# kristi700/ViT-SSL

Hardware: AMD Instinct MI355X
Metric: images_per_sec (higher is better)
Workload: dtype bf16; 1 GPU; ViT-B/16 SimMIM 224x224 mask 0.6 dropout 0.1 AdamW, batch 256/GPU; global_batch=256, parallelism=dp1

## Files before the change

### vit-ssl_amd/csrc/elementwise.hip

```cpp
#include "common.h"

namespace {

constexpr int EW_THREADS = 256;

inline unsigned ew_grid(long long work_items) {
  long long g = (work_items + EW_THREADS - 1) / EW_THREADS;
  if (g < 1) g = 1;
  return (unsigned)g;
}

__global__ void dropout_mask_kernel(unsigned char* keep, long long ngroups, DropKey dk) {
  const long long grp = (long long)blockIdx.x * blockDim.x + threadIdx.x;
  if (grp >= ngroups) return;
  float m[4];
  drop_mult4(dk, (unsigned)grp, m);
  uchar4 o;
  o.x = m[0] != 0.f; o.y = m[1] != 0.f; o.z = m[2] != 0.f; o.w = m[3] != 0.f;
  if (dk.thr == 0) o = make_uchar4(1, 1, 1, 1);
  *(uchar4*)(keep + 4 * grp) = o;
}

template <bool GATHER, typename OutT>
__global__ void patchify_kernel(const float* __restrict__ img, const int* __restrict__ idx, OutT* __restrict__ out,
                                long long nrows, int C, int H, int W, int P) {
  const int gw = W / P, gh = H / P;
  const int pd4 = C * P * P / 4;
  const long long t = (long long)blockIdx.x * blockDim.x + threadIdx.x;
  if (t >= nrows * pd4) return;
  const long long r = t / pd4;
  const int f = (int)(t - r * pd4) * 4;
  const long long m = GATHER ? (long long)idx[r] : r;
  const long long b = m / (gh * gw);
  const int pi = (int)(m - b * gh * gw);
  const int py = pi / gw, px = pi - py * gw;
  const int c = f / (P * P);
  const int kh = (f - c * P * P) / P;
  const int kw = f - c * P * P - kh * P;
  const f32x4 v = *(const f32x4*)(img + ((b * C + c) * H + (py * P + kh)) * (long long)W + px * P + kw);
  if constexpr (sizeof(OutT) == 2) {
    u32x2 w = {pack_bf2(v[0], v[1]), pack_bf2(v[2], v[3])};
    *(u32x2*)((bf16_t*)out + r * (4LL * pd4) + f) = w;
  } else {
    *(f32x4*)((float*)out + r * (4LL * pd4) + f) = v;
  }
}

__global__ void gather_rows_bf16_kernel(const float* __restrict__ x, const int* __restrict__ idx, bf16_t* __restrict__ out,
                                        int n_idx, int cols) {
  const int c4n = cols >> 2;
  const long long t = (long long)blockIdx.x * blockDim.x + threadIdx.x;
  if (t >= (long long)n_idx * c4n) return;
  const int i = (int)(t / c4n);
  const int c = (int)(t - (long long)i * c4n) * 4;
  const f32x4 v = *(const f32x4*)(x + (long long)idx[i] * cols + c);
  u32x2 w = {pack_bf2(v[0], v[1]), pack_bf2(v[2], v[3])};
  *(u32x2*)(out + (long long)i * cols + c) = w;
}

__global__ void scatter_rows_f32_kernel(const bf16_t* __restrict__ src, const int* __restrict__ inv, float* __restrict__ g,
                                        long long rows, int cols) {
  const int c4n = cols >> 2;
  const long long t = (long long)blockIdx.x * blockDim.x + threadIdx.x;
  if (t >= rows * c4n) return;
  const long long r = t / c4n;
  const int c = (int)(t - r * c4n) * 4;
  const int i = inv[r];
  f32x4 v = {0.f, 0.f, 0.f, 0.f};
  if (i >= 0) {
    const u32x2 w = *(const u32x2*)(src + (long long)i * cols + c);
    v = f32x4{bf_lo(w[0]), bf_hi(w[0]), bf_lo(w[1]), bf_hi(w[1])};
  }
  *(f32x4*)(g + r * cols + c) = v;
}

__global__ void gather_cls_kernel(const float* __restrict__ x, float* __restrict__ out, int B, int T, int D) {
  const int d4n = D >> 2;
  const long long t = (long long)blockIdx.x * blockDim.x + threadIdx.x;
  if (t >= (long long)B * d4n) return;
  const int b = (int)(t / d4n);
  const int c = (int)(t - (long long)b * d4n) * 4;
  *(f32x4*)(out + (long long)b * D + c) = *(const f32x4*)(x + (long long)b * T * D + c);
}

__global__ void scatter_cls_kernel(const float* __restrict__ gcls, float* __restrict__ g, int B, int T, int D) {
  const int d4n = D >> 2;
  const long long t = (long long)blockIdx.x * blockDim.x + threadIdx.x;
  if (t >= (long long)B * T * d4n) return;
  const long long row = t / d4n;
  const int c = (int)(t - row * d4n) * 4;
  const long long b = row / T;
  f32x4 v = {0.f, 0.f, 0.f, 0.f};
  if (row - b * T == 0) v = *(const f32x4*)(gcls + b * D + c);
  *(f32x4*)(g + row * D + c) = v;
}

__global__ void embed_bwd_kernel(const float* __restrict__ dtok, const unsigned char* __restrict__ mask,
                                 bf16_t* __restrict__ dproj, float* __restrict__ dpos, float* __restrict__ dmask_token,
                                 float* __restrict__ dbias, float* __restrict__ dcls, int B, int tokens, int tok_offset, int D,
                                 float* __restrict__ ws, float* __restrict__ pos_parts) {
  const int t = blockIdx.x;
  const int T_out = tokens + tok_offset;
  const int per = (B + gridDim.y - 1) / gridDim.y;
  const int b0 = blockIdx.y * per;
  const int b1 = min(B, b0 + per);
  for (int c = threadIdx.x * 4; c < D; c += blockDim.x * 4) {
    f32x4 pos = {0.f, 0.f, 0.f, 0.f}, mt = pos, bias = pos;
    for (int bb = b0; bb < b1; bb += 4) {
      f32x4 v[4];
#pragma unroll
      for (int u = 0; u < 4; ++u)
        if (bb + u < b1) v[u] = *(const f32x4*)(dtok + ((long long)(bb + u) * T_out + t) * D + c);
#pragma unroll
      for (int u = 0; u < 4; ++u) {
        const int b = bb + u;
        if (b >= b1) break;
        pos += v[u];
        if (t >= tok_offset) {
          const long long m = (long long)b * tokens + (t - tok_offset);
          const bool masked = mask && mask[m];
          u32x2 w = {0u, 0u};
          if (masked) {
            mt += v[u];
          } else {
            bias += v[u];
            w = u32x2{pack_bf2(v[u][0], v[u][1]), pack_bf2(v[u][2], v[u][3])};
// ... 290 lines not shown
extern "C" int vitssl_dropout_mask(uint8_t* keep, int64_t rows, int64_t cols, vitssl_dropout_t d, void* stream) {
  VS_CHECK_ARG(keep && rows > 0 && cols > 0 && cols % 4 == 0, "dropout_mask: cols must be a multiple of 4");
  VS_CHECK_ARG((unsigned long long)rows * (unsigned long long)cols < (1ull << 34), "dropout_mask: the stream's group counter is 32 bits (rows * cols < 2^34)");
  const long long ng = rows * cols / 4;
  hipLaunchKernelGGL(dropout_mask_kernel, dim3(ew_grid(ng)), dim3(EW_THREADS), 0, (hipStream_t)stream, keep, ng, make_drop_key(d));
  VS_CHECK_LAUNCH("dropout_mask");
  return VITSSL_OK;
}

static int check_patch_args(const char* who, int B, int C, int H, int W, int P) {
  VS_CHECK_ARG(B > 0 && C > 0 && P > 0 && P % 4 == 0, "%s: patch size %d must be a positive multiple of 4", who, P);
  VS_CHECK_ARG(H % P == 0 && W % P == 0, "%s: image %dx%d not divisible by patch %d", who, H, W, P);
  return VITSSL_OK;
}

extern "C" int vitssl_patchify_bf16(const float* img, void* patches, int B, int C, int H, int W, int P, void* stream) {
  VS_CHECK_ARG(img && patches, "patchify: null pointer");
  if (int rc = check_patch_args("patchify", B, C, H, W, P)) return rc;
  const long long nrows = (long long)B * (H / P) * (W / P);
  const long long work = nrows * (C * P * P / 4);
  hipLaunchKernelGGL((patchify_kernel<false, bf16_t>), dim3(ew_grid(work)), dim3(EW_THREADS), 0, (hipStream_t)stream, img,
                     (const int*)nullptr, (bf16_t*)patches, nrows, C, H, W, P);
  VS_CHECK_LAUNCH("patchify");
  return VITSSL_OK;
}

extern "C" int vitssl_gather_patches_f32(const float* img, const int32_t* idx, float* out, int n_idx, int C, int H, int W,
                                         int P, void* stream) {
  VS_CHECK_ARG(img && idx && out && n_idx > 0, "gather_patches: null pointer / empty");
  if (int rc = check_patch_args("gather_patches", 1, C, H, W, P)) return rc;
  const long long work = (long long)n_idx * (C * P * P / 4);
  hipLaunchKernelGGL((patchify_kernel<true, float>), dim3(ew_grid(work)), dim3(EW_THREADS), 0, (hipStream_t)stream, img, idx,
                     out, (long long)n_idx, C, H, W, P);
  VS_CHECK_LAUNCH("gather_patches");
  return VITSSL_OK;
}

extern "C" int vitssl_gather_rows_bf16(const float* x, const int32_t* idx, void* out, int n_idx, int cols, void* stream) {
  VS_CHECK_ARG(x && idx && out && n_idx > 0 && cols > 0 && cols % 4 == 0, "gather_rows: bad args");
  hipLaunchKernelGGL(gather_rows_bf16_kernel, dim3(ew_grid((long long)n_idx * (cols / 4))), dim3(EW_THREADS), 0,
                     (hipStream_t)stream, x, idx, (bf16_t*)out, n_idx, cols);
  VS_CHECK_LAUNCH("gather_rows");
  return VITSSL_OK;
}

extern "C" int vitssl_scatter_rows_f32(const void* src_bf16, const int32_t* inv, float* g, int64_t rows, int cols, void* stream) {
  VS_CHECK_ARG(src_bf16 && inv && g && rows > 0 && cols > 0 && cols % 4 == 0, "scatter_rows: bad args");
  hipLaunchKernelGGL(scatter_rows_f32_kernel, dim3(ew_grid(rows * (cols / 4))), dim3(EW_THREADS), 0, (hipStream_t)stream,
                     (const bf16_t*)src_bf16, inv, g, (long long)rows, cols);
  VS_CHECK_LAUNCH("scatter_rows");
  return VITSSL_OK;
}

extern "C" int vitssl_gather_cls_f32(const float* x, float* out, int B, int T, int D, void* stream) {
  VS_CHECK_ARG(x && out && B > 0 && T > 0 && D > 0 && D % 4 == 0, "gather_cls: bad args");
  hipLaunchKernelGGL(gather_cls_kernel, dim3(ew_grid((long long)B * (D / 4))), dim3(EW_THREADS), 0, (hipStream_t)stream, x, out, B, T, D);
  VS_CHECK_LAUNCH("gather_cls");
  return VITSSL_OK;
}

extern "C" int vitssl_scatter_cls_f32(const float* gcls, float* g, int B, int T, int D, void* stream) {
  VS_CHECK_ARG(gcls && g && B > 0 && T > 0 && D > 0 && D % 4 == 0, "scatter_cls: bad args");
  hipLaunchKernelGGL(scatter_cls_kernel, dim3(ew_grid((long long)B * T * (D / 4))), dim3(EW_THREADS), 0, (hipStream_t)stream, gcls, g, B, T, D);
  VS_CHECK_LAUNCH("scatter_cls");
  return VITSSL_OK;
}

static int embed_bwd_splits(int B, int T_out) {
  int bs = 2048 / T_out;
  if (bs < 1) bs = 1;
  if (bs > B) bs = B;
  if (bs > 16) bs = 16;
  return bs;
}

constexpr int EMBED_YSPLITS = 128;
static long long embed_slots_floats(int bs, int T_out, int D) {
  const long long a = (long long)bs * T_out * D, b = (long long)EMBED_YSPLITS * 2 * D;
  return a > b ? a : b;
}
static int64_t embed_ws_floats(int bs, int T_out, int D) { return (int64_t)bs * T_out * 2 * D + embed_slots_floats(bs, T_out, D); }

extern "C" int64_t vitssl_embed_bwd_workspace_floats(int B, int tokens, int tok_offset, int D) {
  if (B <= 0 || tokens <= 0 || D <= 0) return 0;
  const int T_out = tokens + tok_offset;
  return embed_ws_floats(embed_bwd_splits(B, T_out), T_out, D);
}

extern "C" int vitssl_embed_bwd(const float* dtok, const uint8_t* mask, void* dproj_bf16, float* dpos, float* dmask_token,
                                float* dbias, float* dcls, int B, int tokens, int tok_offset, int D, float* workspace,
                                int64_t workspace_floats, void* stream) {
  VS_CHECK_ARG(dtok && dproj_bf16 && B > 0 && tokens > 0 && D > 0 && D % 4 == 0, "embed_bwd: bad args");
  VS_CHECK_ARG(tok_offset == 0 || tok_offset == 1, "embed_bwd: tok_offset must be 0 or 1");
  VS_CHECK_ARG(!mask || dmask_token, "embed_bwd: mask without dmask_token");
  const int T_out = tokens + tok_offset;
  const int bs = embed_bwd_splits(B, T_out);
  const int ysplits = EMBED_YSPLITS;
  if (!vs_parts(workspace, workspace_floats, embed_ws_floats(bs, T_out, D), "embed_bwd", "vitssl_embed_bwd_workspace_floats")) return VITSSL_ERR_ARG;
  float* ws = (dmask_token || dbias) ? workspace : nullptr;
  float* parts = workspace + (long long)bs * T_out * 2 * D;
  const bool pos_sums = dpos || (dcls && tok_offset == 1);
  hipLaunchKernelGGL(embed_bwd_kernel, dim3(T_out, bs), dim3(EW_THREADS), 0, (hipStream_t)stream, dtok, mask, (bf16_t*)dproj_bf16,
                     dpos, dmask_token, dbias, dcls, B, tokens, tok_offset, D, ws, pos_sums ? parts : nullptr);
  VS_CHECK_LAUNCH("embed_bwd");
  const long long rows = (long long)T_out * D;
  if (dpos && vs_reduce_parts(dpos, parts, bs, rows, rows, (hipStream_t)stream) != VITSSL_OK) return VITSSL_ERR_LAUNCH;
// ... 89 lines not shown
```

### vit-ssl_amd/csrc/gemm_nt.hip

```cpp
#include "nt_epilogue.h"

namespace {

template <int BK_, int WM_, int WN_, int MI_ = 8>
struct NtCfg {
  static constexpr int BK = BK_, WM = WM_, WN = WN_;
  static constexpr int MI = MI_;
  static constexpr int WROWS = 16 * MI_;
  static constexpr int BM = WROWS * WM_, BN = 64 * WN_;
  static constexpr int WAVES = WM_ * WN_, THREADS = 64 * WM_ * WN_;
  static constexpr int ROWB = BK_ * 2;
  static constexpr int A_BYTES = BM * ROWB, B_BYTES = BN * ROWB;
  static constexpr int BUF_BYTES = A_BYTES + B_BYTES;
  static constexpr int LDS_BYTES = 2 * BUF_BYTES;
  static constexpr int MIN_WAVES_PER_SIMD = 2;
  static constexpr int WG_PER_CU = (WAVES == 8) ? 1 : 2;
};
using NtBig = NtCfg<64, 2, 4>;
using NtSmall = NtCfg<32, 2, 2>;
using NtBig224 = NtCfg<64, 2, 4, 7>;
using NtBig192 = NtCfg<64, 2, 4, 6>;

template <int BK_>
__device__ __forceinline__ int nt_swz(int r) {
// ... 108 lines not shown

    for (int t = 0; t < nk; ++t) {
      char* bufA = smem + par * CFG::BUF_BYTES;
      char* nA = smem + (par ^ 1) * CFG::BUF_BYTES;
      const bool more = t + 1 < nk;
      const bool fetch = more || has_next;
      const long long sm = more ? m0 : m0n;
      const int sn = more ? n0 : n0n;
      const int sk = kb + (more ? (t + 1) * BK : 0);
      if constexpr (BK == 64) {
        if (fetch) stage_tile<BK, BM, CFG::WAVES>(rsA, nA, sm, sk, p.K, wave, lane);
        compute_half(bufA, bufA + CFG::A_BYTES, IC<0>{});
        if (fetch) stage_tile<BK, BN, CFG::WAVES>(rsB, nA + CFG::A_BYTES, sn, sk, p.K, wave, lane);
        compute_half(bufA, bufA + CFG::A_BYTES, IC<1>{});
      } else {
        if (fetch) {
          stage_tile<BK, BM, CFG::WAVES>(rsA, nA, sm, sk, p.K, wave, lane);
          stage_tile<BK, BN, CFG::WAVES>(rsB, nA + CFG::A_BYTES, sn, sk, p.K, wave, lane);
        }
        compute_half(bufA, bufA + CFG::A_BYTES, IC<0>{});
      }
      par ^= 1;
      if (more) {
        asm volatile("s_waitcnt vmcnt(0)" ::: "memory");
        __syncthreads();
      }
    }

    nt_epilogue<EPI, CFG>(p, acc, m0, n0, wm, wn, lane);

    if (!has_next) break;
    constexpr int TAIL = nt_epi_tail_stores<EPI>();
    static_assert(TAIL <= nt_epi_row_ops<EPI, false>(true) * MI, "more than this epilogue is certain to store");
    wait_vmcnt_round_down<TAIL>();
    m0 = m0n;
    n0 = n0n;
  }
}

__device__ __forceinline__ i32x8 join_frags(const bf16x8& lo, const bf16x8& hi) {
  const u32x4 a = __builtin_bit_cast(u32x4, lo), b = __builtin_bit_cast(u32x4, hi);
  return i32x8{(int)a[0], (int)a[1], (int)a[2], (int)a[3], (int)b[0], (int)b[1], (int)b[2], (int)b[3]};
}

template <int EPI, typename CFG, bool F8 = false>
__global__ __launch_bounds__(CFG::THREADS, 2) void gemm_nt_pp_kernel(NtParams p) {
  extern __shared__ __attribute__((aligned(16))) char smem[];
  static_assert(CFG::BK == 64 && CFG::WM == 2 && CFG::WN == 4, "ping-pong loop is written for 8 waves, BK = 64");
  constexpr int BM = CFG::BM, BN = CFG::BN, MI = CFG::MI;
  constexpr int MH1 = MI - 4;
  constexpr int BUF = CFG::BUF_BYTES;
  constexpr int DUMMY = 2 * BUF;
  constexpr unsigned OOBV = 0x80000000u;
  constexpr bool USE_GLUT = EPI == VITSSL_EPI_GELU;
  constexpr int GLUT_BASE = 2 * BUF + 1024;
  constexpr int GLUT_IMM = USE_GLUT ? GLUT_BASE - (int)GLUT_LO8 : -1;
  static_assert(!USE_GLUT || (GLUT_IMM >= 0 && GLUT_IMM < 65536), "the table's offset must fit the ds_read immediate");

  const int lane = threadIdx.x & 63;
  const int wave = __builtin_amdgcn_readfirstlane(threadIdx.x >> 6);
  const int wm = wave >> 2, wn = wave & 3;
  const int ntiles = p.tiles_m * p.tiles_n;
  const int G = gridDim.x;
  const int bid = blockIdx.x;

  auto tile_of = [&](int r, long long& m0, int& n0) { return nt_tile_of<BM, BN>(p, ntiles, G, bid, r, m0, n0); };

  long long m0 = 0;
  int n0 = 0;
  if (!tile_of(0, m0, n0)) return;

  if (p.stagger > 0) {
    const int rem = ntiles % G;
    if (rem != 0 && bid >= rem && wave == 0) {
      const unsigned long long delay = (unsigned long long)p.stagger * (unsigned)(bid - rem) / (unsigned)(G - rem);
      const unsigned long long t0 = __builtin_amdgcn_s_memrealtime();
      while (__builtin_amdgcn_s_memrealtime() - t0 < delay) __builtin_amdgcn_s_sleep(8);
    }
  }

  constexpr unsigned ESZ = F8 ? 1u : 2u;
  const unsigned long long a_bytes = (unsigned long long)p.M * p.K * ESZ;
  const unsigned long long b_bytes = (unsigned long long)p.N * p.K * ESZ;
  const int nk = F8 ? p.K / 128 : p.K / 64;
  const unsigned rowb = (unsigned)p.K * ESZ;

  unsigned voffA[2][2], voffB[2][2];
  int ldsA[2][2], ldsB[2][2];
#pragma unroll
  for (int h = 0; h < 2; ++h)
#pragma unroll
    for (int e = 0; e < 2; ++e) {
      const int s = 2 * wave + e;
      {
        const int per_g = h == 0 ? 8 : 2 * MH1;
        const bool ok = s < 2 * per_g;
        const int g = s / per_g, q = s - g * per_g;
        const int r = g * CFG::WROWS + 64 * h + 8 * q;
        const int rl = r + (lane >> 3);
        const int sc = (lane & 7) ^ ((rl >> 1) & 7);
        voffA[h][e] = ok ? (unsigned)rl * rowb + (unsigned)sc * 16u : OOBV;
        ldsA[h][e] = ok ? r * 128 : DUMMY;
      }
      {
        const int c = s >> 2, q = s & 3;
        const int r = 64 * c + 32 * h + 8 * q;
        const int rl = r + (lane >> 3);
// ... 166 lines not shown
  constexpr int NW_POST = (NW + S) > 63 ? 63 : (NW + S);
  int buf = 0;
#ifdef VITSSL_NT_STAMPS
  auto stamp = [&](int round, int which) {
    if (!(p.stamps && (wave & 3) == 0 && lane == 0 && round < 16)) return;
    p.stamps[(((size_t)bid * 2 + wm) * 16 + round) * 4 + which] = __builtin_amdgcn_s_memrealtime();
    p.stamps[(size_t)256 * 2 * 16 * 4 + (((size_t)bid * 2 + wm) * 16 + round) * 4 + which] = __builtin_amdgcn_s_memtime();
  };
#else
  auto stamp = [&](int, int) {};
#endif
  for (int round = 0;; ++round) {
    stamp(round, 0);
    if (wm == 1) raw_barrier();
#pragma unroll
    for (int j = 0; j < 4; ++j)
#pragma unroll
      for (int i = 0; i < MI; ++i) acc[j][i] = f32x4{0.f, 0.f, 0.f, 0.f};
    for (int t = 0; t < nk; ++t) {
      const bool last = t + 1 == nk;
      if (t == 0 && round > 0) ktile(buf, c1, c2, last, IC<NW_POST>{});
      else ktile(buf, c1, c2, last, IC<NW>{});
      c1 = c2;
      c2 = cur_next(c2);
      buf ^= 1;
    }
    stamp(round, 1);
    if constexpr (F8) {
      if (p.alpha || p.alpha2) {
        const float al = (p.alpha ? *p.alpha : 1.0f) * (p.alpha2 ? *p.alpha2 : 1.0f);
#pragma unroll
        for (int j = 0; j < 4; ++j)
#pragma unroll
          for (int i = 0; i < MI; ++i) acc[j][i] *= al;
      }
    }
    nt_epilogue<EPI, CFG, F8, GLUT_IMM, true>(p, acc, m0, n0, wm, wn, lane, smem, smem + (buf ^ 1) * BUF + ldsB[1][0]);
    stamp(round, 2);
#ifdef VITSSL_NT_STAMPS
    if (p.stamps) {
      asm volatile("s_waitcnt vmcnt(0)" ::: "memory");
      stamp(round, 3);
    }
#endif
    if (!tile_of(round + 1, m0, n0)) break;
  }
  asm volatile("s_waitcnt vmcnt(0)" ::: "memory");
}

int cu_count() { return vitssl_persistent_cus(); }

template <int EPI, typename CFG, bool F8 = false>
int launch_pp(NtParams p, hipStream_t s) {
  constexpr int LDS = 2 * CFG::BUF_BYTES + 1024 + (EPI == VITSSL_EPI_GELU ? GLUT_BYTES : 0);
  static VsOnce attr_done{false};
  if (int rc = ensure_lds(gemm_nt_pp_kernel<EPI, CFG, F8>, LDS, attr_done, "gemm_nt")) return rc;
  const long long ntiles = (long long)p.tiles_m * p.tiles_n;
  const long long slots = cu_count();
  const long long grid = ntiles < slots ? ntiles : slots;
  constexpr float STAGGER_SCALE = 1.0f;
  static VsEnvMilli stagger_knob;
  const float stagger_scale = stagger_knob.get("VITSSL_NT_STAGGER", STAGGER_SCALE);
  constexpr int STAGGER_EPIS = (1 << VITSSL_EPI_RESID) | (1 << VITSSL_EPI_DGELU);
  static VsEnvInt stagger_mask_knob;
  const int stagger_mask = stagger_mask_knob.get("VITSSL_NT_STAGGER_EPIS", STAGGER_EPIS);
  const float tile_us = (float)(p.K * p.esz / 128) * 1.45f * (float)CFG::MI / 8.f + nt_epi(EPI).epi_us;
  p.stagger = ((stagger_mask >> nt_epi(EPI).stagger_bit) & 1) ? (int)(stagger_scale * tile_us * 100.f) : 0;
  vitssl_note_nt_grid((int)grid);
  hipLaunchKernelGGL((gemm_nt_pp_kernel<EPI, CFG, F8>), dim3((unsigned)grid), dim3(CFG::THREADS), LDS, s, p);
  VS_CHECK_LAUNCH("gemm_nt_pp");
  return VITSSL_OK;
}

template <int EPI, typename CFG>
int launch_cfg_parts(NtParams p, hipStream_t s) {
  if constexpr (CFG::LDS_BYTES > 48 * 1024) {
    static VsOnce attr_done{false};
    if (int rc = ensure_lds(gemm_nt_kernel<EPI, CFG>, CFG::LDS_BYTES, attr_done, "gemm_nt")) return rc;
  }
  p.tiles_m = (int)ceil_div64(p.M, CFG::BM);
  p.tiles_n = (int)ceil_div64(p.N, CFG::BN);
  const int want = (int)((2 * 1024 * 1024) / ((long long)CFG::BN * p.K * p.esz));
  static VsEnvInt group_env;
  const int group_knob = group_env.get("VITSSL_NT_GROUPN", 0);
  if (group_knob > 0) p.group_n = group_knob < p.tiles_n ? group_knob : p.tiles_n;
  else if (p.tiles_n <= 4) p.group_n = p.tiles_n;
  else if (want <= 2) p.group_n = 2;
  else if (p.tiles_n % 6 == 0 && want >= 6) p.group_n = 6;
  else if (p.tiles_n % 4 == 0) p.group_n = 4;
  else if (p.tiles_n % 3 == 0) p.group_n = 3;
  else p.group_n = want < 4 ? want : 4;
  if (p.esz == 1) {
    if ((p.N & 7) != 0) {
      vitssl_set_error("gemm_fp8_nt: N=%d must be a multiple of 8", p.N);
      return VITSSL_ERR_ARG;
    }
    if constexpr (CFG::WAVES == 8 && CFG::BK == 64 && nt_epi(EPI).fp8) {
      return launch_pp<EPI, CFG, true>(p, s);
    } else {
      vitssl_set_error("gemm_fp8_nt: epilogue %d / tile configuration not built for fp8 operands", EPI);
      return VITSSL_ERR_ARG;
    }
  }
  if constexpr (CFG::WAVES == 8 && CFG::BK == 64 && EPI != EPI_F32_SPLITK) {
    if (p.k_chunk == 0 && (p.N & 7) == 0) return launch_pp<EPI, CFG>(p, s);
  }
  static VsEnvInt persist_env;
// ... 44 lines not shown
  p.colsum = vs_sum_parts(p.workspace, p.workspace_floats, (long long)groups * p.N, p.M, p.N, "gemm_nt column sums");
  if (!p.colsum) return VITSSL_ERR_ARG;
  const int rc = launch_cfg_parts<EPI, CFG>(p, s);
  if (rc != VITSSL_OK) return rc;
  return vs_reduce_parts(colsum, p.colsum, groups, p.N, p.N, s);
}

template <int EPI>
int launch_nt(const NtParams& p, hipStream_t s) {
  if constexpr (EPI == VITSSL_EPI_F32) {
    if (!p.colsum && p.esz == 2) {
      bool done = false;
      const int rc = launch_splitk_f32(p, s, &done);
      if (rc != VITSSL_OK || done) return rc;
    }
  }
  const int mode = p.esz == 1 ? 0 : nt_tile_override();
  if (mode == 1) return launch_cfg<EPI, NtBig>(p, s);
  if (mode == 2) return launch_cfg<EPI, NtSmall>(p, s);
  if (mode == 3) return launch_cfg<EPI, NtBig192>(p, s);
  if (mode == 4) return launch_cfg<EPI, NtBig224>(p, s);
  const long long big_tiles = ceil_div64(p.M, 256) * ceil_div64(p.N, 256);
  if (big_tiles < 64 && p.esz == 2) return launch_cfg<EPI, NtSmall>(p, s);
  const long long slots = cu_count();
  const long long tn = ceil_div64(p.N, 256);
  const double c256 = (double)ceil_div64(ceil_div64(p.M, 256) * tn, slots);
  const double c224 = 0.90 * (double)ceil_div64(ceil_div64(p.M, 224) * tn, slots);
  const double c192 = 0.78 * (double)ceil_div64(ceil_div64(p.M, 192) * tn, slots);
  double best = c256;
  if (c192 < 0.9 * c256 && c192 <= c224) best = c192;
  else if (c224 < 0.95 * c256) best = c224;
  if (best == c192 && best != c256) return launch_cfg<EPI, NtBig192>(p, s);
  if (best == c224 && best != c256) return launch_cfg<EPI, NtBig224>(p, s);
  return launch_cfg<EPI, NtBig>(p, s);
}

}

#ifdef VITSSL_NT_STAMPS
static unsigned long long* g_nt_stamps = nullptr;
extern "C" void vitssl_debug_nt_stamps(void* buf) { g_nt_stamps = (unsigned long long*)buf; }
#endif

static NtEpiFacts caller_epi(int epi) { return nt_epi(epi >= EPI_F32_SPLITK ? -1 : epi); }

static int check_rowscale(const char* who, const vitssl_rowscale_t* rows, int64_t M) {
  VS_CHECK_ARG(rows->scale && rows->groups > 0 && rows->rows_per_group > 0, "%s: row scales need scale, groups > 0 and rows_per_group > 0", who);
  VS_CHECK_ARG(rows->groups * (int64_t)rows->rows_per_group == M, "%s: groups (%lld) * rows_per_group (%d) must equal M (%lld)", who,
               (long long)rows->groups, rows->rows_per_group, (long long)M);
  return VITSSL_OK;
}

static int gemm_nt_entry(const vitssl_gemm_t* g, int esz, const vitssl_fp8_gemm_t* q, void* stream, const vitssl_rowscale_t* rows = nullptr,
                         const vitssl_colscale_t* cols = nullptr, void* branch = nullptr) {
  const char* who = cols ? "gemm_nt_ls" : rows ? "gemm_nt_rows" : esz == 1 ? "gemm_fp8_nt" : "gemm_nt";
  VS_CHECK_ARG(g && g->A && g->B && (g->out0 || (esz == 1 && caller_epi(g->epilogue).q8_of == 0 && q && q->out_fp8)), "%s: null operand", who);
  VS_CHECK_ARG(g->M > 0 && g->N > 0 && g->K > 0, "%s: empty problem M=%lld N=%d K=%d", who, (long long)g->M, g->N, g->K);
  VS_CHECK_ARG(g->K % (128 / esz) == 0, "%s: K=%d must be a multiple of %d", who, g->K, 128 / esz);
  VS_CHECK_ARG(g->N % 4 == 0, "%s: N=%d must be a multiple of 4", who, g->N);
  VS_CHECK_ARG(g->N <= (1 << 20), "%s: N=%d exceeds 2^20 (epilogue windows use 32-bit byte offsets)", who, g->N);
  VS_CHECK_ARG((unsigned long long)g->M * g->K * (unsigned)esz < (1ull << 31) && (unsigned long long)g->N * g->K * (unsigned)esz < (1ull << 31),
               "%s: operand larger than 2 GiB (M=%lld N=%d K=%d)", who, (long long)g->M, g->N, g->K);
  NtParams p{(const bf16_t*)g->A, (const bf16_t*)g->B, g->M, g->N, g->K, g->bias, g->aux, g->out0, g->out1, g->colsum, g->workspace,
             g->workspace_floats, make_drop_key(g->drop)};
  p.drop_on = p.dk.thr != 0;
  p.embed = g->embed;
  p.esz = esz;
  if (q) {
    p.alpha = q->alpha;
    p.alpha2 = q->alpha2;
    p.out2 = q->out_fp8;
    p.qscale = q->out_scale;
    p.qamax = q->out_amax;
  }
  p.rows_per_group = 1;
#ifdef VITSSL_NT_STAMPS
  p.stamps = g_nt_stamps;
#endif
  hipStream_t s = (hipStream_t)stream;
  VS_CHECK_ARG(!g->colsum || caller_epi(g->epilogue).colsum, "%s: column sums are built for the BF16 / F32 / DGELU epilogues only", who);
  VS_CHECK_ARG(!p.drop_on || (unsigned long long)g->M * (unsigned long long)g->N < (1ull << 34),
               "%s: dropout over %lld x %d elements: the stream's group counter is 32 bits (M * N < 2^34)", who, (long long)g->M, g->N);
  if (rows || cols) {
    VS_CHECK_ARG(g->epilogue == VITSSL_EPI_RESID, "%s: %s scales are built for VITSSL_EPI_RESID only, got epilogue %d", who,
                 cols ? "column" : "row", g->epilogue);
    VS_CHECK_ARG(g->aux, "%s: EPI_RESID needs aux (residual)", who);
    if (cols) {
      VS_CHECK_ARG(cols->gamma, "%s: null gamma", who);
      VS_CHECK_ARG(cols->cols == g->N, "%s: cols (%d) must equal N (%d)", who, cols->cols, g->N);
    }
    if (rows) {
      if (int rc = check_rowscale(who, rows, g->M)) return rc;
      p.rowscale = rows->scale;
      p.rows_per_group = (unsigned)rows->rows_per_group;
    }
    if (!cols) return launch_nt<EPI_RESID_ROWS>(p, s);
    p.colscale = cols->gamma;
    p.out1 = branch;
    return launch_nt<EPI_RESID_LS>(p, s);
  }
  switch (g->epilogue) {
    case VITSSL_EPI_BF16: return launch_nt<VITSSL_EPI_BF16>(p, s);
    case VITSSL_EPI_F32: return launch_nt<VITSSL_EPI_F32>(p, s);
    case VITSSL_EPI_GELU:
      VS_CHECK_ARG(g->out1 || p.out2, "%s: EPI_GELU needs out1 (or, with fp8 operands, out_fp8)", who);
      return launch_nt<VITSSL_EPI_GELU>(p, s);
    case VITSSL_EPI_RESID:
      VS_CHECK_ARG(g->aux, "%s: EPI_RESID needs aux (residual)", who);
      return launch_nt<VITSSL_EPI_RESID>(p, s);
    case VITSSL_EPI_DGELU:
      VS_CHECK_ARG(g->aux, "%s: EPI_DGELU needs aux (pre-activation)", who);
      return launch_nt<VITSSL_EPI_DGELU>(p, s);
    case VITSSL_EPI_EMBED:
      VS_CHECK_ARG(g->embed.pos && g->embed.tokens > 0 && g->embed.out_tokens >= g->embed.tokens + g->embed.tok_offset,
                   "%s: EPI_EMBED needs pos/tokens", who);
      VS_CHECK_ARG(!g->embed.mask || g->embed.mask_token, "%s: EPI_EMBED mask without mask_token", who);
      return launch_nt<VITSSL_EPI_EMBED>(p, s);
    default:
      vitssl_set_error("%s: unknown epilogue %d", who, g->epilogue);
      return VITSSL_ERR_ARG;
  }
}

extern "C" int vitssl_gemm_bf16_nt(const vitssl_gemm_t* g, void* stream) { return gemm_nt_entry(g, 2, nullptr, stream); }

extern "C" int vitssl_gemm_bf16_nt_rows(const vitssl_gemm_t* g, const vitssl_rowscale_t* rows, void* stream) {
  VS_CHECK_ARG(rows, "gemm_nt_rows: null row scales (vitssl_gemm_bf16_nt is the launch without them)");
  return gemm_nt_entry(g, 2, nullptr, stream, rows);
}

extern "C" int vitssl_gemm_bf16_nt_ls(const vitssl_gemm_t* g, const vitssl_colscale_t* cols, const vitssl_rowscale_t* rows,
                                      void* branch_bf16, void* stream) {
  VS_CHECK_ARG(cols, "gemm_nt_ls: null column scales (vitssl_gemm_bf16_nt / vitssl_gemm_bf16_nt_rows are the launches without them)");
  return gemm_nt_entry(g, 2, nullptr, stream, rows, cols, branch_bf16);
}

extern "C" int vitssl_gemm_fp8_nt(const vitssl_gemm_t* g, const vitssl_fp8_gemm_t* q, void* stream) {
  VS_CHECK_ARG(g && caller_epi(g->epilogue).fp8, "gemm_fp8_nt: fp8 operands are built for the BF16 / F32 / GELU / RESID / DGELU epilogues");
  VS_CHECK_ARG(!(q && q->out_fp8) || caller_epi(g->epilogue).q8_of >= 0, "gemm_fp8_nt: out_fp8 belongs to EPI_GELU / EPI_DGELU");
  return gemm_nt_entry(g, 1, q, stream);
}
```

### vit-ssl_amd/csrc/layernorm.hip

```cpp
#include "../../include/vitssl_droppath.h"
#include "../../include/vitssl_layerscale.h"
#include "common.h"

namespace {

constexpr int LN_THREADS = 256;

template <int V, bool Q8 = false>
__global__ __launch_bounds__(LN_THREADS) void ln_fwd_kernel(const float* __restrict__ x, const float* __restrict__ gamma,
                                                            const float* __restrict__ beta, bf16_t* __restrict__ y,
                                                            float* __restrict__ mean, float* __restrict__ rstd,
                                                            long long rows, int cols, float eps, unsigned char* __restrict__ y8 = nullptr) {
  const int lane = threadIdx.x & 63;
  const int wave = threadIdx.x >> 6;
  const int c4n = cols >> 2;
  f32x4 g[V], b[V];
#pragma unroll
  for (int v = 0; v < V; ++v) {
    const int c4 = lane + 64 * v;
    if (c4 < c4n) {
      g[v] = *(const f32x4*)(gamma + 4 * c4);
      b[v] = *(const f32x4*)(beta + 4 * c4);
    }
  }
  const float inv = 1.0f / (float)cols;
  const long long row_step = (long long)gridDim.x * 4;
  f32x4 nxt[V];
  auto fetch = [&](long long row) {
    if (row >= rows) return;
#pragma unroll
    for (int v = 0; v < V; ++v) {
      const int c4 = lane + 64 * v;
      if (c4 < c4n) nxt[v] = *(const f32x4*)(x + row * cols + 4 * c4);
    }
  };
  fetch((long long)blockIdx.x * 4 + wave);
  for (long long row = (long long)blockIdx.x * 4 + wave; row < rows; row += row_step) {
    f32x4 xv[V];
    float s = 0.f;
#pragma unroll
    for (int v = 0; v < V; ++v) {
      const int c4 = lane + 64 * v;
      if (c4 < c4n) {
        xv[v] = nxt[v];
        s += xv[v][0] + xv[v][1] + xv[v][2] + xv[v][3];
      }
    }
    fetch(row + row_step);
    const float mu = wave_sum(s) * inv;
    float ss = 0.f;
#pragma unroll
    for (int v = 0; v < V; ++v) {
      const int c4 = lane + 64 * v;
      if (c4 < c4n) {
        xv[v] -= mu;
        ss += xv[v][0] * xv[v][0] + xv[v][1] * xv[v][1] + xv[v][2] * xv[v][2] + xv[v][3] * xv[v][3];
      }
    }
    const float rs = rsqrtf(wave_sum(ss) * inv + eps);
    if (lane == 0) {
      mean[row] = mu;
      rstd[row] = rs;
    }
    bf16_t* yr = y + row * cols;
#pragma unroll
    for (int v = 0; v < V; ++v) {
      const int c4 = lane + 64 * v;
      if (c4 < c4n) {
        const f32x4 o = xv[v] * rs * g[v] + b[v];
        if (!Q8 || y) {
          u32x2 w = {pack_bf2(o[0], o[1]), pack_bf2(o[2], o[3])};
          *(u32x2*)(yr + 4 * c4) = w;
        }
        if constexpr (Q8) *(unsigned*)(y8 + row * cols + 4 * c4) = pack_fp8x4(o[0], o[1], o[2], o[3]);
      }
    }
  }
}

constexpr int ln_bwd_blocks(int V, bool has_ln, bool has_cs) {
  if (!has_ln) return (V <= 2 || (V == 3 && !has_cs)) ? 4 : (V <= 4 ? 3 : 1);
  return V <= 1 ? 4 : (V == 2 ? (has_cs ? 3 : 4) : (V == 3 ? (has_cs ? 2 : 3) : (V == 4 ? 2 : 1)));
}

struct LnLsArgs {
  const float* gamma;
  const bf16_t* branch;
  float* dls;
};
__device__ __forceinline__ const LnLsArgs& ln_first(const LnLsArgs& a) { return a; }
constexpr int ln_bwd_ls_blocks(int V, bool has_ln) { return has_ln && V == 4 ? 1 : ln_bwd_blocks(V, has_ln, true); }

template <int V, bool HAS_LN, bool HAS_CS, bool Q8 = false, bool PAIR = false, bool ROWS = false, typename... LSARGS>
__global__ __launch_bounds__(LN_THREADS, sizeof...(LSARGS) ? ln_bwd_ls_blocks(V, HAS_LN) : ln_bwd_blocks(V, HAS_LN, HAS_CS || (ROWS && PAIR))) void ln_bwd_kernel(const bf16_t* __restrict__ dy, const float* __restrict__ x,
                                                            const float* __restrict__ mean, const float* __restrict__ rstd,
                                                            const float* __restrict__ gamma, const float* g_res,
                                                            float* g_out, bf16_t* __restrict__ gm, float* __restrict__ dgamma,
                                                            float* __restrict__ dbeta, float* __restrict__ gm_colsum,
                                                            DropKey dk, int drop_on, long long rows, int cols,
                                                            unsigned char* __restrict__ gm8 = nullptr,
                                                            const float* __restrict__ qscale = nullptr, float* qamax = nullptr,
                                                            const float* __restrict__ rowscale = nullptr, unsigned rows_per_group = 1,
                                                            LSARGS... lsargs) {
  constexpr bool LS = sizeof...(LSARGS) > 0;
  const float* __restrict__ lsgamma = nullptr;
  const bf16_t* __restrict__ branch = nullptr;
  float* __restrict__ dls = nullptr;
  if constexpr (LS) {
    const LnLsArgs& a = ln_first(lsargs...);
    lsgamma = a.gamma;
    branch = a.branch;
    dls = a.dls;
  }
  __shared__ __attribute__((aligned(16))) float red[4][V * 256];
  const int lane = threadIdx.x & 63;
  const int wave = threadIdx.x >> 6;
  const int c4n = cols >> 2;
  const int c4h = PAIR ? c4n >> 1 : c4n;
  static_assert(!PAIR || (HAS_LN && !Q8), "row pairs are built for the LayerNorm form with a bf16 image");
  static_assert(!ROWS || !Q8, "row scales are built for the bf16 image");
  static_assert(!LS || (ROWS && HAS_CS), "LayerScale is built on the form with row scales and column sums");
  f32x4 g[V], acc_dg[V], acc_db[V], acc_cs[V];
  f32x4 lsg[V], acc_ls[V];
  bool hi[V];
#pragma unroll
  for (int v = 0; v < V; ++v) {
    const int c4 = lane + 64 * v;
    hi[v] = PAIR && c4 >= c4h;
    acc_dg[v] = f32x4{0.f, 0.f, 0.f, 0.f};
    acc_db[v] = acc_dg[v];
    acc_cs[v] = acc_dg[v];
    if (HAS_LN && c4 < c4n) g[v] = *(const f32x4*)(gamma + 4 * (c4 - (hi[v] ? c4h : 0)));
    if constexpr (LS) {
      acc_ls[v] = acc_dg[v];
      if (c4 < c4n) lsg[v] = *(const f32x4*)(lsgamma + 4 * (c4 - (hi[v] ? c4h : 0)));
    }
  }
  const float inv = 1.0f / (float)(PAIR ? cols >> 1 : cols);
  const float qs = (Q8 && qscale) ? *qscale : 1.0f;
  float qmax = 0.f;
  f32x4 nx[V], ngr[V];
  u32x2 ndy[V];
  u32x2 nbr[V];
  float nmu = 0.f, nrs = 0.f, nmuB = 0.f, nrsB = 0.f;
  float nsc = 1.f, nscB = 1.f;
  auto fetch = [&](long long row) {
    if (!HAS_LN || row >= rows) return;
    if constexpr (ROWS && !LS) {
      nsc = rowscale[(PAIR ? 2u * (unsigned)row : (unsigned)row) / rows_per_group];
      if constexpr (PAIR) nscB = rowscale[(2u * (unsigned)row + 1u) / rows_per_group];
    }
    if constexpr (LS) {
      if (rowscale) {
        nsc = rowscale[(PAIR ? 2u * (unsigned)row : (unsigned)row) / rows_per_group];
        if constexpr (PAIR) nscB = rowscale[(2u * (unsigned)row + 1u) / rows_per_group];
      }
    }
    if constexpr (PAIR) {
      nmu = mean[2 * row];
      nrs = rstd[2 * row];
      nmuB = mean[2 * row + 1];
      nrsB = rstd[2 * row + 1];
    } else {
      nmu = mean[row];
      nrs = rstd[row];
    }
#pragma unroll
    for (int v = 0; v < V; ++v) {
      const int c4 = lane + 64 * v;
      if (c4 < c4n) {
        if (g_res) ngr[v] = *(const f32x4*)(g_res + row * cols + 4 * c4);
        ndy[v] = *(const u32x2*)(dy + row * cols + 4 * c4);
        if constexpr (LS) {
          if (dls) nbr[v] = *(const u32x2*)(branch + row * cols + 4 * c4);
        }
        nx[v] = *(const f32x4*)(x + row * cols + 4 * c4);
      }
    }
  };
  const long long row_step = (long long)gridDim.x * 4;
  fetch((long long)blockIdx.x * 4 + wave);
  for (long long row = (long long)blockIdx.x * 4 + wave; row < rows; row += row_step) {
    f32x4 dx[V];
    u32x2 brp[V];
    float sc = 1.f, scB = 1.f;
    if constexpr (ROWS && !HAS_LN && !LS) sc = rowscale[__builtin_amdgcn_readfirstlane((unsigned)row / rows_per_group)];
    if constexpr (LS && !HAS_LN) {
      if (rowscale) sc = rowscale[__builtin_amdgcn_readfirstlane((unsigned)row / rows_per_group)];
    }
    if constexpr (ROWS && HAS_LN) {
      sc = nsc;
      scB = nscB;
    }
    if constexpr (HAS_LN) {
      const float mu = nmu, rs = nrs, muB = nmuB, rsB = nrsB;
      f32x4 xh[V], gr[V];
      u32x2 dyp[V];
#pragma unroll
      for (int v = 0; v < V; ++v) {
        xh[v] = nx[v];
        gr[v] = ngr[v];
        dyp[v] = ndy[v];
      }
      if constexpr (LS) {
#pragma unroll
        for (int v = 0; v < V; ++v) brp[v] = nbr[v];
      }
      fetch(row + row_step);
      float s1 = 0.f, s2 = 0.f, s1B = 0.f, s2B = 0.f;
#pragma unroll
      for (int v = 0; v < V; ++v) {
        const int c4 = lane + 64 * v;
        if (c4 < c4n) {
          const f32x4 d = {bf_lo(dyp[v][0]), bf_hi(dyp[v][0]), bf_lo(dyp[v][1]), bf_hi(dyp[v][1])};
          xh[v] = (xh[v] - (hi[v] ? muB : mu)) * (hi[v] ? rsB : rs);
          const f32x4 dyg = d * g[v];
          acc_dg[v] += d * xh[v];
          acc_db[v] += d;
          const float t1 = dyg[0] + dyg[1] + dyg[2] + dyg[3];
          const f32x4 t = dyg * xh[v];
          const float t2 = t[0] + t[1] + t[2] + t[3];
          if (hi[v]) {
            s1B += t1;
            s2B += t2;
          } else {
            s1 += t1;
            s2 += t2;
          }
        }
      }
      const float m1 = wave_sum(s1) * inv;
      const float m2 = wave_sum(s2) * inv;
      const float m1B = PAIR ? wave_sum(s1B) * inv : 0.f;
      const float m2B = PAIR ? wave_sum(s2B) * inv : 0.f;
#pragma unroll
      for (int v = 0; v < V; ++v) {
        const int c4 = lane + 64 * v;
        if (c4 < c4n) {
          const f32x4 d = {bf_lo(dyp[v][0]), bf_hi(dyp[v][0]), bf_lo(dyp[v][1]), bf_hi(dyp[v][1])};
          dx[v] = (d * g[v] - (hi[v] ? m1B : m1) - xh[v] * (hi[v] ? m2B : m2)) * (hi[v] ? rsB : rs);
          if (g_res) dx[v] += gr[v];
          *(f32x4*)(g_out + row * cols + 4 * c4) = dx[v];
        }
      }
    } else {
#pragma unroll
      for (int v = 0; v < V; ++v) {
        const int c4 = lane + 64 * v;
        if (c4 < c4n) dx[v] = *(const f32x4*)(g_res + row * cols + 4 * c4);
        if constexpr (LS) {
          if (dls && c4 < c4n) brp[v] = *(const u32x2*)(branch + row * cols + 4 * c4);
        }
      }
    }
    if (gm || (Q8 && gm8)) {
#pragma unroll
      for (int v = 0; v < V; ++v) {
        const int c4 = lane + 64 * v;
        if (c4 < c4n) {
          f32x4 o = dx[v];
          if (drop_on) {
            bool keep[4];
            drop_keep4(dk, drop_words(dk, (unsigned)row * (unsigned)c4n + (unsigned)c4), keep);
#pragma unroll
            for (int r = 0; r < 4; ++r) o[r] = keep[r] ? o[r] * dk.scale : 0.f;
          }
          if constexpr (ROWS) o *= hi[v] ? scB : sc;
          if constexpr (LS) {
            o *= lsg[v];
            if (dls) {
              const float rsv = hi[v] ? scB : sc;
              const f32x4 u = {bf_lo(brp[v][0]), bf_hi(brp[v][0]), bf_lo(brp[v][1]), bf_hi(brp[v][1])};
#pragma unroll
              for (int r = 0; r < 4; ++r) acc_ls[v][r] += rsv == 0.f ? 0.f : rsv * dx[v][r] * u[r];
            }
          }
          if (gm) {
            u32x2 w = {pack_bf2(o[0], o[1]), pack_bf2(o[2], o[3])};
            *(u32x2*)(gm + row * cols + 4 * c4) = w;
          }
          if constexpr (Q8) {
            *(unsigned*)(gm8 + row * cols + 4 * c4) = pack_fp8x4(o[0] * qs, o[1] * qs, o[2] * qs, o[3] * qs);
            qmax = fmaxf(qmax, fmaxf(fmaxf(fabsf(o[0]), fabsf(o[1])), fmaxf(fabsf(o[2]), fabsf(o[3]))));
          }
          if (HAS_CS) acc_cs[v] += o;
        }
      }
    }
  }
  if constexpr (Q8) {
    if (qamax) {
      qmax = wave_max(qmax);
      unsigned* slot = (unsigned*)qamax;
      if (lane == 0 && __float_as_uint(qmax) > __builtin_nontemporal_load(slot)) atomicMax(slot, __float_as_uint(qmax));
    }
  }
#pragma unroll
  for (int qty = 0; qty < (LS ? 4 : 3); ++qty) {
    if (qty < 2 && !HAS_LN) continue;
    if (qty == 2 && !HAS_CS) continue;
    float* target = qty == 0 ? dgamma : (qty == 1 ? dbeta : gm_colsum);
    if constexpr (LS) {
      if (qty == 3) target = dls;
    }
    if (!target) continue;
#pragma unroll
    for (int v = 0; v < V; ++v) {
      const int c4 = lane + 64 * v;
      if (c4 < c4n) {
        f32x4 a = qty == 0 ? acc_dg[v] : (qty == 1 ? acc_db[v] : acc_cs[v]);
        if constexpr (LS) {
          if (qty == 3) a = acc_ls[v];
        }
        *(f32x4*)&red[wave][4 * c4] = a;
      }
    }
    __syncthreads();
    if constexpr (PAIR) {
      const int ch = cols >> 1;
      for (int c = threadIdx.x; c < ch; c += LN_THREADS)
        target[(long long)blockIdx.x * ch + c] = (red[0][c] + red[1][c] + red[2][c] + red[3][c]) +
                                                 (red[0][c + ch] + red[1][c + ch] + red[2][c + ch] + red[3][c + ch]);
    } else {
      for (int c = threadIdx.x; c < cols; c += LN_THREADS)
        target[(long long)blockIdx.x * cols + c] = red[0][c] + red[1][c] + red[2][c] + red[3][c];
    }
    __syncthreads();
  }
}

constexpr long long LN_FWD_GRID_CAP = 4096;
inline int ln_grid(long long rows, bool fwd = false, int cols = 1024) {
  long long g = (rows + 3) / 4;
  long long cap = fwd ? LN_FWD_GRID_CAP : (long long)vitssl_persistent_cus() * (cols <= 512 ? 2 : 1);
  if (g > cap) g = cap;
  if (g < 1) g = 1;
  return (int)g;
}

struct LnBwdCall {
  const char* who;
  const void* dy;
  const float *x, *mean, *rstd, *gamma, *g_res;
  float* g_out;
  void* gm;
  float *dgamma, *dbeta, *gm_colsum;
  vitssl_dropout_t drop;
  int64_t rows;
  int cols;
  float* workspace;
  int64_t workspace_floats;
  hipStream_t s;
  void* gm8;
  const float* qscale;
  float* qamax;
  const vitssl_rowscale_t* rowscale;
  const float* lsgamma;
  const void* branch;
  float* dls;
};

template <bool HAS_LN, bool Q8 = false, bool ROWS = false, bool LS = false>
int launch_ln_bwd(const LnBwdCall& c) {
  static_assert(!Q8 || !ROWS, "row scales are built for the bf16 image");
  static_assert(!LS || ROWS, "LayerScale is built on the form with row scales");
  const int64_t rows = c.rows;
  const int cols = c.cols;
  DropKey dk = make_drop_key(c.drop);
  const int on = dk.thr != 0;
  VS_CHECK_ARG(!on || (unsigned long long)rows * (unsigned long long)cols < (1ull << 34),
               "%s: the dropout stream's group counter is 32 bits (rows * cols < 2^34)", c.who);
  constexpr bool CAN_PAIR = HAS_LN && !Q8;
  const bool pair = CAN_PAIR && cols == 384 && (rows & 1) == 0;
  const long long krows = pair ? rows / 2 : rows;
  const int kcols = pair ? 768 : cols;
  const int grid = ln_grid(krows, false, kcols);
  const long long slab = (long long)grid * cols;

  constexpr int NSUMS = LS ? 4 : 3;
  float* const target[4] = {HAS_LN ? c.dgamma : nullptr, HAS_LN ? c.dbeta : nullptr, c.gm_colsum, LS ? c.dls : nullptr};
  float* slot[4] = {nullptr, nullptr, nullptr, nullptr};
  const bool sums = target[0] || target[1] || target[2] || target[3];
  if (sums) {
    const char* sizing = LS ? "vitssl_layerscale_workspace_floats" : "vitssl_sum_workspace_floats";
    const long long promised = LS ? vitssl_layerscale_workspace_floats(rows, cols) : vitssl_sum_workspace_floats(rows, cols);
    VS_CHECK_ARG(NSUMS * slab <= promised, "%s: this launch needs %lld floats of workspace, %s(%lld, %d) promises %lld", c.who,
                 NSUMS * slab, sizing, (long long)rows, cols, promised);
    float* parts = vs_parts(c.workspace, c.workspace_floats, promised, c.who, sizing);
    if (!parts) return VITSSL_ERR_ARG;
    for (int q = 0; q < NSUMS; ++q)
      if (target[q]) slot[q] = parts + q * slab;
  }

  const float* rscale = c.rowscale ? c.rowscale->scale : nullptr;
  const unsigned rpg = c.rowscale ? (unsigned)c.rowscale->rows_per_group : 1u;
#define VS_LN_BWD_ARGS                                                                                                              \
  dim3(grid), dim3(LN_THREADS), 0, c.s, (const bf16_t*)c.dy, c.x, c.mean, c.rstd, c.gamma, c.g_res, c.g_out, (bf16_t*)c.gm, slot[0], \
      slot[1], slot[2], dk, on, krows, kcols, (unsigned char*)c.gm8, c.qscale, c.qamax, rscale, rpg
  auto launch = [&](auto v, auto cs, auto pr) {
    constexpr int V = decltype(v)::value;
    constexpr bool CS = decltype(cs)::value, PAIR = decltype(pr)::value;
    static_assert(!PAIR || (CAN_PAIR && V == 3), "row pairs: the LayerNorm form with a bf16 image, 2 x 384 columns");
    static_assert(!LS || CS, "LayerScale is built with the column sums");
    if constexpr (LS)
      hipLaunchKernelGGL((ln_bwd_kernel<V, HAS_LN, CS, Q8, PAIR, ROWS, LnLsArgs>), VS_LN_BWD_ARGS,
                         LnLsArgs{c.lsgamma, (const bf16_t*)c.branch, slot[3]});
    else
      hipLaunchKernelGGL((ln_bwd_kernel<V, HAS_LN, CS, Q8, PAIR, ROWS>), VS_LN_BWD_ARGS);
  };
#undef VS_LN_BWD_ARGS
  auto with_cs = [&](auto v, auto pr) {
    if (LS || c.gm_colsum) launch(v, std::true_type{}, pr);
    else if constexpr (!LS) launch(v, std::false_type{}, pr);
  };
  using std::integral_constant;
  if (pair) {
    if constexpr (CAN_PAIR) with_cs(integral_constant<int, 3>{}, std::true_type{});
  } else if (cols <= 256) with_cs(integral_constant<int, 1>{}, std::false_type{});
  else if (cols <= 512) with_cs(integral_constant<int, 2>{}, std::false_type{});
  else if (cols <= 768) with_cs(integral_constant<int, 3>{}, std::false_type{});
  else if (cols <= 1024) with_cs(integral_constant<int, 4>{}, std::false_type{});
  else with_cs(integral_constant<int, 8>{}, std::false_type{});
  VS_CHECK_LAUNCH(LS ? c.who : (ROWS ? "layernorm_bwd_rows" : "layernorm_bwd"));
  if (!sums) return VITSSL_OK;
  return vs_reduce_parts(VsSums{{target[0], target[1], target[2], target[3]}, {slot[0], slot[1], slot[2], slot[3]}}, grid, cols, cols, c.s);
}

template <bool Q8>
int launch_ln_fwd(const char* who, const float* x, const float* gamma, const float* beta, void* y_bf16, void* y_fp8, float* mean,
                  float* rstd, int64_t rows, int cols, float eps, hipStream_t s) {
  const int grid = ln_grid(rows, true);
#define VS_LNF(V)                                                                                                                 \
  hipLaunchKernelGGL((ln_fwd_kernel<V, Q8>), dim3(grid), dim3(LN_THREADS), 0, s, x, gamma, beta, (bf16_t*)y_bf16, mean, rstd, \
                     (long long)rows, cols, eps, (unsigned char*)y_fp8)
  if (cols <= 256) VS_LNF(1);
  else if (cols <= 512) VS_LNF(2);
  else if (cols <= 768) VS_LNF(3);
  else if (cols <= 1024) VS_LNF(4);
  else VS_LNF(8);
#undef VS_LNF
  VS_CHECK_LAUNCH(who);
  return VITSSL_OK;
}

}

extern "C" int vitssl_layernorm_fwd(const float* x, const float* gamma, const float* beta, void* y_bf16, float* mean,
                                    float* rstd, int64_t rows, int cols, float eps, void* stream) {
  VS_CHECK_ARG(x && gamma && beta && y_bf16 && mean && rstd, "layernorm_fwd: null pointer");
  VS_CHECK_ARG(rows > 0 && cols > 0 && cols % 4 == 0 && cols <= 2048, "layernorm_fwd: cols=%d must be a multiple of 4 and <= 2048", cols);
  return launch_ln_fwd<false>("layernorm_fwd", x, gamma, beta, y_bf16, nullptr, mean, rstd, rows, cols, eps, (hipStream_t)stream);
}

extern "C" int vitssl_layernorm_fwd_fp8(const float* x, const float* gamma, const float* beta, void* y_bf16, void* y_fp8,
                                        float* mean, float* rstd, int64_t rows, int cols, float eps, void* stream) {
  VS_CHECK_ARG(x && gamma && beta && y_fp8 && mean && rstd, "layernorm_fwd_fp8: null pointer");
  VS_CHECK_ARG(rows > 0 && cols > 0 && cols % 4 == 0 && cols <= 2048, "layernorm_fwd_fp8: cols=%d must be a multiple of 4 and <= 2048", cols);
  return launch_ln_fwd<true>("layernorm_fwd_fp8", x, gamma, beta, y_bf16, y_fp8, mean, rstd, rows, cols, eps, (hipStream_t)stream);
}
// ... 49 lines not shown
}

extern "C" int vitssl_grad_mask_cast_rows(const float* g, void* gm_bf16, float* gm_colsum, vitssl_dropout_t drop,
                                          const vitssl_rowscale_t* rowscale, int64_t rows, int cols, float* workspace,
                                          int64_t workspace_floats, void* stream) {
  VS_CHECK_ARG(g && gm_bf16, "grad_mask_cast_rows: null pointer");
  VS_CHECK_ARG(rows > 0 && cols > 0 && cols % 4 == 0 && cols <= 2048, "grad_mask_cast_rows: cols=%d must be a multiple of 4 and <= 2048", cols);
  if (int rc = check_rowscale("grad_mask_cast_rows", rowscale, rows)) return rc;
  return launch_ln_bwd<false, false, true>({LN_BWD_WHO, nullptr, nullptr, nullptr, nullptr, nullptr, g, nullptr, gm_bf16, nullptr, nullptr,
                                            gm_colsum, drop, rows, cols, workspace, workspace_floats, (hipStream_t)stream, nullptr, nullptr,
                                            nullptr, rowscale});
}

extern "C" int vitssl_grad_mask_cast(const float* g, void* gm_bf16, float* gm_colsum, vitssl_dropout_t drop,
                                     int64_t rows, int cols, float* workspace, int64_t workspace_floats, void* stream) {
  VS_CHECK_ARG(g && gm_bf16, "grad_mask_cast: null pointer");
  VS_CHECK_ARG(rows > 0 && cols > 0 && cols % 4 == 0 && cols <= 2048, "grad_mask_cast: cols=%d must be a multiple of 4 and <= 2048", cols);
  return launch_ln_bwd<false>({LN_BWD_WHO, nullptr, nullptr, nullptr, nullptr, nullptr, g, nullptr, gm_bf16, nullptr, nullptr, gm_colsum, drop,
                               rows, cols, workspace, workspace_floats, (hipStream_t)stream});
}

static int check_ls(const char* who, const vitssl_rowscale_t* rowscale, const vitssl_colscale_t* colscale, const void* branch,
                    const float* dls, int64_t rows, int cols) {
  VS_CHECK_ARG(rows > 0 && cols > 0 && cols % 4 == 0 && cols <= 2048, "%s: cols=%d must be a multiple of 4 and <= 2048", who, cols);
  VS_CHECK_ARG(rows < (1ll << 31), "%s: rows = %lld outside rows < 2^31", who, (long long)rows);
  VS_CHECK_ARG(colscale && colscale->gamma, "%s: null column scales", who);
  VS_CHECK_ARG(colscale->cols == cols, "%s: column scales hold %d entries for %d columns", who, colscale->cols, cols);
  VS_CHECK_ARG((branch != nullptr) == (dls != nullptr), "%s: branch_bf16 and dls are given together or not at all", who);
  if (rowscale) return check_rowscale(who, rowscale, rows);
  return VITSSL_OK;
}

extern "C" int vitssl_layernorm_bwd_ls(const void* dy_bf16, const float* x, const float* mean, const float* rstd, const float* gamma,
                                       const float* g_res, float* g_out, void* gm_bf16, float* dgamma, float* dbeta, float* gm_colsum,
                                       vitssl_dropout_t drop, const vitssl_rowscale_t* rowscale, const vitssl_colscale_t* colscale,
                                       const void* branch_bf16, float* dls, int64_t rows, int cols, float* workspace,
                                       int64_t workspace_floats, void* stream) {
  VS_CHECK_ARG(dy_bf16 && x && mean && rstd && gamma && g_out && dgamma && dbeta && gm_bf16, "layernorm_bwd_ls: null pointer");
  if (int rc = check_ls("layernorm_bwd_ls", rowscale, colscale, branch_bf16, dls, rows, cols)) return rc;
  return launch_ln_bwd<true, false, true, true>({"layernorm_bwd_ls", dy_bf16, x, mean, rstd, gamma, g_res, g_out, gm_bf16, dgamma, dbeta,
                                                 gm_colsum, drop, rows, cols, workspace, workspace_floats, (hipStream_t)stream, nullptr, nullptr,
                                                 nullptr, rowscale, colscale->gamma, branch_bf16, dls});
}

extern "C" int vitssl_grad_mask_cast_ls(const float* g, void* gm_bf16, float* gm_colsum, vitssl_dropout_t drop,
                                        const vitssl_rowscale_t* rowscale, const vitssl_colscale_t* colscale, const void* branch_bf16,
                                        float* dls, int64_t rows, int cols, float* workspace, int64_t workspace_floats, void* stream) {
  VS_CHECK_ARG(g && gm_bf16, "grad_mask_cast_ls: null pointer");
  if (int rc = check_ls("grad_mask_cast_ls", rowscale, colscale, branch_bf16, dls, rows, cols)) return rc;
  return launch_ln_bwd<false, false, true, true>({"grad_mask_cast_ls", nullptr, nullptr, nullptr, nullptr, nullptr, g, nullptr, gm_bf16, nullptr,
                                                  nullptr, gm_colsum, drop, rows, cols, workspace, workspace_floats, (hipStream_t)stream,
                                                  nullptr, nullptr, nullptr, rowscale, colscale->gamma, branch_bf16, dls});
}
```

### vit-ssl_amd/csrc/nt_epilogue.h

```cpp
#pragma once
#include "../../include/vitssl_droppath.h"
#include "../../include/vitssl_layerscale.h"
#include "common.h"

namespace {

struct NtParams {
  const bf16_t* A;
  const bf16_t* B;
  long long M;
  int N, K;
  const float* bias;
  const void* aux;
  void* out0;
  void* out1;
  float* colsum;
  float* workspace;
  int64_t workspace_floats;
  DropKey dk;
  int drop_on;
  vitssl_embed_t embed;
  int tiles_m, tiles_n;
  int group_n;
  int k_chunk;
  int stagger;
  int esz;
  const float* alpha;
  void* out2;
  const float* alpha2;
  const float* qscale;
  float* qamax;
  const float* rowscale;
  unsigned rows_per_group;
  const float* colscale;
#ifdef VITSSL_NT_STAMPS
  unsigned long long* stamps;
#endif
};

constexpr int EPI_F32_SPLITK = 100;
constexpr int EPI_RESID_ROWS = 101;
constexpr int EPI_RESID_LS = 102;

enum NtOut1 { OUT1_NONE, OUT1_REQUIRED, OUT1_OPTIONAL };
struct NtEpiFacts {
  int out0_esz;
  bool windowed;
  NtOut1 out1;
  int aux_esz;
  bool colsum, fp8;
  int q8_of;
  bool drops, resid;
  int stagger_bit;
  float epi_us;
};
constexpr NtEpiFacts nt_epi(int epi) {
  switch (epi) {
    case VITSSL_EPI_BF16:  return NtEpiFacts{2, true,  OUT1_NONE,     0, true,  true,  -1, false, false, VITSSL_EPI_BF16,  2.f};
    case VITSSL_EPI_F32:   return NtEpiFacts{4, true,  OUT1_NONE,     0, true,  true,  -1, false, false, VITSSL_EPI_F32,   4.f};
    case VITSSL_EPI_GELU:  return NtEpiFacts{2, true,  OUT1_REQUIRED, 0, false, true,   1, true,  false, VITSSL_EPI_GELU,  7.f};
    case VITSSL_EPI_RESID: return NtEpiFacts{4, true,  OUT1_NONE,     4, false, true,  -1, true,  true,  VITSSL_EPI_RESID, 8.f};
    case VITSSL_EPI_DGELU: return NtEpiFacts{2, true,  OUT1_NONE,     2, true,  true,   0, false, false, VITSSL_EPI_DGELU, 5.f};
    case VITSSL_EPI_EMBED: return NtEpiFacts{4, false, OUT1_NONE,     0, false, false, -1, false, false, VITSSL_EPI_EMBED, 4.f};
    case EPI_F32_SPLITK:   return NtEpiFacts{4, false, OUT1_NONE,     0, false, false, -1, false, false, -1,               4.f};
    case EPI_RESID_ROWS:   return NtEpiFacts{4, true,  OUT1_NONE,     4, false, false, -1, true,  true,  VITSSL_EPI_RESID, 8.f};
    case EPI_RESID_LS:     return NtEpiFacts{4, true,  OUT1_OPTIONAL, 4, false, false, -1, true,  true,  VITSSL_EPI_RESID, 8.f};
    default:               return NtEpiFacts{0, false, OUT1_NONE,     0, false, false, -1, false, false, -1,               0.f};
  }
}

template <int EPI, int MI, bool PREF>
constexpr int nt_row_group() {
  return nt_epi(EPI).resid ? (PREF ? 1 : (MI % 2 == 0 ? 2 : 1)) : EPI == VITSSL_EPI_DGELU ? (PREF ? 2 : (MI % 4 == 0 ? 4 : 2)) : 4;
}

template <int EPI, bool F8>
constexpr int nt_epi_row_ops(bool stores_only) {
  constexpr NtEpiFacts E = nt_epi(EPI);
  if (!E.windowed) return 0;
  const int out0 = (F8 && E.q8_of == 0) ? 1 : E.out0_esz;
  const int out1 = E.out1 != OUT1_REQUIRED ? 0 : (F8 && E.q8_of == 1) ? 1 : 2;
  return (stores_only ? 0 : E.aux_esz) + out0 + out1;
}
template <int EPI, int MI, bool F8>
constexpr int nt_epi_vmem_ops() { return nt_epi_row_ops<EPI, F8>(false) * MI; }
template <int EPI>
constexpr int nt_epi_tail_stores() { return nt_epi_row_ops<EPI, false>(true) * nt_row_group<EPI, 8, false>(); }
template <int EPI, int MI>
constexpr bool nt_counts_are(int bf, int f8, int tail) {
  return nt_epi_vmem_ops<EPI, MI, false>() == bf * MI && (!nt_epi(EPI).fp8 || nt_epi_vmem_ops<EPI, MI, true>() == f8 * MI) &&
         nt_epi_tail_stores<EPI>() == tail;
}
template <int MI>
constexpr bool nt_counts_are_as_written() {
  return nt_counts_are<VITSSL_EPI_BF16, MI>(2, 2, 8) && nt_counts_are<VITSSL_EPI_GELU, MI>(4, 3, 16) && nt_counts_are<VITSSL_EPI_DGELU, MI>(4, 3, 8) &&
         nt_counts_are<VITSSL_EPI_F32, MI>(4, 4, 16) && nt_counts_are<VITSSL_EPI_RESID, MI>(8, 8, 8) && nt_counts_are<EPI_RESID_ROWS, MI>(8, 8, 8) &&
         nt_counts_are<EPI_RESID_LS, MI>(8, 8, 8) && nt_counts_are<VITSSL_EPI_EMBED, MI>(0, 0, 0) && nt_counts_are<EPI_F32_SPLITK, MI>(0, 0, 0);
}
static_assert(nt_counts_are_as_written<6>() && nt_counts_are_as_written<7>() && nt_counts_are_as_written<8>(), "epilogue vmem counts");


constexpr int GLUT_E_LO = 127 - 14;
constexpr int GLUT_BINADES = 18;
constexpr int GLUT_ENTRIES = GLUT_BINADES * 128 * 2;
constexpr int GLUT_BYTES = GLUT_ENTRIES * 4;
constexpr unsigned GLUT_LO8 = (unsigned)GLUT_E_LO << 10;
constexpr unsigned GLUT_HI8 = (unsigned)(GLUT_E_LO + GLUT_BINADES) << 10;

__device__ __forceinline__ unsigned glut_rot2(unsigned w) {
  unsigned t, r;
  asm("v_pk_lshrrev_b16 %0, 15, %1 op_sel_hi:[0,1]" : "=v"(t) : "v"(w));
  asm("v_pk_mad_u16 %0, %1, 2, %2 op_sel_hi:[1,0,1]" : "=v"(r) : "v"(w), "v"(t));
  return r;
}
__device__ __forceinline__ void glut_addr2(unsigned r, unsigned& a0, unsigned& a1) {
  asm("v_lshlrev_b32_sdwa %0, 2, %1 dst_sel:DWORD dst_unused:UNUSED_PAD src0_sel:DWORD src1_sel:WORD_0" : "=v"(a0) : "v"(r));
  asm("v_lshlrev_b32_sdwa %0, 2, %1 dst_sel:DWORD dst_unused:UNUSED_PAD src0_sel:DWORD src1_sel:WORD_1" : "=v"(a1) : "v"(r));
}
__device__ __forceinline__ bool glut_out_of_range(unsigned r01, unsigned r23) {
  const unsigned lo2 = ((unsigned)GLUT_E_LO << 8) * 0x10001u, span = ((unsigned)(GLUT_BINADES << 8) - 1u) * 0x10001u;
  unsigned d01, d23, dm, e;
  asm("v_pk_sub_u16 %0, %1, %2" : "=v"(d01) : "v"(r01), "s"(lo2));
  asm("v_pk_sub_u16 %0, %1, %2" : "=v"(d23) : "v"(r23), "s"(lo2));
  asm("v_pk_max_u16 %0, %1, %2" : "=v"(dm) : "v"(d01), "v"(d23));
  asm("v_pk_sub_u16 %0, %1, %2 clamp" : "=v"(e) : "v"(dm), "s"(span));
  return e != 0;
}
template <int OFF>
__device__ __forceinline__ unsigned glut_read(const char* smem, unsigned a) {
  (void)smem;
  return *(const __attribute__((address_space(3))) unsigned*)(unsigned long long)(a + (unsigned)OFF);
}

struct NtWindow {
  char* xs;
  unsigned tw16, tr16a, tw32, tr32a;
  __device__ __forceinline__ void lines_of_bf16(const u32x2 (&w)[2][2], u32x4& s1, u32x4& s2) const {
#pragma unroll
    for (int j = 0; j < 4; ++j) *(u32x2*)(xs + (tw16 ^ (unsigned)(32 * j))) = w[j >> 1][j & 1];
    s1 = *(const u32x4*)(xs + tr16a);
    s2 = *(const u32x4*)(xs + ((tr16a + 1024u) ^ 64u));
  }
  __device__ __forceinline__ void put_lines_bf16(const u32x4& s1, const u32x4& s2) const {
    *(u32x4*)(xs + tr16a) = s1;
    *(u32x4*)(xs + ((tr16a + 1024u) ^ 64u)) = s2;
  }
  __device__ __forceinline__ u32x2 bf16_of_lines(int j) const { return *(const u32x2*)(xs + (tw16 ^ (unsigned)(32 * j))); }
  __device__ __forceinline__ void lines_of_f32(const f32x4& v0, const f32x4& v1, u32x4& s1, u32x4& s2) const {
    *(f32x4*)(xs + tw32) = v0;
    *(f32x4*)(xs + (tw32 ^ 64u)) = v1;
    s1 = *(const u32x4*)(xs + tr32a);
    s2 = *(const u32x4*)(xs + tr32a + 1024);
  }
  __device__ __forceinline__ void f32_of_lines(f32x4& v0, f32x4& v1) const {
    *(f32x4*)(xs + tr32a) = v0;
    *(f32x4*)(xs + tr32a + 1024) = v1;
    v0 = *(const f32x4*)(xs + tw32);
    v1 = *(const f32x4*)(xs + (tw32 ^ 64u));
  }
};

__device__ __forceinline__ float amax4(float a, float b, float c, float d) { return fmaxf(fmaxf(fabsf(a), fabsf(b)), fmaxf(fabsf(c), fabsf(d))); }

template <int EPI, typename CFG, bool Q8 = false, int GLUT_OFF = -1, bool TLS = false>
__device__ __forceinline__ void nt_epilogue(const NtParams& p, f32x4 (&acc)[4][CFG::MI], const long long m0, const int n0,
                                            const int wm, const int wn, const int lane_in, const char* lds = nullptr, char* xs = nullptr) {
  constexpr int MI = CFG::MI;
  constexpr NtEpiFacts E = nt_epi(EPI);
  constexpr bool LS = EPI == EPI_RESID_LS;
  int lane = lane_in;
  if (TLS) asm volatile("" : "+v"(lane));
  constexpr bool GLUT = EPI == VITSSL_EPI_GELU && GLUT_OFF >= 0;
  const bool glut_on = GLUT && (!Q8 || (p.out1 == nullptr && p.qamax == nullptr));
  constexpr bool CS = E.colsum, DROPS = E.drops;
  float csum[4][4];
  if (CS && p.colsum) {
#pragma unroll
    for (int j = 0; j < 4; ++j)
#pragma unroll
      for (int r = 0; r < 4; ++r) csum[j][r] = 0.f;
  }
  const int g4 = lane >> 4;
  const bool wide = TLS || (p.N & 7) == 0;
  constexpr unsigned OOB = 0x80000000u;
  const long long rows_left = p.M - m0;
  auto window = [&](const void* base, int elt) {
    const unsigned long long bytes = (unsigned long long)rows_left * (unsigned long long)p.N * (unsigned)elt;
    const unsigned rec = bytes > 0x80000000ull ? 0x80000000u : (unsigned)bytes;
    return __builtin_amdgcn_make_buffer_rsrc((void*)((const char*)base + m0 * p.N * elt), 0, (int)rec, 0x00020000);
  };
  const unsigned row_l = (unsigned)(wm * CFG::WROWS + (lane & 15));
  const unsigned un = (unsigned)p.N;
  const int odd = g4 & 1;

  auto off_bf16_wide = [&](int i, int jp) -> unsigned {
    const int n = n0 + wn * 64 + (2 * jp + odd) * 16 + 4 * (g4 - odd);
    return n < p.N ? ((row_l + 16u * i) * un + (unsigned)n) * 2u : OOB;
  };
  auto off_elem = [&](int i, int n, unsigned elt) -> unsigned { return n < p.N ? ((row_l + 16u * i) * un + (unsigned)n) * elt : OOB; };
  constexpr bool tls = TLS;
  const int tm = lane & 15, trho = lane >> 3, tkap = lane & 7;
  const unsigned tw16 = (unsigned)(tm * 128 + ((g4 ^ (2 * (tm >> 1))) << 3));
  const unsigned tr16a = (unsigned)(trho * 128 + ((tkap ^ (trho >> 1)) << 4));
  const unsigned tw32 = (unsigned)(tm * 128 + ((g4 ^ (tm & 7)) << 4));
  const unsigned tr32a = (unsigned)(trho * 128 + ((tkap ^ trho) << 4));
  const NtWindow win{xs, tw16, tr16a, tw32, tr32a};
  const unsigned trow = (unsigned)(wm * CFG::WROWS + trho);
  const int tn16 = n0 + wn * 64 + 8 * tkap;
  const unsigned tb16 = tn16 < p.N ? (trow * un + (unsigned)tn16) * 2u : OOB;
  auto off_line16 = [&](int i, int half) -> unsigned { return tb16 + (unsigned)(16 * i + 8 * half) * (un * 2u); };
  auto off_line32 = [&](int i, int jp, int half) -> unsigned {
    const int n = n0 + wn * 64 + 32 * jp + 4 * tkap;
    const unsigned b = n < p.N ? (trow * un + (unsigned)n) * 4u : OOB;
    return b + (unsigned)(16 * i + 8 * half) * (un * 4u);
  };
  int nn[2][2];
  bool okn[2][2];
  auto pack_pair = [&](const u32x2& w0, const u32x2& w1) -> u32x4 {
    auto lo = __builtin_amdgcn_permlane16_swap(w0[0], w1[0], false, false);
    auto hi = __builtin_amdgcn_permlane16_swap(w0[1], w1[1], false, false);
    return u32x4{lo[0], hi[0], lo[1], hi[1]};
  };
  auto store_bf16_row = [&](__amdgpu_buffer_rsrc_t rs, int i, const u32x2 (&w)[2][2], auto aux_c) {
    constexpr int AUXV = decltype(aux_c)::value;
    if (tls) {
// ... 20 lines not shown
      u32x4 s1, s2;
      win.lines_of_f32(v0, v1, s1, s2);
      __builtin_amdgcn_raw_buffer_store_b128(s1, rs, off_line32(i, jp, 0), 0, F32_AUX);
      __builtin_amdgcn_raw_buffer_store_b128(s2, rs, off_line32(i, jp, 1), 0, F32_AUX);
    } else {
      __builtin_amdgcn_raw_buffer_store_b128(__builtin_bit_cast(u32x4, v0), rs, off_elem(i, nnp[0], 4u), 0, F32_AUX);
      __builtin_amdgcn_raw_buffer_store_b128(__builtin_bit_cast(u32x4, v1), rs, off_elem(i, nnp[1], 4u), 0, F32_AUX);
    }
  };
  auto store_fp8_row = [&](__amdgpu_buffer_rsrc_t rs, int i, const unsigned (&out_q)[2][2]) {
    if ((p.N & 15) == 0) {
      auto s02 = __builtin_amdgcn_permlane32_swap(out_q[0][0], out_q[1][0], false, false);
      auto s13 = __builtin_amdgcn_permlane32_swap(out_q[0][1], out_q[1][1], false, false);
      auto e = __builtin_amdgcn_permlane16_swap(s02[0], s13[0], false, false);
      auto f = __builtin_amdgcn_permlane16_swap(s02[1], s13[1], false, false);
      if (tls) {
        *(u32x4*)(xs + tm * 64 + ((g4 ^ ((tm >> 1) & 3)) << 4)) = u32x4{e[0], e[1], f[0], f[1]};
        const int rho4 = lane >> 2, kap4 = lane & 3;
        const u32x4 s8 = *(const u32x4*)(xs + rho4 * 64 + ((kap4 ^ ((rho4 >> 1) & 3)) << 4));
        const int n8 = n0 + wn * 64 + 16 * kap4;
        const unsigned o8 = n8 < p.N ? ((unsigned)(wm * CFG::WROWS + 16 * i + rho4) * un + (unsigned)n8) : OOB;
        __builtin_amdgcn_raw_buffer_store_b128(s8, rs, o8, 0, 0);
      } else {
        const int n = n0 + wn * 64 + 16 * g4;
        __builtin_amdgcn_raw_buffer_store_b128(u32x4{e[0], e[1], f[0], f[1]}, rs, off_elem(i, n, 1u), 0, 0);
      }
    } else {
#pragma unroll
      for (int jp = 0; jp < 2; ++jp)
#pragma unroll
        for (int h = 0; h < 2; ++h) __builtin_amdgcn_raw_buffer_store_b32(out_q[jp][h], rs, off_elem(i, nn[jp][h], 1u), 0, 0);
    }
  };

  __amdgpu_buffer_rsrc_t rsOut0, rsOut1, rsOut2, rsAux;
  constexpr bool Q8EPI = Q8 && E.q8_of >= 0;
  const bool q8 = Q8EPI && p.out2 != nullptr;
  if (q8) rsOut2 = window(p.out2, 1);
  const float qs = (Q8EPI && p.qscale) ? *p.qscale : 1.0f;
  float qmax = 0.f;
  if constexpr (E.windowed) rsOut0 = window(p.out0, E.out0_esz);
  if constexpr (E.out1 != OUT1_NONE) {
    if (E.out1 == OUT1_REQUIRED || p.out1) rsOut1 = window(p.out1, 2);
  }
  if constexpr (E.aux_esz != 0) rsAux = window(p.aux, E.aux_esz);

  f32x4 bias4[2][2];
  f32x4 gam4[2][2];
  unsigned a0col[2][2];
  const unsigned a0rowstep = 16u * (unsigned)(p.N >> 2) * DROP_C0;
  unsigned a0row = 0;
  if (DROPS && p.drop_on)
    a0row = drop_a0(p.dk, (unsigned)(m0 + wm * CFG::WROWS + (lane & 15)) * (unsigned)(p.N >> 2));
  const float gelu_hs = (DROPS && p.drop_on) ? 0.5f * p.dk.scale : 0.5f;
  const float gelu_cs = (DROPS && p.drop_on) ? 0.3989422804014327f * p.dk.scale : 0.3989422804014327f;
#pragma unroll
  for (int jp = 0; jp < 2; ++jp)
#pragma unroll
    for (int h = 0; h < 2; ++h) {
      nn[jp][h] = n0 + wn * 64 + (2 * jp + h) * 16 + 4 * g4;
      a0col[jp][h] = (unsigned)(nn[jp][h] >> 2) * DROP_C0;
      okn[jp][h] = nn[jp][h] < p.N;
      bias4[jp][h] = f32x4{0.f, 0.f, 0.f, 0.f};
      if (p.bias && (EPI != EPI_F32_SPLITK || blockIdx.y == 0) && okn[jp][h]) bias4[jp][h] = *(const f32x4*)(p.bias + nn[jp][h]);
      if constexpr (LS) {
        gam4[jp][h] = f32x4{0.f, 0.f, 0.f, 0.f};
        if (okn[jp][h]) gam4[jp][h] = *(const f32x4*)(p.colscale + nn[jp][h]);
      }
    }

  constexpr bool PREF = TLS && E.aux_esz != 0;
  constexpr int RG = nt_row_group<EPI, MI, PREF>();
  constexpr int NB = PREF ? 2 : 1;
  f32x4 res[NB][RG][2][2];
  u32x4 raw[NB][RG][2];
  float rsc[NB][RG];
  auto load_group = [&](const int ig, const int b) {
    const int cnt = MI - ig < RG ? MI - ig : RG;
    if constexpr (EPI == EPI_RESID_ROWS || LS) {
#pragma unroll
      for (int ii = 0; ii < RG; ++ii) {
        if (ii >= cnt) continue;
        if constexpr (LS) rsc[b][ii] = 1.0f;
        if (EPI == EPI_RESID_ROWS || p.rowscale) {
          const long long mr = m0 + wm * CFG::WROWS + (ig + ii) * 16 + (lane & 15);
          rsc[b][ii] = p.rowscale[mr < p.M ? (unsigned)mr / p.rows_per_group : 0u];
        }
      }
    }
    if constexpr (E.resid) {
#pragma unroll
      for (int ii = 0; ii < RG; ++ii)
#pragma unroll
        for (int jp = 0; jp < 2; ++jp) {
          if (ii >= cnt) continue;
          if (tls) {
            res[b][ii][jp][0] = __builtin_bit_cast(f32x4, __builtin_amdgcn_raw_buffer_load_b128(rsAux, off_line32(ig + ii, jp, 0), 0, 0));
            res[b][ii][jp][1] = __builtin_bit_cast(f32x4, __builtin_amdgcn_raw_buffer_load_b128(rsAux, off_line32(ig + ii, jp, 1), 0, 0));
          } else {
#pragma unroll
            for (int h = 0; h < 2; ++h)
              res[b][ii][jp][h] = __builtin_bit_cast(f32x4, __builtin_amdgcn_raw_buffer_load_b128(rsAux, off_elem(ig + ii, nn[jp][h], 4u), 0, 0));
          }
        }
    }
    if constexpr (EPI == VITSSL_EPI_DGELU) {
// ... 35 lines not shown
              }
              continue;
            }
            auto sa = __builtin_amdgcn_permlane16_swap(raw[gb][ii][jp][0], raw[gb][ii][jp][2], false, false);
            auto sb = __builtin_amdgcn_permlane16_swap(raw[gb][ii][jp][1], raw[gb][ii][jp][3], false, false);
            gpre[ii][jp][0] = u32x2{sa[0], sb[0]};
            gpre[ii][jp][1] = u32x2{sa[1], sb[1]};
          }
      } else {
#pragma unroll
        for (int ii = 0; ii < RG; ++ii)
#pragma unroll
          for (int jp = 0; jp < 2; ++jp)
#pragma unroll
            for (int h = 0; h < 2; ++h)
              if (ii < cnt) gpre[ii][jp][h] = __builtin_amdgcn_raw_buffer_load_b64(rsAux, off_elem(ig + ii, nn[jp][h], 2u), 0, 0);
      }
    }

#pragma unroll
    for (int ii = 0; ii < RG; ++ii) {
      if (ii >= cnt) continue;
      const int i = ig + ii;
      const long long m = m0 + wm * CFG::WROWS + i * 16 + (lane & 15);
      const bool okm = m < p.M;
      u32x2 out_a[2][2], out_b[2][2];
      unsigned out_q[2][2];
      unsigned gl[16];
      bool gslow[2][2];
      if (GLUT && glut_on) {
#pragma unroll
        for (int jp = 0; jp < 2; ++jp)
#pragma unroll
          for (int h = 0; h < 2; ++h) {
            const f32x4 vv = acc[2 * jp + h][i] + bias4[jp][h];
            const unsigned w0 = pack_bf2(vv[0], vv[1]), w1 = pack_bf2(vv[2], vv[3]);
            const unsigned r01 = glut_rot2(w0), r23 = glut_rot2(w1);
            gslow[jp][h] = __builtin_amdgcn_ballot_w64(glut_out_of_range(r01, r23)) != 0;
            unsigned ad[4];
            glut_addr2(r01, ad[0], ad[1]);
            glut_addr2(r23, ad[2], ad[3]);
            const int q = 8 * jp + 4 * h;
#pragma unroll
            for (int r = 0; r < 4; ++r) gl[q + r] = glut_read<GLUT_OFF>(lds, ad[r]);
          }
      }
#pragma unroll
      for (int jp = 0; jp < 2; ++jp) {
        f32x4 v[2] = {acc[2 * jp][i] + bias4[jp][0], acc[2 * jp + 1][i] + bias4[jp][1]};

        if constexpr (EPI == VITSSL_EPI_BF16) {
          out_a[jp][0] = u32x2{pack_bf2(v[0][0], v[0][1]), pack_bf2(v[0][2], v[0][3])};
          out_a[jp][1] = u32x2{pack_bf2(v[1][0], v[1][1]), pack_bf2(v[1][2], v[1][3])};
        } else if constexpr (EPI == VITSSL_EPI_GELU) {
          unsigned km[2][2] = {{0xffffffffu, 0xffffffffu}, {0xffffffffu, 0xffffffffu}};
          u32x2 dw[2] = {u32x2{0u, 0u}, u32x2{0u, 0u}};
          const bool dropping = p.drop_on;
          if (dropping) {
#pragma unroll
            for (int h = 0; h < 2; ++h) {
              dw[h] = drop_words_a0(p.dk, a0row + (unsigned)i * a0rowstep + a0col[jp][h]);
              km[h][0] = drop_keep_pair(p.dk, dw[h][0]);
              km[h][1] = drop_keep_pair(p.dk, dw[h][1]);
            }
          }
#pragma unroll
          for (int h = 0; h < 2; ++h) {
            if (GLUT && glut_on && !gslow[jp][h]) {
              const int q = 8 * jp + 4 * h;
              const u32x2 lo = u32x2{__builtin_amdgcn_perm(gl[q + 1], gl[q], 0x05040100u) & km[h][0],
                                     __builtin_amdgcn_perm(gl[q + 3], gl[q + 2], 0x05040100u) & km[h][1]};
              if constexpr (!Q8) {
                out_b[jp][h] = lo;
                out_a[jp][h] = u32x2{__builtin_amdgcn_perm(gl[q + 1], gl[q], 0x07060302u) & km[h][0],
                                     __builtin_amdgcn_perm(gl[q + 3], gl[q + 2], 0x07060302u) & km[h][1]};
              } else {
                out_a[jp][h] = lo;
                const unsigned b01 = __builtin_amdgcn_perm(gl[q + 1], gl[q], 0x0c0c0602u), b23 = __builtin_amdgcn_perm(gl[q + 3], gl[q + 2], 0x06020c0cu);
                out_q[jp][h] = (b01 | b23) & __builtin_amdgcn_perm(km[h][1], km[h][0], 0x06040200u);
              }
              continue;
            }
            float y[4], d[4];
#pragma unroll
            for (int r = 0; r < 4; ++r) gelu_both_scaled(round_bf(v[h][r]), gelu_hs, gelu_cs, y[r], d[r]);
            out_b[jp][h] = u32x2{pack_bf2(y[0], y[1]) & km[h][0], pack_bf2(y[2], y[3]) & km[h][1]};
            out_a[jp][h] = u32x2{pack_bf2(d[0], d[1]) & km[h][0], pack_bf2(d[2], d[3]) & km[h][1]};
            if constexpr (Q8) {
              if (dropping) {
                bool keep[4];
                drop_keep4(p.dk, dw[h], keep);
#pragma unroll
                for (int r = 0; r < 4; ++r) y[r] = keep[r] ? y[r] : 0.f;
              }
              out_q[jp][h] = pack_fp8x4(y[0] * qs, y[1] * qs, y[2] * qs, y[3] * qs);
              if (okm && okn[jp][h]) qmax = fmaxf(qmax, amax4(y[0], y[1], y[2], y[3]));
            }
          }
        } else if constexpr (EPI == VITSSL_EPI_DGELU) {
#pragma unroll
          for (int h = 0; h < 2; ++h) {
            const u32x2 gpv = gpre[ii][jp][h];
            v[h][0] *= bf_lo(gpv[0]);
            v[h][1] *= bf_hi(gpv[0]);
            v[h][2] *= bf_lo(gpv[1]);
            v[h][3] *= bf_hi(gpv[1]);
            out_a[jp][h] = u32x2{pack_bf2(v[h][0], v[h][1]), pack_bf2(v[h][2], v[h][3])};
            if constexpr (Q8) {
              out_q[jp][h] = pack_fp8x4(v[h][0] * qs, v[h][1] * qs, v[h][2] * qs, v[h][3] * qs);
              if (okm && okn[jp][h]) qmax = fmaxf(qmax, amax4(v[h][0], v[h][1], v[h][2], v[h][3]));
            }
          }
        } else if constexpr (EPI == EPI_F32_SPLITK) {
#pragma unroll
          for (int h = 0; h < 2; ++h) {
            if (!(okm && okn[jp][h])) continue;
            float* o = (float*)p.out0 + m * p.N + nn[jp][h];
#pragma unroll
            for (int r = 0; r < 4; ++r) unsafeAtomicAdd(o + r, v[h][r]);
          }
        } else if constexpr (EPI == VITSSL_EPI_F32) {
          store_f32_pair(rsOut0, i, jp, v[0], v[1], nn[jp]);
        } else if constexpr (E.resid) {
          if (tls) win.f32_of_lines(res[gb][ii][jp][0], res[gb][ii][jp][1]);
          if constexpr (EPI == EPI_RESID_ROWS || LS) {
            const float rs = rsc[gb][ii];
            const float cs = p.drop_on ? rs * p.dk.scale : rs;
#pragma unroll
            for (int h = 0; h < 2; ++h) {
              bool keep[4] = {true, true, true, true};
              if (p.drop_on) drop_keep4(p.dk, drop_words_a0(p.dk, a0row + (unsigned)i * a0rowstep + a0col[jp][h]), keep);
              float u[4];
#pragma unroll
              for (int r = 0; r < 4; ++r) {
                const float kv = keep[r] ? v[h][r] : 0.f;
                float sc = cs;
                if constexpr (LS) {
                  u[r] = p.drop_on ? kv * p.dk.scale : kv;
                  sc = cs * gam4[jp][h][r];
                }
                const float t = fmaf(kv, sc, res[gb][ii][jp][h][r]);
                v[h][r] = rs == 0.f ? res[gb][ii][jp][h][r] : t;
              }
              if constexpr (LS) out_a[jp][h] = u32x2{pack_bf2(u[0], u[1]), pack_bf2(u[2], u[3])};
            }
          } else {
#pragma unroll
            for (int h = 0; h < 2; ++h) {
              if (p.drop_on) {
                bool keep[4];
                drop_keep4(p.dk, drop_words_a0(p.dk, a0row + (unsigned)i * a0rowstep + a0col[jp][h]), keep);
#pragma unroll
                for (int r = 0; r < 4; ++r) v[h][r] = fmaf(keep[r] ? v[h][r] : 0.f, p.dk.scale, res[gb][ii][jp][h][r]);
              } else {
                v[h] += res[gb][ii][jp][h];
              }
            }
          }
          store_f32_pair(rsOut0, i, jp, v[0], v[1], nn[jp]);
        } else {
#pragma unroll
          for (int h = 0; h < 2; ++h) {
            if (!(okm && okn[jp][h])) continue;
            const long long img = m / p.embed.tokens;
            const int rin = (int)(m - img * p.embed.tokens);
            if (p.embed.mask && p.embed.mask[m]) v[h] = *(const f32x4*)(p.embed.mask_token + nn[jp][h]);
            v[h] += *(const f32x4*)(p.embed.pos + (long long)(p.embed.tok_offset + rin) * p.N + nn[jp][h]);
            const long long orow = img * p.embed.out_tokens + p.embed.tok_offset + rin;
            *(f32x4*)((float*)p.out0 + orow * p.N + nn[jp][h]) = v[h];
          }
        }
        if (CS && p.colsum) {
#pragma unroll
          for (int h = 0; h < 2; ++h)
            if (okm && okn[jp][h]) {
#pragma unroll
              for (int r = 0; r < 4; ++r) csum[2 * jp + h][r] += v[h][r];
            }
        }
      }
      if constexpr (E.windowed && E.out0_esz == 2) {
        if (!(Q8 && E.q8_of == 0) || p.out0) store_bf16_row(rsOut0, i, out_a, IC<EPI == VITSSL_EPI_GELU ? 2 : 0>{});
      }
      if constexpr (E.out1 == OUT1_REQUIRED) {
        if (!(Q8 && E.q8_of == 1) || p.out1) store_bf16_row(rsOut1, i, out_b, IC<0>{});
      }
      if constexpr (E.out1 == OUT1_OPTIONAL) {
        if (p.out1) store_bf16_row(rsOut1, i, out_a, IC<2>{});
      }
      if constexpr (Q8EPI) {
        if (q8) store_fp8_row(rsOut2, i, out_q);
      }
    }
  }

  if (CS && p.colsum) {
    f32x4 red[4];
#pragma unroll
    for (int j = 0; j < 4; ++j) {
#pragma unroll
      for (int r = 0; r < 4; ++r) {
        float s = csum[j][r];
        s += __shfl_xor(s, 1, 64);
        s += __shfl_xor(s, 2, 64);
        s += __shfl_xor(s, 4, 64);
        s += __shfl_xor(s, 8, 64);
        red[j][r] = s;
      }
    }
    if (tls) {
      if ((lane & 15) == 0) {
#pragma unroll
        for (int j = 0; j < 4; ++j) *(f32x4*)(xs + (16 * j + 4 * g4) * 4) = red[j];
      }
      asm volatile("" ::: "memory");
      const float v = *(const volatile float*)(xs + lane * 4);
      const int n = n0 + wn * 64 + lane;
      if (n < p.N) p.colsum[(m0 / CFG::WROWS + wm) * p.N + n] = v;
    } else {
#pragma unroll
      for (int j = 0; j < 4; ++j)
#pragma unroll
        for (int r = 0; r < 4; ++r) {
          const int n = n0 + wn * 64 + j * 16 + 4 * (lane >> 4) + r;
          if ((lane & 15) == 0 && n < p.N) p.colsum[(m0 / CFG::WROWS + wm) * p.N + n] = red[j][r];
        }
    }
  }
  if constexpr (Q8EPI) {
    if (p.qamax) {
      qmax = wave_max(qmax);
      unsigned* slot = (unsigned*)p.qamax;
      if (lane == 0 && __float_as_uint(qmax) > __builtin_nontemporal_load(slot)) atomicMax(slot, __float_as_uint(qmax));
    }
  }
// ... 4 lines not shown
```

### vit-ssl_amd/vit_core/ssl/simmim/model.py

```python
from typing import Optional

import torch
from torch import nn
from torch.autograd import Function

from ... import _runtime as R
from ..._runtime import BF16, F32, L, ops
from ...encoder_block import EncoderBlock, check_layer_scale_init
from .masking import draw_mask, mask_indices_np


class _SimMIMRuntime:

    def __init__(self, model: "SimMIMViT", device):
        self.model = model
        self.device = device
        C, H, W = model.input_shape
        self.P = model.patch_size
        self.C, self.H, self.W = C, H, W
        self.N = (H // self.P) * (W // self.P)
        self.geo = R.PatchGeometry(C, self.P)
        self.Pd, self.Pdp, self.Np = self.geo.Pd, self.geo.Pdp, self.geo.Np
        self.D = model.embed_dim
        self.store = R.FlatStore(model, device)
        st = self.store
        prefixes = [f"encoder_blocks.{i}." for i in range(len(model.encoder_blocks))]
        self.stack = R.EncoderStack(st, prefixes, self.D, model.num_heads, model.mlp_dim, model.dropout_p,
                                    drop_path=R.drop_path_rates(model.drop_path_rate, len(prefixes)),
                                    layer_scale=model.layer_scale_init is not None)
        self.ws = R.Workspace()
        self.geo.register_proj(st, "proj", lambda: st.view("projection.weight", (self.D, self.Pd)), self.D)
        self.head = R.PatchHead(st, self.geo, "head", "simmim_head.weight", "simmim_head.bias", self.D, self.ws)
        self.stage = R.HostStage()
        self.rec = None
        self.save_gen = 0

    def valid_for(self, device) -> bool:
        return device == self.device and self.store.is_attached()

    def embed(self, x, mask_d, tag=""):
        st, ws = self.store, self.ws
        B = x.shape[0]
        M = B * self.N
        patches = ws.get(tag + "patches", (M, self.Pdp), BF16, x.device)
        self.geo.patchify(x, patches)
        x0 = ws.get(tag + "x0", (M, self.D), F32, x.device)
        ops.gemm_nt(patches, st.w("proj"), x0, L.EPI_EMBED, bias=st.view("projection.bias"),
                    embed=(mask_d, st.view("mask_token") if mask_d is not None else None,
                           st.view("positional_embedding", (self.N, self.D)), self.N, self.N, 0))
        return x0, patches

    def prepare_mask(self, mask_cpu, dev):
        return tuple(self.stage.upload(mask_indices_np(mask_cpu.contiguous()), dev))

    def forward(self, x, training: bool, save: bool, mask_cpu=None, prepared=None):
        st, ws = self.store, self.ws
        if x.dim() != 4 or tuple(x.shape[1:]) != (self.C, self.H, self.W):
            raise L.VitsslError(f"SimMIMViT: expected input [B,{self.C},{self.H},{self.W}], got {tuple(x.shape)}")
        self.stack.check_tokens(self.N)
        x = R.as_f32(x)
        B = x.shape[0]
        M = B * self.N
        st.refresh_weights()
        dev = x.device
        if prepared is None:
            if mask_cpu is None:
                mask_cpu = draw_mask(B, self.N, self.model.mask_ratio)
            prepared = self.prepare_mask(mask_cpu, dev)
        seed = R.next_seed() if self.stack.needs_seed(training) else 0
        idx_d, inv_d, mask_d = prepared
        Mm = idx_d.numel()

        targets = torch.empty(Mm, self.Pd, dtype=F32, device=dev)
        if Mm == 0:
            if save:
                self.save_gen += 1
                self.rec = dict(B=B, M=M, Mm=0)
            return torch.empty(0, self.Pd, dtype=F32, device=dev), targets, mask_d.view(B, self.N, 1).bool()
        self.geo.gather_targets(x, idx_d, targets)
        tag = "" if save else "tmp."
        x0, patches = self.embed(x, mask_d, tag)
        xL, _ = self.stack.forward(x0, B, self.N, training, seed, save=save, slot="a")
        sel = ws.get(tag + "sel", (Mm, self.D), BF16, dev)
        ops.gather_rows_bf16(xL, idx_d, sel)
        pred = self.head.forward(sel)
        if save:
            self.save_gen += 1
            self.rec = dict(B=B, M=M, Mm=Mm, idx=idx_d, inv=inv_d, mask=mask_d, patches=patches, sel=sel)
        return pred, targets, mask_d.view(B, self.N, 1).bool()

    def backward(self, dpred_bf16, reducer=None):
        st, ws, rec = self.store, self.ws, self.rec
        B, M, Mm = rec["B"], rec["M"], rec["Mm"]
        if Mm == 0:
            if reducer is not None:
                reducer.ready(0, st.gflat.numel())
            return
        dev = dpred_bf16.device
        gv = st.gview
        self.head.wgrad(dpred_bf16, rec["sel"])
        dsel = ws.get("dsel", (Mm, self.D), BF16, dev)
        self.head.dgrad(dpred_bf16, dsel)
        g = ws.get("g", (M, self.D), F32, dev)
        ops.scatter_rows_f32(dsel, rec["inv"], g)
        if reducer is not None:
            reducer.ready(*st.span("simmim_head.weight", "simmim_head.bias"))
        g = self.stack.backward(g, slot="a", reducer=reducer)
        dproj = ws.get("dproj", (M, self.D), BF16, dev)
        ops.embed_bwd(g, rec["mask"], dproj, gv("positional_embedding", (self.N, self.D)), gv("mask_token"),
                      gv("projection.bias"), None, B, self.N, 0, self.D)
        self.geo.proj_wgrad(dproj, rec["patches"], gv("projection.weight", (self.D, self.Pd)), ws)
        if reducer is not None:
            reducer.ready(*st.span("mask_token", "positional_embedding"))
            reducer.ready(*st.span("projection.weight", "projection.bias"))


class _SimMIMFn(Function):
    @staticmethod
    def forward(ctx, rt, x, training, need, *params):
        pred, targets, mask = rt.forward(x, training, save=need)
        ctx.rt, ctx.gen = rt, rt.save_gen
        ctx.mark_non_differentiable(targets, mask)
        return pred, targets, mask

    @staticmethod
    def backward(ctx, dpred, _dt, _dm):
        rt = ctx.rt
        return (None, None, None, None, *R.backward_grads("SimMIMViT", ctx.gen, rt.save_gen, rt.store,
                                                          lambda: rt.backward(rt.geo.widen_grad(dpred))))


class SimMIMViT(nn.Module):
    def __init__(
        self,
        num_blocks: int,
        input_shape,
        embed_dim: int,
        patch_size: int,
        num_heads: int = 8,
        mlp_dim: int = 3072,
        dropout: float = 0.1,
        mask_ratio: float = 0.6,
        *,
        layer_scale_init: Optional[float] = None,
        drop_path_rate: float = 0.0,
    ):
        super().__init__()
        self.layer_scale_init = check_layer_scale_init(layer_scale_init)
        self.encoder_blocks = nn.ModuleList(
            [EncoderBlock(embed_dim, num_heads, mlp_dim, dropout, layer_scale_init=self.layer_scale_init) for _ in range(num_blocks)]
        )
        self.unfold = nn.Unfold(kernel_size=(patch_size, patch_size), stride=patch_size)
        self.projection = nn.Linear((input_shape[0] * patch_size * patch_size), embed_dim)
        self.mask_token = nn.Parameter(torch.randn(1, 1, embed_dim))
        self.positional_embedding = nn.Parameter(torch.rand(1, (input_shape[1] // patch_size) ** 2, embed_dim))
        self.simmim_head = nn.Linear(embed_dim, input_shape[0] * patch_size * patch_size)

        self.mask_ratio = mask_ratio
        self.input_shape = tuple(input_shape)
        self.embed_dim, self.patch_size = embed_dim, patch_size
        self.num_heads, self.mlp_dim, self.dropout_p = num_heads, mlp_dim, float(dropout)
        self.drop_path_rate = float(drop_path_rate)
        R.drop_path_rates(self.drop_path_rate, num_blocks)
        if input_shape[1] % patch_size != 0 or input_shape[2] % patch_size != 0:
            raise ValueError(
                f"Image dimensions H={input_shape[1]}, W={input_shape[2]} must be divisible by patch_size={patch_size}")
        self._rt = None

    def runtime(self, device=None) -> _SimMIMRuntime:
        return R.model_runtime(self, "SimMIMViT", _SimMIMRuntime, self.mask_token, device)

    def flat_store(self):
        return self.runtime().store

    def forward(self, x: torch.Tensor, return_bool_mask=False):
        R.require_gpu(x, "SimMIMViT")
        rt = self.runtime(x.device)
        need = torch.is_grad_enabled() and any(p.requires_grad for p in rt.store.params)
        pred, targets, mask = _SimMIMFn.apply(rt, x, self.training, need, *rt.store.params)
        if return_bool_mask:
            return pred, targets, mask
        return pred, targets

    @torch.no_grad()
    def inference_forward(self, x: torch.Tensor, return_patch_features=False):
        self.eval()
        R.require_gpu(x, "SimMIMViT")
        rt = self.runtime(x.device)
        rt.stack.check_tokens(rt.N)
        rt.store.refresh_weights()
        x = R.as_f32(x)
        B = x.shape[0]
        x0, _ = rt.embed(x, None, "inf.")
        xL, _ = rt.stack.forward(x0, B, rt.N, False, 0, save=False, slot="inf")
        feats = xL.view(B, rt.N, rt.D)
        return feats.clone() if return_patch_features else feats.mean(dim=1)

    def train_step(self, x: torch.Tensor, optimizer, reducer=None, mask_cpu=None, prepared=None) -> torch.Tensor:
        R.require_gpu(x, "SimMIMViT.train_step")
        rt = self.runtime(x.device)
        with R.fused_step(self, rt.store, optimizer, reducer) as apply:
            pred, targets, _ = rt.forward(x, True, save=True, mask_cpu=mask_cpu, prepared=prepared)
            n = pred.numel()
            loss_sum = rt.ws.get("loss_sum", (1,), F32, x.device)
            loss_sum.zero_()
            if n == 0:
                loss_sum.fill_(float("nan"))
                n = 1
                rt.backward(pred, reducer)
            else:
                dpb = rt.ws.get("dpred", (pred.shape[0], rt.Pdp), BF16, x.device)
                rt.geo.l1_loss(pred, targets, loss_sum, dpb, gscale=1.0 / n)
                rt.backward(dpb, reducer)
            apply()
            self.last_pred, self.last_targets = pred, targets
            return loss_sum[0] / n
```

### vit-ssl_amd/vitssl_hip/_lib.py

```python
import ctypes as C
import os
import re

_HERE = os.path.dirname(os.path.abspath(__file__))
LIB_PATH = os.environ.get("VITSSL_LIB") or os.path.join(_HERE, "libvitssl_hip.so")
_INCLUDE = os.path.normpath(os.path.join(_HERE, "..", "..", "include"))
HEADERS = {key: os.path.join(_INCLUDE, f"vitssl_{key}.h")
           for key in ("hip", "transforms", "metrics", "classify", "attention_hd", "patch", "optim", "mixup", "droppath", "layerscale",
                       "lamb", "bce")}
_INCLUDE_EXT = os.path.normpath(os.path.join(_HERE, "..", "..", "include_ext"))
EXT_HEADERS = {"mae": os.path.join(_INCLUDE_EXT, "vitssl_mae.h")}
_INCLUDE_ADDONS = os.path.normpath(os.path.join(_HERE, "..", "..", "include_addons"))
ADDON_HEADERS = {m.group(1): os.path.join(_INCLUDE_ADDONS, m.group(0))
                 for m in (re.fullmatch(r"vitssl_(\w+)\.h", f) for f in sorted(os.listdir(_INCLUDE_ADDONS))) if m}


class VitsslError(RuntimeError):
    pass


class Dropout(C.Structure):
    _fields_ = [("p", C.c_float), ("site", C.c_uint32), ("seed", C.c_uint64)]


# ... 157 lines not shown
        "vitssl_optim_table_build": [C.POINTER(OptimSegment), _i, _i64, _vp, _i64],
        "vitssl_grad_sumsq_workspace_bytes": _returns(_i64, _i),
        "vitssl_grad_sumsq": [_vp, _vp, _i, _vp, _vp, _i64, _vp],
        "vitssl_adamw_segments": [_vp, _vp, _vp, _vp, _vp, _i, _f, _f, _f, _f, _i, _f, _vp, _f, _vp],
    },
    "mixup": {
        "vitssl_mix_batch": [_vp, _vp, _vp, _vp, _i, _i, _i, _i, _vp],
        "vitssl_classify_loss_mix_workspace_floats": _returns(_i64, _i, _i),
        "vitssl_classify_loss_mix": [_vp, _vp, _vp, _vp, _i, _i, _i, _d, _i64, _f, _vp, _vp, _i, _vp, _vp, _vp, _vp, _vp, _i64, _vp],
    },
    "droppath": {
        "vitssl_droppath_table": [_vp, C.POINTER(C.c_float), C.POINTER(C.c_uint32), _i, _i, C.c_uint64, _vp],
        "vitssl_gemm_bf16_nt_rows": [_pGemm, _pRows, _vp],
        "vitssl_layernorm_bwd_rows": [_vp, _vp, _vp, _vp, _vp, _vp, _vp, _vp, _vp, _vp, _vp, Dropout, _pRows, _i64, _i, _vp, _i64, _vp],
        "vitssl_grad_mask_cast_rows": [_vp, _vp, _vp, Dropout, _pRows, _i64, _i, _vp, _i64, _vp],
    },
    "layerscale": {
        "vitssl_gemm_bf16_nt_ls": [_pGemm, _pCols, _pRows, _vp, _vp],
        "vitssl_layerscale_workspace_floats": _returns(_i64, _i64, _i),
        "vitssl_layernorm_bwd_ls": [_vp, _vp, _vp, _vp, _vp, _vp, _vp, _vp, _vp, _vp, _vp, Dropout, _pRows, _pCols, _vp, _vp, _i64, _i,
                                    _vp, _i64, _vp],
        "vitssl_grad_mask_cast_ls": [_vp, _vp, _vp, Dropout, _pRows, _pCols, _vp, _vp, _i64, _i, _vp, _i64, _vp],
    },
    "lamb": {
        "vitssl_lamb_workspace_bytes": _returns(_i64, C.POINTER(OptimSegment), _i),
        "vitssl_lamb_segments": [_vp, _vp, _vp, _vp, _vp, _i, _f, _f, _f, _f, _i, _f, _vp, _f, _i, _vp, _vp, _i64, _vp],
    },
    "bce": {
        "vitssl_classify_bce_workspace_floats": _returns(_i64, _i, _i),
        "vitssl_classify_bce": [_vp, _vp, _vp, _vp, _i, _i, _i, _d, _d, _i, _i64, _f, _vp, _vp, _i, _vp, _vp, _vp, _vp, _vp, _i64, _vp],
    },
}
REGISTRY = {key: {name: p if isinstance(p, tuple) else (C.c_int, p) for name, p in table.items()} for key, table in _ABI.items()}

_EXT_ABI = {
    "mae": {
        "vitssl_mae_tokens_fwd": [_vp, _vp, _vp, _vp, _vp, _i, _i, _i, _i, _vp],
        "vitssl_mae_tokens_bwd": [_vp, _vp, _vp, _vp, _i, _i, _i, _i, _vp, _i64, _vp],
        "vitssl_mae_unshuffle_fwd": [_vp, _vp, _vp, _vp, _vp, _i, _i, _i, _i, _vp],
        "vitssl_mae_unshuffle_bwd": [_vp, _vp, _vp, _vp, _vp, _i, _i, _i, _i, _vp, _i64, _vp],
        "vitssl_mae_loss": [_vp, _i64, _vp, _vp, _vp, _i64, _i, _i, _i, _f, _vp, _i64, _vp],
        "vitssl_mae_gather_rows_bf16": [_vp, _vp, _vp, _i64, _i, _vp],
        "vitssl_mae_gather_rows_f32": [_vp, _vp, _vp, _i64, _i, _vp],
        "vitssl_mae_scatter_rows_f32": [_vp, _vp, _vp, _i64, _i, _vp],
    },
}
EXT_REGISTRY = {key: {name: p if isinstance(p, tuple) else (C.c_int, p) for name, p in table.items()} for key, table in _EXT_ABI.items()}

_ADDON_ABI = {
    "pool": {
        "vitssl_pool_tokens_fwd": [_vp, _vp, _i, _i, _i, _vp],
        "vitssl_pool_tokens_bwd": [_vp, _vp, _i, _i, _i, _vp],
    },
}
ADDON_REGISTRY = {key: {name: p if isinstance(p, tuple) else (C.c_int, p) for name, p in _ADDON_ABI[key].items()} for key in ADDON_HEADERS}

DROPPATH_SITE_BIT = 0x80000000
DROPPATH_MAX_SITES = 128
LAMB_ALWAYS_ADAPT, LAMB_TRUST_CLIP = 1, 2

_lib = None


def header_path(key):
    for table in (HEADERS, EXT_HEADERS):
        if key in table:
            return table[key]
    return ADDON_HEADERS[key]


def header_text(key):
    with open(header_path(key)) as f:
        txt = re.sub(r"/\*.*?\*/", "", f.read(), flags=re.S)
    return re.sub(r"//.*$|^\s*#.*$", "", txt, flags=re.M)


def declarations(key="hip"):
    def ctype(s):
        return re.sub(r"\s*\*", "*", " ".join(s.split()))
    decls = {}
    for ret, name, params in re.findall(r"(?<=[;{}])\s*([A-Za-z_][\w\s*]*?)\b(vitssl_[a-z0-9_]+)\s*\(([^()]*)\)\s*;", header_text(key)):
        params = [] if params.strip() == "void" else [ctype(re.sub(r"\w+\s*$", "", p)) for p in params.split(",")]
        decls[name] = (ctype(ret), params)
    return decls


def header_symbols(key="hip"):
    return sorted(declarations(key))


def lib():
    global _lib
    if _lib is not None:
        return _lib
    if not os.path.exists(LIB_PATH):
        raise VitsslError(
            f"{LIB_PATH} not found: the HIP library is not built. Run `python __graft_entry__.py` "
            "(or __graft_entry__.build()). There is no CPU fallback for the vit_core hot path.")
    import torch
    l = C.CDLL(LIB_PATH)
    if l.vitssl_version() != ABI_VERSION:
        raise VitsslError(f"{LIB_PATH} implements C-ABI version {l.vitssl_version()}, these bindings expect {ABI_VERSION}: "
                          "rebuild it (python __graft_entry__.py)")
    for table in list(REGISTRY.values()) + list(EXT_REGISTRY.values()) + list(ADDON_REGISTRY.values()):
        for name, (restype, argtypes) in table.items():
            fn = getattr(l, name)
# ... 11 lines not shown
```

### vit-ssl_amd/vitssl_hip/engine.py

```python
from __future__ import annotations

import re
from typing import Callable, Dict, List, NamedTuple, Optional, Tuple

import numpy as np
import torch
from torch import nn

from . import _lib as L
from . import ops

BF16 = torch.bfloat16
F32 = torch.float32
FP8 = ops.FP8
ALIGN = 64
MAX_TOKENS = 2048
FP8_MAX_TOKENS = 256

import os as _os

_LINEAR_OPERANDS = _os.environ.get("VITSSL_LINEAR_OPERANDS", "bf16")


def set_linear_operands(kind: str):
# ... 542 lines not shown
                        raise L.VitsslError(f"LayerScale: {b + leaf!r} holds {store.offsets[b + leaf][1]} values, expected embed_dim = {D}")
        if self.fp8 and (D % 128 != 0 or F % 128 != 0):
            raise L.VitsslError(f"fp8 linear operands need embed_dim ({D}) and mlp_dim ({F}) to be multiples of 128")
        for b in self.bp:
            a = b + "self_attention."
            srcs = {
                "wqkv": lambda a=a, D=D: store.span_view(a + "w_query.weight", a + "w_value.weight", (3 * D, D)),
                "wo": lambda a=a: store.view(a + "final_linear.weight", (D, D)),
                "w1": lambda b=b: store.view(b + "feed_forward.linear_in.weight", (F, D)),
                "w2": lambda b=b: store.view(b + "feed_forward.linear_out.weight", (D, F)),
            }
            for leaf, src in srcs.items():
                if self.fp8:
                    store.register_fp8_weight(b + leaf, src)
                else:
                    store.register_weight(b + leaf, src)
        self._gs_by_slot: Dict[str, dict] = {}
        self._gs = None

    def _n(self, i, leaf):
        return self.bp[i] + leaf

    def block_span(self, i) -> Tuple[int, int]:
        return self._spans[i]

    def _drop(self, i, which, seed, training):
        if not training or self.p <= 0.0:
            return ops.NO_DROP
        return ops.make_dropout(self.p, seed, self.site_base + 3 * i + which)

    def needs_seed(self, training: bool) -> bool:
        return bool(training) and (self.p > 0.0 or self.drop_path is not None)

    def drop_path_sites(self) -> List[Tuple[float, int]]:
        return [(r, L.DROPPATH_SITE_BIT | ((self.site_base + 2 * i + br) & 0x7FFFFFFF)) for i, r in enumerate(self.drop_path or [])
                for br in (0, 1)]

    def drop_path_table(self, slot: str = "a") -> Optional[torch.Tensor]:
        return self._saved[slot].get("dp")

    def check_tokens(self, T: int):
        if self.fp8 and self.dh != 64:
            raise L.VitsslError(f"fp8 linear operands support head dim 64 only, got embed_dim / num_heads = {self.D} / {self.H} = "
                                f"{self.dh}: use bf16 operands (set_linear_operands('bf16') or VITSSL_LINEAR_OPERANDS=bf16), which "
                                f"cover {ops.HD_SUPPORTED}")
        ops.attn_family(self.dh)
        if self.fp8 and T > FP8_MAX_TOKENS:
            raise L.VitsslError(f"fp8 linear operands support sequences of up to {FP8_MAX_TOKENS} tokens, got {T}: use bf16 "
                                f"operands (set_linear_operands('bf16') or VITSSL_LINEAR_OPERANDS=bf16), which cover up to "
                                f"{MAX_TOKENS} tokens")
        if T > MAX_TOKENS:
            raise L.VitsslError(f"sequence length {T} > {MAX_TOKENS} unsupported by the attention kernels")

    def _scaled(self, dp, T, i, k, branch=None, dls=False):
        kw = {}
        if dp is not None and self.drop_path[i] > 0.0:
            kw["rows"] = (dp[2 * i + k - 1], T)
        if self.layer_scale:
            name = self._n(i, f"layer_scale{k}.gamma")
            kw["cols"] = self.store.view(name)
            if branch is not None:
                kw["branch"] = branch
            if dls:
                kw["dls"] = self.store.gview(name)
        return kw

    def _ln_fwd(self, x, i, leaf, y, mean, rstd):
        gamma, beta = self.store.view(self._n(i, leaf + ".weight")), self.store.view(self._n(i, leaf + ".bias"))
        if self.fp8:
            ops.layernorm_fwd_fp8(x, gamma, beta, None, y, mean, rstd)
        else:
            ops.layernorm_fwd(x, gamma, beta, y, mean, rstd)

    def _gemm(self, A, i, leaf, out, epilogue, dgrad=False, image=None, **kw):
        name = self._n(i, leaf)
        if self.fp8:
            w, alpha = (self.store.w8t if dgrad else self.store.w8)(name)
            ops.gemm_fp8_nt(A, w, out, epilogue, alpha=alpha, out_fp8=image, **kw)
        else:
            ops.gemm_nt(A, self.store.w(name + ".T" if dgrad else name), out, epilogue, out1=image, **kw)

    def _attn_fwd(self, qkv, att, att_op, lse, B, T, probs):
        if self.fp8:
            ops.attn_fwd(qkv, att, lse, B, T, self.H, self.dh, probs=probs, out_fp8=att_op)
        else:
            ops.attn_fwd_any(qkv, att, lse, B, T, self.H, self.dh, probs=probs)

    def _attn_bwd(self, s, dout, q, delta, B, T):
        if self.fp8:
            ops.attn_bwd(s["qkv"], s["att"], dout, s["lse"], q.x, delta, B, T, self.H, self.dh, dqkv_fp8=q.x8, scale=q.scale, amax=q.amax)
            self._settle(q)
        else:
            ops.attn_bwd_any(s["qkv"], s["att"], dout, s["lse"], q.x, delta, B, T, self.H, self.dh)

    def _dgrad(self, q, i, leaf, out, epilogue=L.EPI_BF16, emits=None, **kw):
        if self.fp8:
            kw["alpha2"] = q.inv
            if emits is not None:
                kw.update(image=emits.x8, out_scale=emits.scale, out_amax=emits.amax)
        self._gemm(q.x8 if self.fp8 else q.x, i, leaf, out, epilogue, dgrad=True, **kw)
        if self.fp8 and emits is not None:
            self._settle(emits)

    def _ln_bwd(self, ln, g, q, gm_colsum, drop, **scaled):
        f8 = (q.x8, q.scale, q.amax) if self.fp8 else ()
        if ln is None:
            (ops.grad_mask_cast_fp8 if self.fp8 else ops.grad_mask_cast)(g, q.x, *f8, gm_colsum, drop, **scaled)
        else:
            *head, i, leaf = ln
            w, b = self._n(i, leaf + ".weight"), self._n(i, leaf + ".bias")
            (ops.layernorm_bwd_fp8 if self.fp8 else ops.layernorm_bwd)(*head, self.store.view(w), g, g, q.x, *f8, self.store.gview(w),
                                                                       self.store.gview(b), gm_colsum, drop, **scaled)
        if self.fp8:
            self._settle(q)

    def forward(self, x: torch.Tensor, B: int, T: int, training: bool, seed: int, save: bool, slot: str = "a",
                return_attn: bool = False):
        st, D, H, F = self.store, self.D, self.H, self.F
        self.check_tokens(T)
        M = B * T
        dev = x.device
        g = self.ws.get
        probs = None
        rec = {"B": B, "T": T, "seed": seed, "training": training, "blocks": []}
        dp = None
        if training and self.drop_path is not None:
            dp = ops.droppath_table(self.drop_path_sites(), B, seed, g(f"{slot}.dp" if save else f"{slot}.tmp.dp", (2 * self.L, B), F32, dev))
        rec["dp"] = dp
        cur = x
        for i in range(self.L):
            tag = f"{slot}.{i}." if save else f"{slot}.tmp."
            img = lambda n, n8, cols: g(tag + (n8 if self.fp8 else n), (M, cols), FP8 if self.fp8 else BF16, dev)
            h1, h2, a = img("h1", "h1_8", D), img("h2", "h2_8", D), img("a", "a8", F)
            att = g(tag + "att", (M, D), BF16, dev)
            att_op = img("att", "att8", D) if self.fp8 else att
            ls1 = g(tag + "ls1", (M, D), BF16, dev) if self.layer_scale and save else None
            ls2 = g(tag + "ls2", (M, D), BF16, dev) if self.layer_scale and save else None
            mean1, rstd1 = g(tag + "mean1", (M,), F32, dev), g(tag + "rstd1", (M,), F32, dev)
            mean2, rstd2 = g(tag + "mean2", (M,), F32, dev), g(tag + "rstd2", (M,), F32, dev)
            qkv = g(tag + "qkv", (M, 3 * D), BF16, dev)
            lse = g(tag + "lse", (B, H, T), F32, dev)
            xmid = g(tag + "xmid", (M, D), F32, dev)
            u = g(tag + "u", (M, F), BF16, dev)
            xout = g(f"{slot}.{i}.xout" if save else f"{slot}.tmp.xout{i & 1}", (M, D), F32, dev)

            if return_attn and i == self.L - 1:
                probs = torch.empty(B, H, T, T, dtype=F32, device=dev)
            b1, b2 = st.view(self._n(i, "feed_forward.linear_in.bias")), st.view(self._n(i, "feed_forward.linear_out.bias"))
            self._ln_fwd(cur, i, "layer_norm1", h1, mean1, rstd1)
            self._gemm(h1, i, "wqkv", qkv, L.EPI_BF16)
            self._attn_fwd(qkv, att, att_op, lse, B, T, probs if i == self.L - 1 else None)
            self._gemm(att_op, i, "wo", xmid, L.EPI_RESID, aux=cur, drop=self._drop(i, 0, seed, training), **self._scaled(dp, T, i, 1, branch=ls1))
            self._ln_fwd(xmid, i, "layer_norm2", h2, mean2, rstd2)
            self._gemm(h2, i, "w1", u, L.EPI_GELU, bias=b1, image=a, drop=self._drop(i, 1, seed, training))
            self._gemm(a, i, "w2", xout, L.EPI_RESID, bias=b2, aux=xmid, drop=self._drop(i, 2, seed, training), **self._scaled(dp, T, i, 2, branch=ls2))
            if save:
                rec["blocks"].append(dict(xin=cur, h1=h1, mean1=mean1, rstd1=rstd1, qkv=qkv, att=att, att_op=att_op, lse=lse, xmid=xmid,
                                          h2=h2, mean2=mean2, rstd2=rstd2, u=u, a=a, ls1=ls1, ls2=ls2))
            cur = xout
        if save:
            self._saved[slot] = rec
        return cur, probs

    def backward(self, g: torch.Tensor, slot: str = "a", reducer: Optional[GradReducer] = None,
                 scale_key: Optional[str] = None, input_grad_only: bool = False) -> torch.Tensor:
        st, D, H, F = self.store, self.D, self.H, self.F
        rec = self._saved[slot]
        B, T, seed, training, dp = rec["B"], rec["T"], rec["seed"], rec["training"], rec.get("dp")
        M = B * T
        dev = g.device
        w = self.ws.get
        bw = f"bwd{M}."
        gv = st.gview
        last = self.L - 1
        wgrad = self.fp8 or not input_grad_only
        gs = self._grad_scale_state(dev, scale_key or slot) if self.fp8 else None
        jit = self.fp8 and not gs["valid"]
        kinds = (("gm", "gm8", D), ("du", "du8", F), ("gm2" if wgrad and not self.fp8 else "gm", "gm8b", D), ("dqkv", "dq8", 3 * D))
        x = [w(bw + n, (M, cols), BF16, dev) if not self.fp8 or jit else None for n, _, cols in kinds]
        x8 = [w(bw + n8, (M, cols), FP8, dev) if self.fp8 else None for _, n8, cols in kinds]
        dh_ = w(bw + "dh", (M, D), BF16, dev)
        delta = w(bw + "delta", (B, H, T), F32, dev)

        plain = [_GradOperand(t) for t in x]

        def grad(i, t):
            if not self.fp8:
                return plain[t]
            return _GradOperand(x[t], x8[t], gs["scale"][i, t:t + 1], gs["amax"][i, t:t + 1], gs["inv"][i, t:t + 1])

        def scaled(i, k):
            return self._scaled(dp, T, i, k, branch=rec["blocks"][i][f"ls{k}"] if wgrad else None, dls=wgrad)

        gm = grad(last, 0)
        self._ln_bwd(None, g, gm, gv(self._n(last, "feed_forward.linear_out.bias")), self._drop(last, 2, seed, training), **scaled(last, 2))
        for i in range(last, -1, -1):
            s = rec["blocks"][i]
            a_ = self.bp[i] + "self_attention."
            du, gm2, dqkv = grad(i, 1), grad(i, 2), grad(i, 3)
            self._dgrad(gm, i, "w2", du.x, L.EPI_DGELU, emits=du, aux=s["u"],
                        colsum=gv(self._n(i, "feed_forward.linear_in.bias")))
            self._dgrad(du, i, "w1", dh_)
            self._ln_bwd((dh_, s["xmid"], s["mean2"], s["rstd2"], i, "layer_norm2"), g, gm2, None, self._drop(i, 0, seed, training),
                         **scaled(i, 1))
            self._dgrad(gm2, i, "wo", dh_)
            self._attn_bwd(s, dh_, dqkv, delta, B, T)
            self._dgrad(dqkv, i, "wqkv", dh_)
            if wgrad:
                jobs = [(gm, s["a"], gv(self._n(i, "feed_forward.linear_out.weight"), (D, F))),
                        (du, s["h2"], gv(self._n(i, "feed_forward.linear_in.weight"), (F, D))),
                        (gm2, s["att_op"], gv(a_ + "final_linear.weight", (D, D))),
                        (dqkv, s["h1"], st.span_view(a_ + "w_query.weight", a_ + "w_value.weight", (3 * D, D), grad=True))]
                if self.fp8:
                    ops.gemm_fp8_tn_batch([(q.x8, act, dw, None, q.inv) for q, act, dw in jobs])
                else:
                    ops.gemm_tn_batch([(q.x, act, dw) for q, act, dw in jobs])
            ln1 = (dh_, s["xin"], s["mean1"], s["rstd1"])
            if i > 0:
                gm = grad(i - 1, 0)
                self._ln_bwd(ln1 + (i, "layer_norm1"), g, gm, gv(self._n(i - 1, "feed_forward.linear_out.bias")),
                             self._drop(i - 1, 2, seed, training), **scaled(i - 1, 2))
            else:
                ops.layernorm_bwd(*ln1, st.view(self._n(i, "layer_norm1.weight")), g, g, None,
                                  gv(self._n(i, "layer_norm1.weight")), gv(self._n(i, "layer_norm1.bias")), None, ops.NO_DROP)
            if reducer is not None and wgrad:
                lo, hi = self.block_span(i)
                reducer.ready(lo, hi)
        if self.fp8:
            gs["used"].copy_(gs["scale"])
            self._rescale(gs["scale"], gs["inv"], gs["amax"], margin=1)
            gs["amax"].zero_()
            gs["valid"] = True
        return g

    @staticmethod
    def _scale_from_amax(amax: torch.Tensor, margin: int) -> torch.Tensor:
        mant, e = torch.frexp(amax)
        k = (9 - e - (mant > 0.875).to(e.dtype) - margin).clamp(-120, 120)
        return torch.bitwise_left_shift(k.to(torch.int32) + 127, 23).view(torch.float32)

    def _grad_scale_state(self, dev, slot: str = "a"):
        gs = self._gs_by_slot.get(slot)
        if gs is None or gs["scale"].device != dev:
            mk = lambda v: torch.full((self.L, 4), v, dtype=F32, device=dev)
            gs = {"scale": mk(1.0), "inv": mk(1.0), "amax": mk(0.0), "used": mk(1.0), "valid": False}
            self._gs_by_slot[slot] = gs
        self._gs = gs
        return gs

    def _rescale(self, scale, inv, amax, margin: int):
        ok = (amax > 0) & torch.isfinite(amax)
        new = torch.where(ok, self._scale_from_amax(torch.where(ok, amax, torch.ones_like(amax)), margin), scale)
        scale.copy_(new)
        inv.copy_(1.0 / new)

    def _settle(self, q):
        if q.x is not None and q.x8 is not None:
            self._rescale(q.scale, q.inv, q.amax, margin=0)
            ops.quantize_fp8(q.x, q.x8, scale=q.scale)

    def fp8_grad_scales(self, slot: Optional[str] = None) -> torch.Tensor:
        gs = self._gs if slot is None else self._gs_by_slot[slot]
        return gs["used"].clone()

    def recalibrate_fp8(self):
        for gs in self._gs_by_slot.values():
            gs["valid"] = False
# ... 1 lines not shown
```

### vit-ssl_amd/vitssl_hip/ops.py

```python
import collections
import ctypes as C
import operator

import torch

from . import _lib as L
from ._lib import Dropout, Embed, Fp8Gemm, Gemm, call

BF16 = torch.bfloat16
F32 = torch.float32
FP8 = torch.float8_e4m3fn


def _stream():
    return C.c_void_p(torch.cuda.current_stream().cuda_stream)


def _chk(t, dtype, name, shape=None):
    if t is None:
        raise L.VitsslError(f"{name}: tensor is None")
    if not t.is_cuda:
        raise L.VitsslError(f"{name}: expected a CUDA (HIP) tensor, got {t.device}; there is no CPU fallback")
    if t.device.index != torch.cuda.current_device():
        raise L.VitsslError(f"{name}: tensor lives on {t.device} but the current device is cuda:{torch.cuda.current_device()}; "
# ... 45 lines not shown
def layernorm_fwd(x, gamma, beta, y, mean, rstd, eps=1e-5):
    rows, cols = x.shape
    ev = _prof_begin()
    call("vitssl_layernorm_fwd", _chk(x, F32, "x"), _chk(gamma, F32, "gamma", (cols,)), _chk(beta, F32, "beta", (cols,)),
         _chk(y, BF16, "y", (rows, cols)), _chk(mean, F32, "mean", (rows,)), _chk(rstd, F32, "rstd", (rows,)),
         rows, cols, float(eps), _stream())
    _prof_end(ev, "ln_fwd", 0.0, rows * (6 * cols + 8))


def layernorm_fwd_fp8(x, gamma, beta, y, y8, mean, rstd, eps=1e-5):
    rows, cols = x.shape
    ev = _prof_begin()
    call("vitssl_layernorm_fwd_fp8", _chk(x, F32, "x"), _chk(gamma, F32, "gamma", (cols,)), _chk(beta, F32, "beta", (cols,)),
         _opt(y, BF16, "y", (rows, cols)), _chk(y8, FP8, "y8", (rows, cols)), _chk(mean, F32, "mean", (rows,)),
         _chk(rstd, F32, "rstd", (rows,)), rows, cols, float(eps), _stream())
    _prof_end(ev, "ln_fwd", 0.0, rows * ((7 if y is not None else 5) * cols + 8))


def _scalar(t, name):
    if t is None:
        return C.c_void_p(0)
    if t.numel() != 1:
        raise L.VitsslError(f"{name}: expected a 1-element fp32 device tensor")
    return _chk(t, F32, name)


def quantize_fp8(x, y8, scale=None, amax=None):
    call("vitssl_quantize_fp8_scaled", _chk(x, BF16, "x"), _chk(y8, FP8, "y8", x.shape), x.numel(), _scalar(scale, "scale"),
         _scalar(amax, "amax"), _stream())


def droppath_table(pairs, B, seed, out):
    n = len(pairs)
    if not 1 <= n <= L.DROPPATH_MAX_SITES:
        raise L.VitsslError(f"droppath_table: {n} (rate, site) pairs outside [1, {L.DROPPATH_MAX_SITES}]")
    rates = (C.c_float * n)(*[float(r) for r, _ in pairs])
    sites = (C.c_uint32 * n)(*[int(s) & 0xFFFFFFFF for _, s in pairs])
    call("vitssl_droppath_table", _chk(out, F32, "scale", (n, B)), rates, sites, n, int(B), C.c_uint64(int(seed) & 0xFFFFFFFFFFFFFFFF),
         _stream())
    return out


def _rowscale(rows, M, name):
    scale, rpg = rows
    rpg = int(rpg)
    if rpg <= 0 or M % rpg != 0:
        raise L.VitsslError(f"{name}: rows_per_group {rpg} does not divide the {M} rows")
    r = L.RowScale()
    r.scale = _chk(scale, F32, name + " rows.scale", (M // rpg,))
    r.groups, r.rows_per_group = M // rpg, rpg
    return r


def _colscale(cols, N, name):
    c = L.ColScale()
    c.gamma = _chk(cols, F32, name + " cols(gamma)", (N,))
    c.cols = N
    return c


_LnForm = collections.namedtuple("_LnForm", "sfx query")
_LN_PLAIN = _LnForm("", "vitssl_sum_workspace_floats")
_LN_FP8 = _LnForm("_fp8", "vitssl_sum_workspace_floats")
_LN_ROWS = _LnForm("_rows", "vitssl_sum_workspace_floats")
_LN_LS = _LnForm("_ls", "vitssl_layerscale_workspace_floats")


def _ln_bwd(who, ln, g_res, gm, gm_colsum, drop, fp8=None, rows=None, cols=None, branch=None, dls=None):
    M, N = (ln[1] if ln else g_res).shape
    if cols is not None:
        if (branch is None) != (dls is None):
            raise L.VitsslError(f"{who}: branch= and dls= are given together (gamma's gradient) or both left out")
        form = _LN_LS
        extra = (C.byref(_rowscale(rows, M, who)) if rows is not None else None, C.byref(_colscale(cols, N, who)),
                 _opt(branch, BF16, who + " branch", (M, N)), _opt(dls, F32, who + " dls", (N,)))
    else:
        if branch is not None or dls is not None:
            raise L.VitsslError(f"{who}: branch= / dls= belong to cols= (LayerScale)")
        form = _LN_FP8 if fp8 else (_LN_PLAIN if rows is None else _LN_ROWS)
        extra = () if rows is None else (C.byref(_rowscale(rows, M, who)),)
    if ln:
        dy, x, mean, rstd, gamma, g_out, dgamma, dbeta = ln
        head = (_chk(dy, BF16, "dy", (M, N)), _chk(x, F32, "x"), _chk(mean, F32, "mean", (M,)), _chk(rstd, F32, "rstd", (M,)),
                _chk(gamma, F32, "gamma", (N,)), _opt(g_res, F32, "g_res", (M, N)), _chk(g_out, F32, "g_out", (M, N)))
    else:
        head = (_chk(g_res, F32, "g"),)
    gm_p = (_opt if fp8 or (ln and form is not _LN_LS) else _chk)(gm, BF16, "gm", (M, N))
    q8 = (_chk(fp8[0], FP8, "gm8", (M, N)), _scalar(fp8[1], "scale"), _scalar(fp8[2], "amax")) if fp8 else ()
    sums = (_chk(dgamma, F32, "dgamma", (N,)), _chk(dbeta, F32, "dbeta", (N,))) if ln else ()
    ws = _tn_workspace((ln[1] if ln else g_res).device, int(getattr(L.lib(), form.query)(M, N)))
    ev = _prof_begin() if ln else None
    call("vitssl_" + ("layernorm_bwd" if ln else "grad_mask_cast") + form.sfx, *head, gm_p, *q8, *sums,
         _opt(gm_colsum, F32, "gm_colsum", (N,)), drop, *extra, M, N, C.c_void_p(ws.data_ptr()), ws.numel(), _stream())
    _prof_end(ev, "ln_bwd", 0.0, M * (N * (2 + 4 + (4 if g_res is not None else 0) + 4 + (2 if gm is not None else 0) + (1 if fp8 else 0)
                                           + (2 if branch is not None else 0)) + 8))


def layernorm_bwd(dy, x, mean, rstd, gamma, g_res, g_out, gm, dgamma, dbeta, gm_colsum=None, drop=NO_DROP, rows=None, cols=None,
                  branch=None, dls=None):
    _ln_bwd("layernorm_bwd", (dy, x, mean, rstd, gamma, g_out, dgamma, dbeta), g_res, gm, gm_colsum, drop, rows=rows, cols=cols,
            branch=branch, dls=dls)


def layernorm_bwd_fp8(dy, x, mean, rstd, gamma, g_res, g_out, gm, gm8, scale, amax, dgamma, dbeta, gm_colsum=None, drop=NO_DROP):
    _ln_bwd("layernorm_bwd_fp8", (dy, x, mean, rstd, gamma, g_out, dgamma, dbeta), g_res, gm, gm_colsum, drop, fp8=(gm8, scale, amax))


def grad_mask_cast(g, gm, gm_colsum=None, drop=NO_DROP, rows=None, cols=None, branch=None, dls=None):
    _ln_bwd("grad_mask_cast", None, g, gm, gm_colsum, drop, rows=rows, cols=cols, branch=branch, dls=dls)


def grad_mask_cast_fp8(g, gm, gm8, scale, amax, gm_colsum=None, drop=NO_DROP):
    _ln_bwd("grad_mask_cast_fp8", None, g, gm, gm_colsum, drop, fp8=(gm8, scale, amax))


_OUT0_DTYPE = {L.EPI_BF16: BF16, L.EPI_F32: F32, L.EPI_GELU: BF16, L.EPI_RESID: F32, L.EPI_DGELU: BF16, L.EPI_EMBED: F32}


def _nt_desc(who, sfx, dtype, A, B, epilogue, bias, set_out0, aux, dgelu_aux, out1, colsum, drop, epilogues=None):
    M, K = A.shape
    N, K2 = B.shape
    if K != K2:
        raise L.VitsslError(f"{who}: K mismatch {K} vs {K2}")
    if epilogues is not None and epilogue not in epilogues:
        raise L.VitsslError(f"{who}: epilogue {epilogue} has no fp8-operand form")
    g = Gemm()
    g.A = _chk(A, dtype, "A" + sfx)
    g.B = _chk(B, dtype, "B" + sfx)
    g.M, g.N, g.K = M, N, K
    g.epilogue = epilogue
    g.bias = _opt(bias, F32, "bias", (N,))
    set_out0(g, M, N)
    if epilogue == L.EPI_RESID:
        g.aux = _chk(aux, F32, "aux(residual)", (M, N))
    elif epilogue == L.EPI_DGELU:
        g.aux = _chk(aux, BF16, dgelu_aux, (M, N))
    g.out1 = _opt(out1, BF16, "out1", (M, N))
    g.colsum = _opt(colsum, F32, "colsum", (N,))
    if colsum is not None:
        g.workspace, g.workspace_floats = _sum_ws(colsum.device, M, N)
    g.drop = drop
    return g, M, N, K


def gemm_nt(A, B, out0, epilogue, bias=None, aux=None, out1=None, colsum=None, drop=NO_DROP, embed=None, rows=None, cols=None,
            branch=None):
    def set_out0(g, M, N):
        if epilogue != L.EPI_EMBED:
            g.out0 = _chk(out0, _OUT0_DTYPE[epilogue], "out0", (M, N))
            return
        if embed is None:
            raise L.VitsslError("gemm_nt: EPI_EMBED needs embed=(mask, mask_token, pos, tokens, out_tokens, tok_offset)")
        mask, mask_token, pos, tokens, out_tokens, tok_offset = embed
        if M % tokens != 0:
            raise L.VitsslError("gemm_nt: M must be a multiple of tokens")
        e = Embed()
        e.mask = _opt(mask, torch.uint8, "mask", (M,))
        e.mask_token = _opt(mask_token, F32, "mask_token", (N,))
        e.pos = _chk(pos, F32, "pos", (out_tokens, N))
        e.tokens, e.out_tokens, e.tok_offset = tokens, out_tokens, tok_offset
        g.embed = e
        g.out0 = _chk(out0, F32, "out0", ((M // tokens) * out_tokens, N))

    g, M, N, K = _nt_desc("gemm_nt", "", BF16, A, B, epilogue, bias, set_out0, aux, "aux(u)", out1, colsum, drop)
    ev = _prof_begin()
    if cols is not None:
        if epilogue != L.EPI_RESID:
            raise L.VitsslError(f"gemm_nt: cols= belongs to EPI_RESID, got epilogue {epilogue}")
        call("vitssl_gemm_bf16_nt_ls", C.byref(g), C.byref(_colscale(cols, N, "gemm_nt")),
             C.byref(_rowscale(rows, M, "gemm_nt")) if rows is not None else None, _opt(branch, BF16, "branch", (M, N)), _stream())
    elif branch is not None:
        raise L.VitsslError("gemm_nt: branch= belongs to cols= (LayerScale)")
    elif rows is not None:
        if epilogue != L.EPI_RESID:
            raise L.VitsslError(f"gemm_nt: rows= belongs to EPI_RESID, got epilogue {epilogue}")
        call("vitssl_gemm_bf16_nt_rows", C.byref(g), C.byref(_rowscale(rows, M, "gemm_nt")), _stream())
    else:
        call("vitssl_gemm_bf16_nt", C.byref(g), _stream())
    _prof_end(ev, f"gemm_nt[epi{epilogue}] {M}x{N}x{K}", 2.0 * M * N * K)


def gemm_fp8_nt(A8, B8, out0, epilogue, alpha=None, bias=None, aux=None, out1=None, out_fp8=None, drop=NO_DROP,
                alpha2=None, colsum=None, out_scale=None, out_amax=None):
    def set_out0(g, M, N):
        if out0 is None and not (epilogue == L.EPI_DGELU and out_fp8 is not None):
            raise L.VitsslError("gemm_fp8_nt: out0 may only be omitted for EPI_DGELU with out_fp8")
        g.out0 = _opt(out0, _OUT0_DTYPE[epilogue], "out0", (M, N))

    g, M, N, K = _nt_desc("gemm_fp8_nt", "8", FP8, A8, B8, epilogue, bias, set_out0, aux, "aux(g')", out1, colsum, drop,
                          epilogues=(L.EPI_BF16, L.EPI_F32, L.EPI_GELU, L.EPI_RESID, L.EPI_DGELU))
    q = Fp8Gemm()
    q.alpha = _scalar(alpha, "alpha")
    q.alpha2 = _scalar(alpha2, "alpha2")
    q.out_fp8 = _opt(out_fp8, FP8, "out_fp8", (M, N))
    q.out_scale = _scalar(out_scale, "out_scale")
    q.out_amax = _scalar(out_amax, "out_amax")
    if out_fp8 is not None and epilogue not in (L.EPI_GELU, L.EPI_DGELU):
        raise L.VitsslError("gemm_fp8_nt: out_fp8 belongs to EPI_GELU / EPI_DGELU")
    ev = _prof_begin()
    call("vitssl_gemm_fp8_nt", C.byref(g), C.byref(q), _stream())
    _prof_end(ev, f"gemm_fp8_nt[epi{epilogue}] {M}x{N}x{K}", 2.0 * M * N * K)


_TN_WS = {}


def _tn_workspace(device, floats):
    key = (device, torch.cuda.current_stream().cuda_stream)
    ws = _TN_WS.get(key)
    if ws is None or ws.numel() < floats:
        ws = torch.empty(max(floats, 1 << 20), dtype=F32, device=device)
        _TN_WS[key] = ws
    return ws


def _sum_ws(device, rows, cols):
    ws = _tn_workspace(device, int(L.lib().vitssl_sum_workspace_floats(rows, cols)))
    return C.c_void_p(ws.data_ptr()), ws.numel()

# ... 106 lines not shown
    _prof_end(ev, f"attn_hd_fwd B{B} N{N} H{H} dh{dh}", 4.0 * B * H * N * N * dh)


def attn_hd_bwd(qkv, out, dout, lse, dqkv, delta_ws, B, N, H, dh):
    ev = _prof_begin()
    call("vitssl_attn_hd_bwd", _chk(qkv, BF16, "qkv", (B * N, 3 * H * dh)), _chk(out, BF16, "out", (B * N, H * dh)),
         _chk(dout, BF16, "dout", (B * N, H * dh)), _chk(lse, F32, "lse", (B, H, N)),
         _chk(dqkv, BF16, "dqkv", (B * N, 3 * H * dh)), _chk(delta_ws, F32, "delta_ws", (B, H, N)), B, N, H, dh, _stream())
    _prof_end(ev, f"attn_hd_bwd B{B} N{N} H{H} dh{dh}", 8.0 * B * H * N * N * dh)


def attn_family(dh):
    try:
        d = operator.index(dh)
    except TypeError:
        d = None
    if d == 64:
        return attn_fwd, attn_bwd
    if d is not None and HD_MIN <= d <= HD_MAX and d % HD_STEP == 0:
        return attn_hd_fwd, attn_hd_bwd
    raise L.VitsslError(f"head dim {dh} (embed_dim / num_heads) unsupported by the attention kernels: supported are {HD_SUPPORTED}")


def attn_fwd_any(qkv, out, lse, B, N, H, dh, probs=None):
    attn_family(dh)[0](qkv, out, lse, B, N, H, dh, probs=probs)


def attn_bwd_any(qkv, out, dout, lse, dqkv, delta_ws, B, N, H, dh):
    attn_family(dh)[1](qkv, out, dout, lse, dqkv, delta_ws, B, N, H, dh)


def patchify_bf16(img, patches, P):
    B, Cc, H, W = img.shape
    call("vitssl_patchify_bf16", _chk(img, F32, "img"), _chk(patches, BF16, "patches", (B * (H // P) * (W // P), Cc * P * P)),
         B, Cc, H, W, P, _stream())


def gather_patches_f32(img, idx, out, P):
    B, Cc, H, W = img.shape
    n = idx.numel()
    call("vitssl_gather_patches_f32", _chk(img, F32, "img"), _chk(idx, torch.int32, "idx"), _chk(out, F32, "out", (n, Cc * P * P)),
         n, Cc, H, W, P, _stream())


def gather_rows_bf16(x, idx, out):
    rows, cols = x.shape
    n = idx.numel()
    call("vitssl_gather_rows_bf16", _chk(x, F32, "x"), _chk(idx, torch.int32, "idx"), _chk(out, BF16, "out", (n, cols)), n, cols, _stream())


def scatter_rows_f32(src, inv, g):
    rows, cols = g.shape
    call("vitssl_scatter_rows_f32", _chk(src, BF16, "src"), _chk(inv, torch.int32, "inv", (rows,)), _chk(g, F32, "g"), rows, cols, _stream())


def gather_cls_f32(x, out, B, T, D):
    call("vitssl_gather_cls_f32", _chk(x, F32, "x", (B * T, D)), _chk(out, F32, "out", (B, D)), B, T, D, _stream())


def scatter_cls_f32(gcls, g, B, T, D):
    call("vitssl_scatter_cls_f32", _chk(gcls, F32, "gcls", (B, D)), _chk(g, F32, "g", (B * T, D)), B, T, D, _stream())


def pool_tokens_fwd(x, out, B, T, D):
    call("vitssl_pool_tokens_fwd", _chk(x, F32, "x", (B * T, D)), _chk(out, F32, "out", (B, D)), B, T, D, _stream())


def pool_tokens_bwd(dout, g, B, T, D):
    call("vitssl_pool_tokens_bwd", _chk(dout, F32, "dout", (B, D)), _chk(g, F32, "g", (B * T, D)), B, T, D, _stream())


def embed_bwd(dtok, mask, dproj, dpos, dmask_token, dbias, dcls, B, tokens, tok_offset, D):
    T_out = tokens + tok_offset
    wsn = int(L.lib().vitssl_embed_bwd_workspace_floats(B, tokens, tok_offset, D))
    ws = _tn_workspace(dtok.device, wsn)
    call("vitssl_embed_bwd", _chk(dtok, F32, "dtok", (B * T_out, D)), _opt(mask, torch.uint8, "mask", (B * tokens,)),
         _chk(dproj, BF16, "dproj", (B * tokens, D)), _opt(dpos, F32, "dpos", (T_out, D)),
         _opt(dmask_token, F32, "dmask_token", (D,)), _opt(dbias, F32, "dbias", (D,)), _opt(dcls, F32, "dcls", (D,)),
         B, tokens, tok_offset, D, C.c_void_p(ws.data_ptr()), ws.numel(), _stream())


def l1_loss(pred, target, loss_sum, dpred=None, gscale=0.0):
    n = pred.numel()
    call("vitssl_l1_loss", _chk(pred, F32, "pred"), _chk(target, F32, "target", pred.shape), _chk(loss_sum, F32, "loss_sum", (1,)),
         _opt(dpred, BF16, "dpred", pred.shape), float(gscale), n, *_sum_ws(pred.device, n, 1), _stream())


def cross_entropy(logits, labels, loss_sum, dlogits=None, gscale=0.0):
    B, Cn = logits.shape
    call("vitssl_cross_entropy", _chk(logits, F32, "logits"), _chk(labels, torch.int64, "labels", (B,)),
         _chk(loss_sum, F32, "loss_sum", (1,)), _opt(dlogits, BF16, "dlogits", (B, Cn)), float(gscale), B, Cn, _stream())


def colsum_bf16(x, out):
    rows, cols = x.shape
    call("vitssl_colsum_bf16", _chk(x, BF16, "x"), _chk(out, F32, "out", (cols,)), rows, cols, *_sum_ws(x.device, rows, cols), _stream())


def cast_bf16(src, dst):
    call("vitssl_cast_bf16", _chk(src, F32, "src"), _chk(dst, BF16, "dst", src.shape), src.numel(), _stream())


def cast_transpose_bf16(src, dst, dst_t):
    R, Cn = src.shape
    call("vitssl_cast_transpose_bf16", _chk(src, F32, "src"), _opt(dst, BF16, "dst", (R, Cn)), _opt(dst_t, BF16, "dst_t", (Cn, R)),
         R, Cn, _stream())
# ... 490 lines not shown
```

Before: 7974 images/s.

## Compute last encoder block's MLP only on rows the loss uses via row map

For the final encoder block, the MLP half (GELU GEMM, residual GEMM, LN backward and its dgrads) runs on a compacted subset of rows, the ones the SimMIM tail actually reads. Index-based gather and scatter kernels move rows in and out. A row map keeps the dropout masks keyed to the original full-row positions so the random stream matches the full computation. This avoids MLP forward and backward work on rows whose outputs never reach the loss, at the cost of extra gather/scatter kernels and new GEMM/LN epilogue variants.

```diff
diff --git a/include_addons/vitssl_rowmap.h b/include_addons/vitssl_rowmap.h
--- /dev/null
+++ b/include_addons/vitssl_rowmap.h
@@ -0,0 +1,31 @@
+#ifndef VITSSL_ROWMAP_H
+#define VITSSL_ROWMAP_H
+
+#include <stdint.h>
+
+#include "../include/vitssl_hip.h"
+
+#ifdef __cplusplus
+extern "C" {
+#endif
+
+int vitssl_gemm_bf16_nt_rowmap(const vitssl_gemm_t* g, const int32_t* rowmap, int64_t full_rows, void* stream);
+
+int vitssl_layernorm_bwd_rowmap(const void* dy_bf16, const float* x, const float* mean, const float* rstd, const float* gamma,
+                                const float* g_res, float* g_out, void* gm_bf16, float* dgamma, float* dbeta, float* gm_colsum,
+                                vitssl_dropout_t drop, const int32_t* rowmap, int64_t full_rows, int64_t rows, int cols,
+                                float* workspace, int64_t workspace_floats, void* stream);
+int vitssl_grad_mask_cast_rowmap(const float* g, void* gm_bf16, float* gm_colsum, vitssl_dropout_t drop, const int32_t* rowmap,
+                                 int64_t full_rows, int64_t rows, int cols, float* workspace, int64_t workspace_floats,
+                                 void* stream);
+
+int vitssl_rows_gather_bf16(const void* src_bf16, const int32_t* idx, void* out_bf16, int64_t n_idx, int cols, void* stream);
+int vitssl_rows_gather_f32(const float* src, const int32_t* idx, float* out, int64_t n_idx, int cols, void* stream);
+int vitssl_rows_scatter_bf16(const void* src_bf16, int64_t n_src, const int32_t* inv, void* out_bf16, int64_t rows, int cols,
+                             void* stream);
+int vitssl_rows_scatter_f32(const float* src, int64_t n_src, const int32_t* inv, float* out, int64_t rows, int cols, void* stream);
+
+#ifdef __cplusplus
+}
+#endif
+#endif
diff --git a/vit-ssl_amd/csrc/elementwise.hip b/vit-ssl_amd/csrc/elementwise.hip
--- a/vit-ssl_amd/csrc/elementwise.hip
+++ b/vit-ssl_amd/csrc/elementwise.hip
@@ -1,3 +1,4 @@
+#include "../../include_addons/vitssl_rowmap.h"
 #include "common.h"
 
 namespace {
@@ -72,6 +73,35 @@
     v = f32x4{bf_lo(w[0]), bf_hi(w[0]), bf_lo(w[1]), bf_hi(w[1])};
   }
   *(f32x4*)(g + r * cols + c) = v;
+}
+
+template <bool SCATTER>
+__global__ void rows_by_index_kernel(const u32x4* __restrict__ src, const int* __restrict__ idx, u32x4* __restrict__ out, long long rows,
+                                     int pieces) {
+  const long long t = (long long)blockIdx.x * blockDim.x + threadIdx.x;
+  if (t >= rows * pieces) return;
+  const long long r = t / pieces;
+  const int p = (int)(t - r * pieces);
+  const int i = idx[r];
+  u32x4 v = {0u, 0u, 0u, 0u};
+  if (!SCATTER || i >= 0) v = src[(long long)i * pieces + p];
+  out[r * pieces + p] = v;
+}
+
+template <bool SCATTER>
+int launch_rows_by_index(const char* who, const void* src, int64_t n_src, const int32_t* idx, void* out, int64_t rows, int cols, int esz,
+                         void* stream) {
+  const int per = 16 / esz;
+  VS_CHECK_ARG(rows >= 0 && rows < (1LL << 31) && cols > 0 && cols % per == 0, "%s: rows=%lld outside [0, 2^31) or cols=%d no positive multiple of %d",
+               who, (long long)rows, cols, per);
+  if (rows == 0) return VITSSL_OK;
+  VS_CHECK_ARG(idx && out && (src || (SCATTER && n_src == 0)), "%s: null pointer", who);
+  VS_CHECK_ARG(n_src >= 0 && n_src < (1LL << 31), "%s: n_src=%lld outside [0, 2^31)", who, (long long)n_src);
+  VS_CHECK_ARG((((uintptr_t)src | (uintptr_t)out) & 15) == 0, "%s: src / out must be 16-byte aligned", who);
+  hipLaunchKernelGGL((rows_by_index_kernel<SCATTER>), dim3(ew_grid(rows * (cols / per))), dim3(EW_THREADS), 0, (hipStream_t)stream,
+                     (const u32x4*)src, (const int*)idx, (u32x4*)out, (long long)rows, cols / per);
+  VS_CHECK_LAUNCH(who);
+  return VITSSL_OK;
 }
 
 __global__ void gather_cls_kernel(const float* __restrict__ x, float* __restrict__ out, int B, int T, int D) {
@@ -468,6 +498,23 @@
   return VITSSL_OK;
 }
 
+extern "C" int vitssl_rows_gather_bf16(const void* src_bf16, const int32_t* idx, void* out_bf16, int64_t n_idx, int cols, void* stream) {
+  return launch_rows_by_index<false>("rows_gather_bf16", src_bf16, 0, idx, out_bf16, n_idx, cols, 2, stream);
+}
+
+extern "C" int vitssl_rows_gather_f32(const float* src, const int32_t* idx, float* out, int64_t n_idx, int cols, void* stream) {
+  return launch_rows_by_index<false>("rows_gather_f32", src, 0, idx, out, n_idx, cols, 4, stream);
+}
+
+extern "C" int vitssl_rows_scatter_bf16(const void* src_bf16, int64_t n_src, const int32_t* inv, void* out_bf16, int64_t rows, int cols,
+                                        void* stream) {
+  return launch_rows_by_index<true>("rows_scatter_bf16", src_bf16, n_src, inv, out_bf16, rows, cols, 2, stream);
+}
+
+extern "C" int vitssl_rows_scatter_f32(const float* src, int64_t n_src, const int32_t* inv, float* out, int64_t rows, int cols, void* stream) {
+  return launch_rows_by_index<true>("rows_scatter_f32", src, n_src, inv, out, rows, cols, 4, stream);
+}
+
 extern "C" int vitssl_gather_cls_f32(const float* x, float* out, int B, int T, int D, void* stream) {
   VS_CHECK_ARG(x && out && B > 0 && T > 0 && D > 0 && D % 4 == 0, "gather_cls: bad args");
   hipLaunchKernelGGL(gather_cls_kernel, dim3(ew_grid((long long)B * (D / 4))), dim3(EW_THREADS), 0, (hipStream_t)stream, x, out, B, T, D);
diff --git a/vit-ssl_amd/csrc/gemm_nt.hip b/vit-ssl_amd/csrc/gemm_nt.hip
--- a/vit-ssl_amd/csrc/gemm_nt.hip
+++ b/vit-ssl_amd/csrc/gemm_nt.hip
@@ -184,7 +184,7 @@
   constexpr int BUF = CFG::BUF_BYTES;
   constexpr int DUMMY = 2 * BUF;
   constexpr unsigned OOBV = 0x80000000u;
-  constexpr bool USE_GLUT = EPI == VITSSL_EPI_GELU;
+  constexpr bool USE_GLUT = nt_is_gelu(EPI);
   constexpr int GLUT_BASE = 2 * BUF + 1024;
   constexpr int GLUT_IMM = USE_GLUT ? GLUT_BASE - (int)GLUT_LO8 : -1;
   static_assert(!USE_GLUT || (GLUT_IMM >= 0 && GLUT_IMM < 65536), "the table's offset must fit the ds_read immediate");
@@ -457,7 +457,7 @@
 
 template <int EPI, typename CFG, bool F8 = false>
 int launch_pp(NtParams p, hipStream_t s) {
-  constexpr int LDS = 2 * CFG::BUF_BYTES + 1024 + (EPI == VITSSL_EPI_GELU ? GLUT_BYTES : 0);
+  constexpr int LDS = 2 * CFG::BUF_BYTES + 1024 + (nt_is_gelu(EPI) ? GLUT_BYTES : 0);
   static VsOnce attr_done{false};
   if (int rc = ensure_lds(gemm_nt_pp_kernel<EPI, CFG, F8>, LDS, attr_done, "gemm_nt")) return rc;
   const long long ntiles = (long long)p.tiles_m * p.tiles_n;
@@ -608,8 +608,8 @@
 }
 
 static int gemm_nt_entry(const vitssl_gemm_t* g, int esz, const vitssl_fp8_gemm_t* q, void* stream, const vitssl_rowscale_t* rows = nullptr,
-                         const vitssl_colscale_t* cols = nullptr, void* branch = nullptr) {
-  const char* who = cols ? "gemm_nt_ls" : rows ? "gemm_nt_rows" : esz == 1 ? "gemm_fp8_nt" : "gemm_nt";
+                         const vitssl_colscale_t* cols = nullptr, void* branch = nullptr, const int32_t* rowmap = nullptr, int64_t full_rows = 0) {
+  const char* who = rowmap ? "gemm_nt_rowmap" : cols ? "gemm_nt_ls" : rows ? "gemm_nt_rows" : esz == 1 ? "gemm_fp8_nt" : "gemm_nt";
   VS_CHECK_ARG(g && g->A && g->B && (g->out0 || (esz == 1 && caller_epi(g->epilogue).q8_of == 0 && q && q->out_fp8)), "%s: null operand", who);
   VS_CHECK_ARG(g->M > 0 && g->N > 0 && g->K > 0, "%s: empty problem M=%lld N=%d K=%d", who, (long long)g->M, g->N, g->K);
   VS_CHECK_ARG(g->K % (128 / esz) == 0, "%s: K=%d must be a multiple of %d", who, g->K, 128 / esz);
@@ -654,6 +654,23 @@
     p.colscale = cols->gamma;
     p.out1 = branch;
     return launch_nt<EPI_RESID_LS>(p, s);
+  }
+  if (rowmap) {
+    VS_CHECK_ARG(g->epilogue == VITSSL_EPI_GELU || g->epilogue == VITSSL_EPI_RESID,
+                 "%s: a row map is built for VITSSL_EPI_GELU and VITSSL_EPI_RESID only, got epilogue %d", who, g->epilogue);
+    VS_CHECK_ARG(full_rows >= g->M && full_rows < (1ll << 31), "%s: full_rows (%lld) must be at least M (%lld) and below 2^31", who,
+                 (long long)full_rows, (long long)g->M);
+    VS_CHECK_ARG(!p.drop_on || (unsigned long long)full_rows * (unsigned long long)g->N < (1ull << 34),
+                 "%s: dropout over %lld x %d elements: the stream's group counter is 32 bits (full_rows * N < 2^34)", who, (long long)full_rows, g->N);
+    if (p.drop_on) {
+      p.rowmap = rowmap;
+      if (g->epilogue == VITSSL_EPI_GELU) {
+        VS_CHECK_ARG(g->out1, "%s: EPI_GELU needs out1", who);
+        return launch_nt<EPI_GELU_MAP>(p, s);
+      }
+      VS_CHECK_ARG(g->aux, "%s: EPI_RESID needs aux (residual)", who);
+      return launch_nt<EPI_RESID_MAP>(p, s);
+    }
   }
   switch (g->epilogue) {
     case VITSSL_EPI_BF16: return launch_nt<VITSSL_EPI_BF16>(p, s);
@@ -691,6 +708,11 @@
   return gemm_nt_entry(g, 2, nullptr, stream, rows, cols, branch_bf16);
 }
 
+extern "C" int vitssl_gemm_bf16_nt_rowmap(const vitssl_gemm_t* g, const int32_t* rowmap, int64_t full_rows, void* stream) {
+  VS_CHECK_ARG(rowmap, "gemm_nt_rowmap: null row map (vitssl_gemm_bf16_nt is the launch without one)");
+  return gemm_nt_entry(g, 2, nullptr, stream, nullptr, nullptr, nullptr, rowmap, full_rows);
+}
+
 extern "C" int vitssl_gemm_fp8_nt(const vitssl_gemm_t* g, const vitssl_fp8_gemm_t* q, void* stream) {
   VS_CHECK_ARG(g && caller_epi(g->epilogue).fp8, "gemm_fp8_nt: fp8 operands are built for the BF16 / F32 / GELU / RESID / DGELU epilogues");
   VS_CHECK_ARG(!(q && q->out_fp8) || caller_epi(g->epilogue).q8_of >= 0, "gemm_fp8_nt: out_fp8 belongs to EPI_GELU / EPI_DGELU");
diff --git a/vit-ssl_amd/csrc/layernorm.hip b/vit-ssl_amd/csrc/layernorm.hip
--- a/vit-ssl_amd/csrc/layernorm.hip
+++ b/vit-ssl_amd/csrc/layernorm.hip
@@ -1,5 +1,6 @@
 #include "../../include/vitssl_droppath.h"
 #include "../../include/vitssl_layerscale.h"
+#include "../../include_addons/vitssl_rowmap.h"
 #include "common.h"
 
 namespace {
@@ -89,10 +90,16 @@
   float* dls;
 };
 __device__ __forceinline__ const LnLsArgs& ln_first(const LnLsArgs& a) { return a; }
+struct LnMapArgs {
+  const int* rowmap;
+};
+__device__ __forceinline__ const LnMapArgs& ln_first(const LnMapArgs& a) { return a; }
+template <typename T, typename... A>
+constexpr bool ln_pack_has = (std::is_same<T, A>::value || ...);
 constexpr int ln_bwd_ls_blocks(int V, bool has_ln) { return has_ln && V == 4 ? 1 : ln_bwd_blocks(V, has_ln, true); }
 
 template <int V, bool HAS_LN, bool HAS_CS, bool Q8 = false, bool PAIR = false, bool ROWS = false, typename... LSARGS>
-__global__ __launch_bounds__(LN_THREADS, sizeof...(LSARGS) ? ln_bwd_ls_blocks(V, HAS_LN) : ln_bwd_blocks(V, HAS_LN, HAS_CS || (ROWS && PAIR))) void ln_bwd_kernel(const bf16_t* __restrict__ dy, const float* __restrict__ x,
+__global__ __launch_bounds__(LN_THREADS, ((ln_pack_has<LnLsArgs, LSARGS...>) ? ln_bwd_ls_blocks(V, HAS_LN) : ln_bwd_blocks(V, HAS_LN, HAS_CS || (ROWS && PAIR)))) void ln_bwd_kernel(const bf16_t* __restrict__ dy, const float* __restrict__ x,
                                                             const float* __restrict__ mean, const float* __restrict__ rstd,
                                                             const float* __restrict__ gamma, const float* g_res,
                                                             float* g_out, bf16_t* __restrict__ gm, float* __restrict__ dgamma,
@@ -102,7 +109,11 @@
                                                             const float* __restrict__ qscale = nullptr, float* qamax = nullptr,
                                                             const float* __restrict__ rowscale = nullptr, unsigned rows_per_group = 1,
                                                             LSARGS... lsargs) {
-  constexpr bool LS = sizeof...(LSARGS) > 0;
+  constexpr bool LS = ln_pack_has<LnLsArgs, LSARGS...>;
+  constexpr bool MAP = ln_pack_has<LnMapArgs, LSARGS...>;
+  static_assert(!MAP || !(LS || ROWS || PAIR || Q8), "the row map is built on the plain bf16 form");
+  const int* __restrict__ rowmap = nullptr;
+  if constexpr (MAP) rowmap = ln_first(lsargs...).rowmap;
   const float* __restrict__ lsgamma = nullptr;
   const bf16_t* __restrict__ branch = nullptr;
   float* __restrict__ dls = nullptr;
@@ -144,8 +155,12 @@
   u32x2 nbr[V];
   float nmu = 0.f, nrs = 0.f, nmuB = 0.f, nrsB = 0.f;
   float nsc = 1.f, nscB = 1.f;
+  unsigned nmap = 0;
   auto fetch = [&](long long row) {
     if (!HAS_LN || row >= rows) return;
+    if constexpr (MAP) {
+      if (drop_on) nmap = (unsigned)rowmap[row];
+    }
     if constexpr (ROWS && !LS) {
       nsc = rowscale[(PAIR ? 2u * (unsigned)row : (unsigned)row) / rows_per_group];
       if constexpr (PAIR) nscB = rowscale[(2u * (unsigned)row + 1u) / rows_per_group];
@@ -184,6 +199,11 @@
     f32x4 dx[V];
     u32x2 brp[V];
     float sc = 1.f, scB = 1.f;
+    unsigned drow = 0;
+    if constexpr (MAP) {
+      if (HAS_LN) drow = nmap;
+      else if (drop_on) drow = (unsigned)rowmap[__builtin_amdgcn_readfirstlane((unsigned)row)];
+    }
     if constexpr (ROWS && !HAS_LN && !LS) sc = rowscale[__builtin_amdgcn_readfirstlane((unsigned)row / rows_per_group)];
     if constexpr (LS && !HAS_LN) {
       if (rowscale) sc = rowscale[__builtin_amdgcn_readfirstlane((unsigned)row / rows_per_group)];
@@ -261,7 +281,7 @@
           f32x4 o = dx[v];
           if (drop_on) {
             bool keep[4];
-            drop_keep4(dk, drop_words(dk, (unsigned)row * (unsigned)c4n + (unsigned)c4), keep);
+            drop_keep4(dk, drop_words(dk, (MAP ? drow : (unsigned)row) * (unsigned)c4n + (unsigned)c4), keep);
 #pragma unroll
             for (int r = 0; r < 4; ++r) o[r] = keep[r] ? o[r] * dk.scale : 0.f;
           }
@@ -358,19 +378,25 @@
   const float* lsgamma;
   const void* branch;
   float* dls;
+  const int32_t* rowmap;
+  int64_t full_rows;
 };
 
-template <bool HAS_LN, bool Q8 = false, bool ROWS = false, bool LS = false>
+template <bool HAS_LN, bool Q8 = false, bool ROWS = false, bool LS = false, bool MAP = false>
 int launch_ln_bwd(const LnBwdCall& c) {
   static_assert(!Q8 || !ROWS, "row scales are built for the bf16 image");
   static_assert(!LS || ROWS, "LayerScale is built on the form with row scales");
+  static_assert(!MAP || !(Q8 || ROWS || LS), "the row map is built on the plain bf16 form");
   const int64_t rows = c.rows;
   const int cols = c.cols;
   DropKey dk = make_drop_key(c.drop);
   const int on = dk.thr != 0;
-  VS_CHECK_ARG(!on || (unsigned long long)rows * (unsigned long long)cols < (1ull << 34),
+  VS_CHECK_ARG(!on || (unsigned long long)(MAP ? c.full_rows : rows) * (unsigned long long)cols < (1ull << 34),
                "%s: the dropout stream's group counter is 32 bits (rows * cols < 2^34)", c.who);
-  constexpr bool CAN_PAIR = HAS_LN && !Q8;
+  if constexpr (MAP) {
+    if (!on) return launch_ln_bwd<HAS_LN>(c);
+  }
+  constexpr bool CAN_PAIR = HAS_LN && !Q8 && !MAP;
   const bool pair = CAN_PAIR && cols == 384 && (rows & 1) == 0;
   const long long krows = pair ? rows / 2 : rows;
   const int kcols = pair ? 768 : cols;
@@ -405,6 +431,8 @@
     if constexpr (LS)
       hipLaunchKernelGGL((ln_bwd_kernel<V, HAS_LN, CS, Q8, PAIR, ROWS, LnLsArgs>), VS_LN_BWD_ARGS,
                          LnLsArgs{c.lsgamma, (const bf16_t*)c.branch, slot[3]});
+    else if constexpr (MAP)
+      hipLaunchKernelGGL((ln_bwd_kernel<V, HAS_LN, CS, Q8, PAIR, ROWS, LnMapArgs>), VS_LN_BWD_ARGS, LnMapArgs{(const int*)c.rowmap});
     else
       hipLaunchKernelGGL((ln_bwd_kernel<V, HAS_LN, CS, Q8, PAIR, ROWS>), VS_LN_BWD_ARGS);
   };
@@ -560,3 +588,32 @@
                                                   nullptr, gm_colsum, drop, rows, cols, workspace, workspace_floats, (hipStream_t)stream,
                                                   nullptr, nullptr, nullptr, rowscale, colscale->gamma, branch_bf16, dls});
 }
+
+static int check_rowmap(const char* who, const int32_t* rowmap, int64_t full_rows, int64_t rows, int cols) {
+  VS_CHECK_ARG(rows > 0 && cols > 0 && cols % 4 == 0 && cols <= 2048, "%s: cols=%d must be a multiple of 4 and <= 2048", who, cols);
+  VS_CHECK_ARG(rowmap, "%s: null row map", who);
+  VS_CHECK_ARG(full_rows >= rows && full_rows < (1ll << 31), "%s: full_rows (%lld) must be at least rows (%lld) and below 2^31", who,
+               (long long)full_rows, (long long)rows);
+  return VITSSL_OK;
+}
+
+extern "C" int vitssl_layernorm_bwd_rowmap(const void* dy_bf16, const float* x, const float* mean, const float* rstd, const float* gamma,
+                                           const float* g_res, float* g_out, void* gm_bf16, float* dgamma, float* dbeta, float* gm_colsum,
+                                           vitssl_dropout_t drop, const int32_t* rowmap, int64_t full_rows, int64_t rows, int cols,
+                                           float* workspace, int64_t workspace_floats, void* stream) {
+  VS_CHECK_ARG(dy_bf16 && x && mean && rstd && gamma && g_out && dgamma && dbeta && gm_bf16, "layernorm_bwd_rowmap: null pointer");
+  if (int rc = check_rowmap("layernorm_bwd_rowmap", rowmap, full_rows, rows, cols)) return rc;
+  return launch_ln_bwd<true, false, false, false, true>({LN_BWD_WHO, dy_bf16, x, mean, rstd, gamma, g_res, g_out, gm_bf16, dgamma, dbeta,
+                                                         gm_colsum, drop, rows, cols, workspace, workspace_floats, (hipStream_t)stream, nullptr,
+                                                         nullptr, nullptr, nullptr, nullptr, nullptr, nullptr, rowmap, full_rows});
+}
+
+extern "C" int vitssl_grad_mask_cast_rowmap(const float* g, void* gm_bf16, float* gm_colsum, vitssl_dropout_t drop, const int32_t* rowmap,
+                                            int64_t full_rows, int64_t rows, int cols, float* workspace, int64_t workspace_floats,
+                                            void* stream) {
+  VS_CHECK_ARG(g && gm_bf16, "grad_mask_cast_rowmap: null pointer");
+  if (int rc = check_rowmap("grad_mask_cast_rowmap", rowmap, full_rows, rows, cols)) return rc;
+  return launch_ln_bwd<false, false, false, false, true>({LN_BWD_WHO, nullptr, nullptr, nullptr, nullptr, nullptr, g, nullptr, gm_bf16, nullptr,
+                                                          nullptr, gm_colsum, drop, rows, cols, workspace, workspace_floats, (hipStream_t)stream,
+                                                          nullptr, nullptr, nullptr, nullptr, nullptr, nullptr, nullptr, rowmap, full_rows});
+}
diff --git a/vit-ssl_amd/csrc/nt_epilogue.h b/vit-ssl_amd/csrc/nt_epilogue.h
--- a/vit-ssl_amd/csrc/nt_epilogue.h
+++ b/vit-ssl_amd/csrc/nt_epilogue.h
@@ -1,6 +1,7 @@
 #pragma once
 #include "../../include/vitssl_droppath.h"
 #include "../../include/vitssl_layerscale.h"
+#include "../../include_addons/vitssl_rowmap.h"
 #include "common.h"
 
 namespace {
@@ -30,7 +31,10 @@
   const float* alpha2;
   const float* qscale;
   float* qamax;
-  const float* rowscale;
+  union {
+    const float* rowscale;
+    const int* rowmap;
+  };
   unsigned rows_per_group;
   const float* colscale;
 #ifdef VITSSL_NT_STAMPS
@@ -41,6 +45,9 @@
 constexpr int EPI_F32_SPLITK = 100;
 constexpr int EPI_RESID_ROWS = 101;
 constexpr int EPI_RESID_LS = 102;
+constexpr int EPI_GELU_MAP = 103;
+constexpr int EPI_RESID_MAP = 104;
+constexpr bool nt_is_gelu(int epi) { return epi == VITSSL_EPI_GELU || epi == EPI_GELU_MAP; }
 
 enum NtOut1 { OUT1_NONE, OUT1_REQUIRED, OUT1_OPTIONAL };
 struct NtEpiFacts {
@@ -53,6 +60,7 @@
   bool drops, resid;
   int stagger_bit;
   float epi_us;
+  bool rowmap = false;
 };
 constexpr NtEpiFacts nt_epi(int epi) {
   switch (epi) {
@@ -65,6 +73,8 @@
     case EPI_F32_SPLITK:   return NtEpiFacts{4, false, OUT1_NONE,     0, false, false, -1, false, false, -1,               4.f};
     case EPI_RESID_ROWS:   return NtEpiFacts{4, true,  OUT1_NONE,     4, false, false, -1, true,  true,  VITSSL_EPI_RESID, 8.f};
     case EPI_RESID_LS:     return NtEpiFacts{4, true,  OUT1_OPTIONAL, 4, false, false, -1, true,  true,  VITSSL_EPI_RESID, 8.f};
+    case EPI_GELU_MAP:     return NtEpiFacts{2, true,  OUT1_REQUIRED, 0, false, false, -1, true,  false, VITSSL_EPI_GELU,  7.f, true};
+    case EPI_RESID_MAP:    return NtEpiFacts{4, true,  OUT1_NONE,     4, false, false, -1, true,  true,  VITSSL_EPI_RESID, 8.f, true};
     default:               return NtEpiFacts{0, false, OUT1_NONE,     0, false, false, -1, false, false, -1,               0.f};
   }
 }
@@ -95,7 +105,8 @@
 constexpr bool nt_counts_are_as_written() {
   return nt_counts_are<VITSSL_EPI_BF16, MI>(2, 2, 8) && nt_counts_are<VITSSL_EPI_GELU, MI>(4, 3, 16) && nt_counts_are<VITSSL_EPI_DGELU, MI>(4, 3, 8) &&
          nt_counts_are<VITSSL_EPI_F32, MI>(4, 4, 16) && nt_counts_are<VITSSL_EPI_RESID, MI>(8, 8, 8) && nt_counts_are<EPI_RESID_ROWS, MI>(8, 8, 8) &&
-         nt_counts_are<EPI_RESID_LS, MI>(8, 8, 8) && nt_counts_are<VITSSL_EPI_EMBED, MI>(0, 0, 0) && nt_counts_are<EPI_F32_SPLITK, MI>(0, 0, 0);
+         nt_counts_are<EPI_RESID_LS, MI>(8, 8, 8) && nt_counts_are<VITSSL_EPI_EMBED, MI>(0, 0, 0) && nt_counts_are<EPI_F32_SPLITK, MI>(0, 0, 0) &&
+         nt_counts_are<EPI_GELU_MAP, MI>(4, 3, 16) && nt_counts_are<EPI_RESID_MAP, MI>(8, 8, 8);
 }
 static_assert(nt_counts_are_as_written<6>() && nt_counts_are_as_written<7>() && nt_counts_are_as_written<8>(), "epilogue vmem counts");
 
@@ -170,7 +181,7 @@
   constexpr bool LS = EPI == EPI_RESID_LS;
   int lane = lane_in;
   if (TLS) asm volatile("" : "+v"(lane));
-  constexpr bool GLUT = EPI == VITSSL_EPI_GELU && GLUT_OFF >= 0;
+  constexpr bool GLUT = nt_is_gelu(EPI) && GLUT_OFF >= 0;
   const bool glut_on = GLUT && (!Q8 || (p.out1 == nullptr && p.qamax == nullptr));
   constexpr bool CS = E.colsum, DROPS = E.drops;
   float csum[4][4];
@@ -297,6 +308,16 @@
   unsigned a0row = 0;
   if (DROPS && p.drop_on)
     a0row = drop_a0(p.dk, (unsigned)(m0 + wm * CFG::WROWS + (lane & 15)) * (unsigned)(p.N >> 2));
+  unsigned a0map[E.rowmap ? MI : 1];
+  if constexpr (E.rowmap) {
+    if (p.drop_on) {
+#pragma unroll
+      for (int i = 0; i < MI; ++i) {
+        const long long mr = m0 + wm * CFG::WROWS + i * 16 + (lane & 15);
+        a0map[i] = drop_a0(p.dk, (unsigned)p.rowmap[mr < p.M ? mr : 0] * (unsigned)(p.N >> 2));
+      }
+    }
+  }
   const float gelu_hs = (DROPS && p.drop_on) ? 0.5f * p.dk.scale : 0.5f;
   const float gelu_cs = (DROPS && p.drop_on) ? 0.3989422804014327f * p.dk.scale : 0.3989422804014327f;
 #pragma unroll
@@ -438,14 +459,14 @@
         if constexpr (EPI == VITSSL_EPI_BF16) {
           out_a[jp][0] = u32x2{pack_bf2(v[0][0], v[0][1]), pack_bf2(v[0][2], v[0][3])};
           out_a[jp][1] = u32x2{pack_bf2(v[1][0], v[1][1]), pack_bf2(v[1][2], v[1][3])};
-        } else if constexpr (EPI == VITSSL_EPI_GELU) {
+        } else if constexpr (nt_is_gelu(EPI)) {
           unsigned km[2][2] = {{0xffffffffu, 0xffffffffu}, {0xffffffffu, 0xffffffffu}};
           u32x2 dw[2] = {u32x2{0u, 0u}, u32x2{0u, 0u}};
           const bool dropping = p.drop_on;
           if (dropping) {
 #pragma unroll
             for (int h = 0; h < 2; ++h) {
-              dw[h] = drop_words_a0(p.dk, a0row + (unsigned)i * a0rowstep + a0col[jp][h]);
+              dw[h] = drop_words_a0(p.dk, (E.rowmap ? a0map[E.rowmap ? i : 0] : a0row + (unsigned)i * a0rowstep) + a0col[jp][h]);
               km[h][0] = drop_keep_pair(p.dk, dw[h][0]);
               km[h][1] = drop_keep_pair(p.dk, dw[h][1]);
             }
@@ -515,7 +536,7 @@
 #pragma unroll
             for (int h = 0; h < 2; ++h) {
               bool keep[4] = {true, true, true, true};
-              if (p.drop_on) drop_keep4(p.dk, drop_words_a0(p.dk, a0row + (unsigned)i * a0rowstep + a0col[jp][h]), keep);
+              if (p.drop_on) drop_keep4(p.dk, drop_words_a0(p.dk, (E.rowmap ? a0map[E.rowmap ? i : 0] : a0row + (unsigned)i * a0rowstep) + a0col[jp][h]), keep);
               float u[4];
 #pragma unroll
               for (int r = 0; r < 4; ++r) {
@@ -535,7 +556,7 @@
             for (int h = 0; h < 2; ++h) {
               if (p.drop_on) {
                 bool keep[4];
-                drop_keep4(p.dk, drop_words_a0(p.dk, a0row + (unsigned)i * a0rowstep + a0col[jp][h]), keep);
+                drop_keep4(p.dk, drop_words_a0(p.dk, (E.rowmap ? a0map[E.rowmap ? i : 0] : a0row + (unsigned)i * a0rowstep) + a0col[jp][h]), keep);
 #pragma unroll
                 for (int r = 0; r < 4; ++r) v[h][r] = fmaf(keep[r] ? v[h][r] : 0.f, p.dk.scale, res[gb][ii][jp][h][r]);
               } else {
@@ -566,7 +587,7 @@
         }
       }
       if constexpr (E.windowed && E.out0_esz == 2) {
-        if (!(Q8 && E.q8_of == 0) || p.out0) store_bf16_row(rsOut0, i, out_a, IC<EPI == VITSSL_EPI_GELU ? 2 : 0>{});
+        if (!(Q8 && E.q8_of == 0) || p.out0) store_bf16_row(rsOut0, i, out_a, IC<nt_is_gelu(EPI) ? 2 : 0>{});
       }
       if constexpr (E.out1 == OUT1_REQUIRED) {
         if (!(Q8 && E.q8_of == 1) || p.out1) store_bf16_row(rsOut1, i, out_b, IC<0>{});
diff --git a/vit-ssl_amd/vit_core/ssl/simmim/model.py b/vit-ssl_amd/vit_core/ssl/simmim/model.py
--- a/vit-ssl_amd/vit_core/ssl/simmim/model.py
+++ b/vit-ssl_amd/vit_core/ssl/simmim/model.py
@@ -1,3 +1,4 @@
+import os
 from typing import Optional
 
 import torch
@@ -8,6 +9,9 @@
 from ..._runtime import BF16, F32, L, ops
 from ...encoder_block import EncoderBlock, check_layer_scale_init
 from .masking import draw_mask, mask_indices_np
+
+
+_TAIL_ROWS = int(os.environ.get("VITSSL_SIMMIM_TAIL_ROWS", "0"))
 
 
 class _SimMIMRuntime:
@@ -33,6 +37,7 @@
         self.head = R.PatchHead(st, self.geo, "head", "simmim_head.weight", "simmim_head.bias", self.D, self.ws)
         self.stage = R.HostStage()
         self.rec = None
+        self._ident = None
         self.save_gen = 0
 
     def valid_for(self, device) -> bool:
@@ -53,7 +58,7 @@
     def prepare_mask(self, mask_cpu, dev):
         return tuple(self.stage.upload(mask_indices_np(mask_cpu.contiguous()), dev))
 
-    def forward(self, x, training: bool, save: bool, mask_cpu=None, prepared=None):
+    def forward(self, x, training: bool, save: bool, mask_cpu=None, prepared=None, tail_rows: bool = False):
         st, ws = self.store, self.ws
         if x.dim() != 4 or tuple(x.shape[1:]) != (self.C, self.H, self.W):
             raise L.VitsslError(f"SimMIMViT: expected input [B,{self.C},{self.H},{self.W}], got {tuple(x.shape)}")
@@ -80,13 +85,18 @@
         self.geo.gather_targets(x, idx_d, targets)
         tag = "" if save else "tmp."
         x0, patches = self.embed(x, mask_d, tag)
-        xL, _ = self.stack.forward(x0, B, self.N, training, seed, save=save, slot="a")
         sel = ws.get(tag + "sel", (Mm, self.D), BF16, dev)
-        ops.gather_rows_bf16(xL, idx_d, sel)
+        tail = tail_rows and bool(_TAIL_ROWS) and save and training and self.stack.supports_tail_rows()
+        if tail:
+            xc, _ = self.stack.forward(x0, B, self.N, training, seed, save=save, slot="a", tail_rows=(idx_d, inv_d))
+            ops.cast_bf16(xc, sel)
+        else:
+            xL, _ = self.stack.forward(x0, B, self.N, training, seed, save=save, slot="a")
+            ops.gather_rows_bf16(xL, idx_d, sel)
         pred = self.head.forward(sel)
         if save:
             self.save_gen += 1
-            self.rec = dict(B=B, M=M, Mm=Mm, idx=idx_d, inv=inv_d, mask=mask_d, patches=patches, sel=sel)
+            self.rec = dict(B=B, M=M, Mm=Mm, idx=idx_d, inv=inv_d, mask=mask_d, patches=patches, sel=sel, tail=tail)
         return pred, targets, mask_d.view(B, self.N, 1).bool()
 
     def backward(self, dpred_bf16, reducer=None):
@@ -101,8 +111,15 @@
         self.head.wgrad(dpred_bf16, rec["sel"])
         dsel = ws.get("dsel", (Mm, self.D), BF16, dev)
         self.head.dgrad(dpred_bf16, dsel)
-        g = ws.get("g", (M, self.D), F32, dev)
-        ops.scatter_rows_f32(dsel, rec["inv"], g)
+        if rec["tail"]:
+            ident = self._ident
+            if ident is None or ident.numel() != Mm or ident.device != dev:
+                ident = self._ident = torch.arange(Mm, dtype=torch.int32, device=dev)
+            g = ws.get("g_c", (Mm, self.D), F32, dev)
+            ops.scatter_rows_f32(dsel, ident, g)
+        else:
+            g = ws.get("g", (M, self.D), F32, dev)
+            ops.scatter_rows_f32(dsel, rec["inv"], g)
         if reducer is not None:
             reducer.ready(*st.span("simmim_head.weight", "simmim_head.bias"))
         g = self.stack.backward(g, slot="a", reducer=reducer)
@@ -200,7 +217,7 @@
         R.require_gpu(x, "SimMIMViT.train_step")
         rt = self.runtime(x.device)
         with R.fused_step(self, rt.store, optimizer, reducer) as apply:
-            pred, targets, _ = rt.forward(x, True, save=True, mask_cpu=mask_cpu, prepared=prepared)
+            pred, targets, _ = rt.forward(x, True, save=True, mask_cpu=mask_cpu, prepared=prepared, tail_rows=True)
             n = pred.numel()
             loss_sum = rt.ws.get("loss_sum", (1,), F32, x.device)
             loss_sum.zero_()
diff --git a/vit-ssl_amd/vitssl_hip/_lib.py b/vit-ssl_amd/vitssl_hip/_lib.py
--- a/vit-ssl_amd/vitssl_hip/_lib.py
+++ b/vit-ssl_amd/vitssl_hip/_lib.py
@@ -233,6 +233,15 @@
         "vitssl_pool_tokens_fwd": [_vp, _vp, _i, _i, _i, _vp],
         "vitssl_pool_tokens_bwd": [_vp, _vp, _i, _i, _i, _vp],
     },
+    "rowmap": {
+        "vitssl_gemm_bf16_nt_rowmap": [_pGemm, _vp, _i64, _vp],
+        "vitssl_layernorm_bwd_rowmap": [_vp, _vp, _vp, _vp, _vp, _vp, _vp, _vp, _vp, _vp, _vp, Dropout, _vp, _i64, _i64, _i, _vp, _i64, _vp],
+        "vitssl_grad_mask_cast_rowmap": [_vp, _vp, _vp, Dropout, _vp, _i64, _i64, _i, _vp, _i64, _vp],
+        "vitssl_rows_gather_bf16": [_vp, _vp, _vp, _i64, _i, _vp],
+        "vitssl_rows_gather_f32": [_vp, _vp, _vp, _i64, _i, _vp],
+        "vitssl_rows_scatter_bf16": [_vp, _i64, _vp, _vp, _i64, _i, _vp],
+        "vitssl_rows_scatter_f32": [_vp, _i64, _vp, _vp, _i64, _i, _vp],
+    },
 }
 ADDON_REGISTRY = {key: {name: p if isinstance(p, tuple) else (C.c_int, p) for name, p in _ADDON_ABI[key].items()} for key in ADDON_HEADERS}
 
diff --git a/vit-ssl_amd/vitssl_hip/engine.py b/vit-ssl_amd/vitssl_hip/engine.py
--- a/vit-ssl_amd/vitssl_hip/engine.py
+++ b/vit-ssl_amd/vitssl_hip/engine.py
@@ -618,6 +618,9 @@
         if T > MAX_TOKENS:
             raise L.VitsslError(f"sequence length {T} > {MAX_TOKENS} unsupported by the attention kernels")
 
+    def supports_tail_rows(self) -> bool:
+        return not (self.fp8 or self.drop_path is not None or self.layer_scale or self.D == 384)
+
     def _scaled(self, dp, T, i, k, branch=None, dls=False):
         kw = {}
         if dp is not None and self.drop_path[i] > 0.0:
@@ -681,10 +684,17 @@
             self._settle(q)
 
     def forward(self, x: torch.Tensor, B: int, T: int, training: bool, seed: int, save: bool, slot: str = "a",
-                return_attn: bool = False):
+                return_attn: bool = False, tail_rows: Optional[Tuple[torch.Tensor, torch.Tensor]] = None):
         st, D, H, F = self.store, self.D, self.H, self.F
         self.check_tokens(T)
         M = B * T
+        if tail_rows is not None:
+            if not (save and training):
+                raise L.VitsslError("tail_rows belongs to a saving training pass")
+            if not self.supports_tail_rows():
+                raise L.VitsslError("tail_rows is built for bf16 linear operands without drop path and LayerScale: pass full rows")
+            if tail_rows[0].numel() == 0 or tuple(tail_rows[1].shape) != (M,):
+                raise L.VitsslError(f"tail_rows: idx must name at least one row and inv hold {M} entries")
         dev = x.device
         g = self.ws.get
         probs = None
@@ -696,19 +706,21 @@
         cur = x
         for i in range(self.L):
             tag = f"{slot}.{i}." if save else f"{slot}.tmp."
-            img = lambda n, n8, cols: g(tag + (n8 if self.fp8 else n), (M, cols), FP8 if self.fp8 else BF16, dev)
-            h1, h2, a = img("h1", "h1_8", D), img("h2", "h2_8", D), img("a", "a8", F)
+            tail = tail_rows if i == self.L - 1 else None
+            Mr, c = (tail[0].numel(), "_c") if tail is not None else (M, "")
+            img = lambda n, n8, cols, rows=M: g(tag + (n8 if self.fp8 else n), (rows, cols), FP8 if self.fp8 else BF16, dev)
+            h1, h2, a = img("h1", "h1_8", D), img("h2" + c, "h2_8", D, Mr), img("a" + c, "a8", F, Mr)
             att = g(tag + "att", (M, D), BF16, dev)
             att_op = img("att", "att8", D) if self.fp8 else att
             ls1 = g(tag + "ls1", (M, D), BF16, dev) if self.layer_scale and save else None
             ls2 = g(tag + "ls2", (M, D), BF16, dev) if self.layer_scale and save else None
             mean1, rstd1 = g(tag + "mean1", (M,), F32, dev), g(tag + "rstd1", (M,), F32, dev)
-            mean2, rstd2 = g(tag + "mean2", (M,), F32, dev), g(tag + "rstd2", (M,), F32, dev)
+            mean2, rstd2 = g(tag + "mean2" + c, (Mr,), F32, dev), g(tag + "rstd2" + c, (Mr,), F32, dev)
             qkv = g(tag + "qkv", (M, 3 * D), BF16, dev)
             lse = g(tag + "lse", (B, H, T), F32, dev)
-            xmid = g(tag + "xmid", (M, D), F32, dev)
-            u = g(tag + "u", (M, F), BF16, dev)
-            xout = g(f"{slot}.{i}.xout" if save else f"{slot}.tmp.xout{i & 1}", (M, D), F32, dev)
+            xmid = g(tag + "xmid" + c, (Mr, D), F32, dev)
+            u = g(tag + "u" + c, (Mr, F), BF16, dev)
+            xout = g(f"{slot}.{i}.xout{c}" if save else f"{slot}.tmp.xout{i & 1}", (Mr, D), F32, dev)
 
             if return_attn and i == self.L - 1:
                 probs = torch.empty(B, H, T, T, dtype=F32, device=dev)
@@ -716,13 +728,19 @@
             self._ln_fwd(cur, i, "layer_norm1", h1, mean1, rstd1)
             self._gemm(h1, i, "wqkv", qkv, L.EPI_BF16)
             self._attn_fwd(qkv, att, att_op, lse, B, T, probs if i == self.L - 1 else None)
-            self._gemm(att_op, i, "wo", xmid, L.EPI_RESID, aux=cur, drop=self._drop(i, 0, seed, training), **self._scaled(dp, T, i, 1, branch=ls1))
+            xin, rm = cur, {}
+            if tail is not None:
+                att_op, xin_c = g(tag + "att_c", (Mr, D), BF16, dev), g(tag + "xin_c", (Mr, D), F32, dev)
+                ops.rows_gather_bf16(att, tail[0], att_op)
+                ops.rows_gather_f32(cur, tail[0], xin_c)
+                cur, rm = xin_c, {"rowmap": (tail[0], M)}
+            self._gemm(att_op, i, "wo", xmid, L.EPI_RESID, aux=cur, drop=self._drop(i, 0, seed, training), **rm, **self._scaled(dp, T, i, 1, branch=ls1))
             self._ln_fwd(xmid, i, "layer_norm2", h2, mean2, rstd2)
-            self._gemm(h2, i, "w1", u, L.EPI_GELU, bias=b1, image=a, drop=self._drop(i, 1, seed, training))
-            self._gemm(a, i, "w2", xout, L.EPI_RESID, bias=b2, aux=xmid, drop=self._drop(i, 2, seed, training), **self._scaled(dp, T, i, 2, branch=ls2))
+            self._gemm(h2, i, "w1", u, L.EPI_GELU, bias=b1, image=a, drop=self._drop(i, 1, seed, training), **rm)
+            self._gemm(a, i, "w2", xout, L.EPI_RESID, bias=b2, aux=xmid, drop=self._drop(i, 2, seed, training), **rm, **self._scaled(dp, T, i, 2, branch=ls2))
             if save:
-                rec["blocks"].append(dict(xin=cur, h1=h1, mean1=mean1, rstd1=rstd1, qkv=qkv, att=att, att_op=att_op, lse=lse, xmid=xmid,
-                                          h2=h2, mean2=mean2, rstd2=rstd2, u=u, a=a, ls1=ls1, ls2=ls2))
+                rec["blocks"].append(dict(xin=xin, h1=h1, mean1=mean1, rstd1=rstd1, qkv=qkv, att=att, att_op=att_op, lse=lse, xmid=xmid,
+                                          h2=h2, mean2=mean2, rstd2=rstd2, u=u, a=a, ls1=ls1, ls2=ls2, tail=tail))
             cur = xout
         if save:
             self._saved[slot] = rec
@@ -758,18 +776,39 @@
         def scaled(i, k):
             return self._scaled(dp, T, i, k, branch=rec["blocks"][i][f"ls{k}"] if wgrad else None, dls=wgrad)
 
-        gm = grad(last, 0)
-        self._ln_bwd(None, g, gm, gv(self._n(last, "feed_forward.linear_out.bias")), self._drop(last, 2, seed, training), **scaled(last, 2))
+        tail = rec["blocks"][last].get("tail")
+        if tail is None:
+            gm = grad(last, 0)
+            self._ln_bwd(None, g, gm, gv(self._n(last, "feed_forward.linear_out.bias")), self._drop(last, 2, seed, training), **scaled(last, 2))
+        else:
+            idx, inv = tail
+            Mc = idx.numel()
+            rm = {"rowmap": (idx, M)}
+            bc = f"bwd{Mc}c."
+            gm, du_c, gm2_c = (_GradOperand(w(bc + n, (Mc, cols), BF16, dev)) for n, cols in (("gm", D), ("du", F), ("gm2", D)))
+            dh_c = w(bc + "dh", (Mc, D), BF16, dev)
+            self._ln_bwd(None, g, gm, gv(self._n(last, "feed_forward.linear_out.bias")), self._drop(last, 2, seed, training), **rm)
         for i in range(last, -1, -1):
             s = rec["blocks"][i]
             a_ = self.bp[i] + "self_attention."
             du, gm2, dqkv = grad(i, 1), grad(i, 2), grad(i, 3)
-            self._dgrad(gm, i, "w2", du.x, L.EPI_DGELU, emits=du, aux=s["u"],
-                        colsum=gv(self._n(i, "feed_forward.linear_in.bias")))
-            self._dgrad(du, i, "w1", dh_)
-            self._ln_bwd((dh_, s["xmid"], s["mean2"], s["rstd2"], i, "layer_norm2"), g, gm2, None, self._drop(i, 0, seed, training),
-                         **scaled(i, 1))
-            self._dgrad(gm2, i, "wo", dh_)
+            if i == last and tail is not None:
+                du, gm2 = du_c, gm2_c
+                self._dgrad(gm, i, "w2", du.x, L.EPI_DGELU, emits=du, aux=s["u"], colsum=gv(self._n(i, "feed_forward.linear_in.bias")))
+                self._dgrad(du, i, "w1", dh_c)
+                self._ln_bwd((dh_c, s["xmid"], s["mean2"], s["rstd2"], i, "layer_norm2"), g, gm2, None, self._drop(i, 0, seed, training), **rm)
+                self._dgrad(gm2, i, "wo", dh_c)
+                ops.rows_scatter_bf16(dh_c, inv, dh_)
+                gfull = w(bw + "gfull", (M, D), F32, dev)
+                ops.rows_scatter_f32(g, inv, gfull)
+                g = gfull
+            else:
+                self._dgrad(gm, i, "w2", du.x, L.EPI_DGELU, emits=du, aux=s["u"],
+                            colsum=gv(self._n(i, "feed_forward.linear_in.bias")))
+                self._dgrad(du, i, "w1", dh_)
+                self._ln_bwd((dh_, s["xmid"], s["mean2"], s["rstd2"], i, "layer_norm2"), g, gm2, None, self._drop(i, 0, seed, training),
+                             **scaled(i, 1))
+                self._dgrad(gm2, i, "wo", dh_)
             self._attn_bwd(s, dh_, dqkv, delta, B, T)
             self._dgrad(dqkv, i, "wqkv", dh_)
             if wgrad:
@@ -779,6 +818,9 @@
                         (dqkv, s["h1"], st.span_view(a_ + "w_query.weight", a_ + "w_value.weight", (3 * D, D), grad=True))]
                 if self.fp8:
                     ops.gemm_fp8_tn_batch([(q.x8, act, dw, None, q.inv) for q, act, dw in jobs])
+                elif i == last and tail is not None:
+                    ops.gemm_tn_batch([(q.x, act, dw) for q, act, dw in jobs[:3]])
+                    ops.gemm_tn_batch([(q.x, act, dw) for q, act, dw in jobs[3:]])
                 else:
                     ops.gemm_tn_batch([(q.x, act, dw) for q, act, dw in jobs])
             ln1 = (dh_, s["xin"], s["mean1"], s["rstd1"])
diff --git a/vit-ssl_amd/vitssl_hip/ops.py b/vit-ssl_amd/vitssl_hip/ops.py
--- a/vit-ssl_amd/vitssl_hip/ops.py
+++ b/vit-ssl_amd/vitssl_hip/ops.py
@@ -121,6 +121,14 @@
     return r
 
 
+def _rowmap(rowmap, M, name):
+    rmap, full = rowmap
+    full = int(full)
+    if full < M:
+        raise L.VitsslError(f"{name}: the row map names {full} full rows for {M} compact ones")
+    return _chk(rmap, torch.int32, name + " rowmap", (M,)), full
+
+
 def _colscale(cols, N, name):
     c = L.ColScale()
     c.gamma = _chk(cols, F32, name + " cols(gamma)", (N,))
@@ -133,11 +141,19 @@
 _LN_FP8 = _LnForm("_fp8", "vitssl_sum_workspace_floats")
 _LN_ROWS = _LnForm("_rows", "vitssl_sum_workspace_floats")
 _LN_LS = _LnForm("_ls", "vitssl_layerscale_workspace_floats")
-
-
-def _ln_bwd(who, ln, g_res, gm, gm_colsum, drop, fp8=None, rows=None, cols=None, branch=None, dls=None):
+_LN_MAP = _LnForm("_rowmap", "vitssl_sum_workspace_floats")
+
+
+def _ln_bwd(who, ln, g_res, gm, gm_colsum, drop, fp8=None, rows=None, cols=None, branch=None, dls=None, rowmap=None):
     M, N = (ln[1] if ln else g_res).shape
-    if cols is not None:
+    if rowmap is not None and M == 0:
+        return
+    if rowmap is not None:
+        if fp8 or rows is not None or cols is not None or branch is not None or dls is not None:
+            raise L.VitsslError(f"{who}: rowmap= is built on the plain bf16 form (no fp8=, rows=, cols=)")
+        form = _LN_MAP
+        extra = _rowmap(rowmap, M, who)
+    elif cols is not None:
         if (branch is None) != (dls is None):
             raise L.VitsslError(f"{who}: branch= and dls= are given together (gamma's gradient) or both left out")
         form = _LN_LS
@@ -154,7 +170,7 @@
                 _chk(gamma, F32, "gamma", (N,)), _opt(g_res, F32, "g_res", (M, N)), _chk(g_out, F32, "g_out", (M, N)))
     else:
         head = (_chk(g_res, F32, "g"),)
-    gm_p = (_opt if fp8 or (ln and form is not _LN_LS) else _chk)(gm, BF16, "gm", (M, N))
+    gm_p = (_opt if fp8 or (ln and form not in (_LN_LS, _LN_MAP)) else _chk)(gm, BF16, "gm", (M, N))
     q8 = (_chk(fp8[0], FP8, "gm8", (M, N)), _scalar(fp8[1], "scale"), _scalar(fp8[2], "amax")) if fp8 else ()
     sums = (_chk(dgamma, F32, "dgamma", (N,)), _chk(dbeta, F32, "dbeta", (N,))) if ln else ()
     ws = _tn_workspace((ln[1] if ln else g_res).device, int(getattr(L.lib(), form.query)(M, N)))
@@ -166,17 +182,17 @@
 
 
 def layernorm_bwd(dy, x, mean, rstd, gamma, g_res, g_out, gm, dgamma, dbeta, gm_colsum=None, drop=NO_DROP, rows=None, cols=None,
-                  branch=None, dls=None):
+                  branch=None, dls=None, rowmap=None):
     _ln_bwd("layernorm_bwd", (dy, x, mean, rstd, gamma, g_out, dgamma, dbeta), g_res, gm, gm_colsum, drop, rows=rows, cols=cols,
-            branch=branch, dls=dls)
+            branch=branch, dls=dls, rowmap=rowmap)
 
 
 def layernorm_bwd_fp8(dy, x, mean, rstd, gamma, g_res, g_out, gm, gm8, scale, amax, dgamma, dbeta, gm_colsum=None, drop=NO_DROP):
     _ln_bwd("layernorm_bwd_fp8", (dy, x, mean, rstd, gamma, g_out, dgamma, dbeta), g_res, gm, gm_colsum, drop, fp8=(gm8, scale, amax))
 
 
-def grad_mask_cast(g, gm, gm_colsum=None, drop=NO_DROP, rows=None, cols=None, branch=None, dls=None):
-    _ln_bwd("grad_mask_cast", None, g, gm, gm_colsum, drop, rows=rows, cols=cols, branch=branch, dls=dls)
+def grad_mask_cast(g, gm, gm_colsum=None, drop=NO_DROP, rows=None, cols=None, branch=None, dls=None, rowmap=None):
+    _ln_bwd("grad_mask_cast", None, g, gm, gm_colsum, drop, rows=rows, cols=cols, branch=branch, dls=dls, rowmap=rowmap)
 
 
 def grad_mask_cast_fp8(g, gm, gm8, scale, amax, gm_colsum=None, drop=NO_DROP):
@@ -213,7 +229,7 @@
 
 
 def gemm_nt(A, B, out0, epilogue, bias=None, aux=None, out1=None, colsum=None, drop=NO_DROP, embed=None, rows=None, cols=None,
-            branch=None):
+            branch=None, rowmap=None):
     def set_out0(g, M, N):
         if epilogue != L.EPI_EMBED:
             g.out0 = _chk(out0, _OUT0_DTYPE[epilogue], "out0", (M, N))
@@ -231,9 +247,16 @@
         g.embed = e
         g.out0 = _chk(out0, F32, "out0", ((M // tokens) * out_tokens, N))
 
+    if rowmap is not None and A.shape[0] == 0:
+        return
     g, M, N, K = _nt_desc("gemm_nt", "", BF16, A, B, epilogue, bias, set_out0, aux, "aux(u)", out1, colsum, drop)
     ev = _prof_begin()
-    if cols is not None:
+    if rowmap is not None:
+        if rows is not None or cols is not None or branch is not None or epilogue not in (L.EPI_GELU, L.EPI_RESID):
+            raise L.VitsslError(f"gemm_nt: rowmap= belongs to EPI_GELU / EPI_RESID without rows= / cols=, got epilogue {epilogue}")
+        rmap, full = _rowmap(rowmap, M, "gemm_nt")
+        call("vitssl_gemm_bf16_nt_rowmap", C.byref(g), rmap, full, _stream())
+    elif cols is not None:
         if epilogue != L.EPI_RESID:
             raise L.VitsslError(f"gemm_nt: cols= belongs to EPI_RESID, got epilogue {epilogue}")
         call("vitssl_gemm_bf16_nt_ls", C.byref(g), C.byref(_colscale(cols, N, "gemm_nt")),
@@ -446,6 +469,35 @@
 def scatter_rows_f32(src, inv, g):
     rows, cols = g.shape
     call("vitssl_scatter_rows_f32", _chk(src, BF16, "src"), _chk(inv, torch.int32, "inv", (rows,)), _chk(g, F32, "g"), rows, cols, _stream())
+
+
+def _rows_by_index(entry, dtype, per, src, idx, out, scatter):
+    rows, cols = out.shape
+    if src.dim() != 2 or src.shape[1] != cols or cols % per != 0:
+        raise L.VitsslError(f"{entry}: src {tuple(src.shape)} / out {tuple(out.shape)} must share a column count that is a multiple of {per}")
+    i = _chk(idx, torch.int32, entry + " idx", (rows,))
+    o = _chk(out, dtype, entry + " out") if rows else C.c_void_p(0)
+    if scatter:
+        s = _chk(src, dtype, entry + " src") if src.shape[0] else C.c_void_p(0)
+        call("vitssl_" + entry, s, src.shape[0], i, o, rows, cols, _stream())
+    else:
+        call("vitssl_" + entry, _chk(src, dtype, entry + " src"), i, o, rows, cols, _stream())
+
+
+def rows_gather_bf16(src, idx, out):
+    _rows_by_index("rows_gather_bf16", BF16, 8, src, idx, out, False)
+
+
+def rows_gather_f32(src, idx, out):
+    _rows_by_index("rows_gather_f32", F32, 4, src, idx, out, False)
+
+
+def rows_scatter_bf16(src, inv, out):
+    _rows_by_index("rows_scatter_bf16", BF16, 8, src, inv, out, True)
+
+
+def rows_scatter_f32(src, inv, out):
+    _rows_by_index("rows_scatter_f32", F32, 4, src, inv, out, True)
 
 
 def gather_cls_f32(x, out, B, T, D):
```

After: 7945 images/s. No clear change (-0.4%).
